# LayoutLLM-T2I/LayoutLLM-T2I

Hardware: AMD Instinct MI355X
Metric: 512x512 50-step images/sec (PLMS, CFG 7.5, layout-conditioned GLIGEN UNet) (higher is better)
Workload: dtype fp16 (fp32 accumulate); 1 GPU; configs[1]: 512x512, 50 PLMS steps, batch=4/GPU, 8 grounding boxes/image, fp16; survey_config=2, unet_forwards_per_image=102, parallelism=replicas x1, one weight broadcast, no per-step collectives

## Files before the change

include/gligen_hip.h:

```cpp
#ifndef GLIGEN_HIP_H
#define GLIGEN_HIP_H

#include <stdint.h>

#ifdef __cplusplus
extern "C" {
#endif

#define GL_ABI_VERSION 15

#define GL_ERR_BAD_ARG (-1)
#define GL_ERR_UNSUPPORTED (-2)

enum gl_epilogue {
    GL_EPI_BIAS = 0,
    GL_EPI_SILU = 1,
    GL_EPI_GEGLU = 2,
    GL_EPI_RES = 3,
    GL_EPI_GATE_RES = 4,
    GL_EPI_ROWBIAS = 5
};

enum gl_out_mode {
    GL_OUT_F16_ROWMAJOR = 0,
// ... 213 lines not shown
int gl_conv3x3(const gl_conv_args* a, void* stream);
int gl_conv3x3_pad01(const gl_conv_args* a, void* stream);
int gl_attention(const gl_attn_args* a, void* stream);

typedef struct gl_vae_config {
    int32_t ch;
    int32_t ch_mult[8];
    int32_t n_mult;
    int32_t num_res_blocks;
    int32_t z_channels;
    int32_t out_ch;
    int32_t embed_dim;
    float scale_factor;
} gl_vae_config;
typedef struct gl_vae gl_vae;
int gl_vae_create(const gl_vae_config* cfg, gl_vae** out);
int gl_vae_destroy(gl_vae* v);
int gl_vae_num_weights(const gl_vae* v);
int gl_vae_weight_at(const gl_vae* v, int32_t i, gl_weight_info* info);
int64_t gl_vae_weights_bytes(const gl_vae* v);
int gl_vae_load_weights(gl_vae* v, const void* packed, int64_t bytes, void* stream);
int gl_vae_decode(gl_vae* v, const float* z, int32_t B, int32_t side, float* out, int32_t use_graph, void* stream);
int gl_vae_decode_hw(gl_vae* v, const float* z, int32_t B, int32_t h, int32_t w, float* out, int32_t use_graph, void* stream);
int gl_vae_num_launches(const gl_vae* v);
int64_t gl_vae_pool_bytes(const gl_vae* v);
int gl_sizeof_vae_config(void);
int gl_vae_encoder_create(const gl_vae_config* cfg, gl_vae** out);
int gl_vae_encode(gl_vae* v, const float* x, int32_t B, int32_t side, const float* noise, float* z, int32_t use_graph, void* stream);
int gl_vae_encode_hw(gl_vae* v, const float* x, int32_t B, int32_t h, int32_t w, const float* noise, float* z, int32_t use_graph,
                     void* stream);

int gl_clip_patchify(const float* pixel_values, int32_t B, int32_t S, int32_t patch, int32_t Kpad, void* out, void* stream);
int gl_clip_assemble(const void* patch_emb, int32_t ldpe, const float* class_emb, const float* pos_emb, int32_t B, int32_t T,
                     int32_t C, const float* ln_gamma, const float* ln_beta, float ln_eps, float* x, void* stream);
int gl_clip_embed_tokens(const int32_t* ids, const float* tok_emb, const float* pos_emb, int32_t B, int32_t T, int32_t C,
                         int32_t vocab, float* x, void* stream);
int gl_clip_gather_rows(const float* x, int32_t ldx, const int32_t* rows, int32_t B, int32_t C, float* out, void* stream);
int gl_attention_small(const void* q, const void* k, const void* v, int32_t ld, int32_t B, int32_t T, int32_t H, int32_t d,
                       float scale, int32_t causal, void* out, int32_t ldo, void* stream);

int gl_image_to_u8(const float* img_nchw, int32_t B, int32_t H, int32_t W, uint8_t* out_hwc, void* stream);
int gl_resample_h_u8(const uint8_t* in, int32_t B, int32_t H, int32_t W, const int32_t* bounds, const int32_t* coeffs, int32_t ksize,
                     int32_t Wout, uint8_t* out, void* stream);
int gl_resample_v_norm(const uint8_t* in, int32_t B, int32_t H, int32_t W, const int32_t* bounds, const int32_t* coeffs, int32_t ksize,
                       int32_t Hout, int32_t top, int32_t left, int32_t crop_h, int32_t crop_w, const float* mean3, const float* std3,
                       float* out_nchw, uint8_t* out_u8_hwc, void* stream);

int gl_abi_version(void);
int gl_sizeof_gemm_args(void);
int gl_sizeof_conv_args(void);
int gl_sizeof_attn_args(void);
int gl_sizeof_gn_args(void);
int gl_set_option(int key, int value);
int gl_set_handle_option(gl_engine* e, int key, int value);
int gl_clear_handle_options(gl_engine* e);
int gl_vae_set_option(gl_vae* v, int key, int value);
int gl_debug_read(int what, void* dst, int64_t bytes);
int gl_init(void);

#ifdef __cplusplus
}
#endif
#endif
```

layoutllm_t2i_amd/_lib.py:

```python
from __future__ import annotations

import ctypes as C
import os

_HERE = os.path.dirname(os.path.abspath(__file__))
LIB_PATH = os.path.join(_HERE, os.path.basename(os.environ.get("GLIGEN_HIP_LIB", "") or "libgligen_hip.so"))
ABI_VERSION = 15

EPI_BIAS, EPI_SILU, EPI_GEGLU, EPI_RES, EPI_GATE_RES, EPI_ROWBIAS = range(6)
OUT_F16_ROWMAJOR, OUT_F32_NCHW, OUT_F32_ROWMAJOR, OUT_F16_HILO = 0, 1, 2, 3

GROUNDING_IDS = {"text": 0, "text_image": 1}

vp = C.c_void_p
i32 = C.c_int32
i64 = C.c_int64
f32 = C.c_float
fp = C.c_void_p


class GemmArgs(C.Structure):
    _fields_ = [
        ("a", vp), ("lda", i32),
        ("a2", vp), ("lda2", i32), ("ksplit", i32),
# ... 117 lines not shown
    "gl_layernorm": (i32, [vp, i32, i32, vp, i32, fp, fp, i32, i32, i32, i32, i32, f32, fp, vp, i32, i32, vp]),
    "gl_layernorm_stats": (i32, [fp, i32, i32, i32, f32, fp, vp]),
    "gl_split_f32": (i32, [fp, i32, i64, i32, vp, i32, vp]),
    "gl_timestep_embedding_f32": (i32, [fp, i32, i32, fp, vp]),
    "gl_posnet_input_f32": (i32, [fp, fp, fp, fp, fp, i32, i32, i32, fp, vp]),
    "gl_rela_pool_ln3": (i32, [fp, fp, fp, fp, i32, i32, i32, i32, vp, vp, vp, i32, i32, vp, fp, fp, vp, vp]),
    "gl_rela_pool": (i32, [vp, i32, i32, i32, i32, vp, vp, vp, i32, i32, vp, fp, fp, vp, vp]),
    "gl_rela_merge": (i32, [vp, i32, vp, fp, fp, fp, vp, i32, i32, i32, i32, vp, vp, vp, i32, i32, vp, fp, fp, vp, vp]),
    "gl_posnet_input": (i32, [fp, fp, fp, fp, fp, i32, i32, i32, vp, vp]),
    "gl_timestep_embedding": (i32, [fp, i32, i32, vp, vp]),
    "gl_silu_f16": (i32, [vp, vp, i64, vp]),
    "gl_cfg_combine": (i32, [fp, f32, i64, fp, vp]),
    "gl_plms_update": (i32, [fp, fp, fp, fp, fp, f32, f32, f32, f32, f32, f32, f32, f32, f32, i64, fp, vp]),
    "gl_pack_latent": (i32, [fp, i32, i32, i32, i32, i32, i32, vp, vp]),
    "gl_pack_latent_extra": (i32, [fp, fp, i32, i32, i32, i32, i32, i32, i32, i32, vp, vp]),
    "gl_latent_affine_pack": (i32, [fp, fp, fp, f32, i32, i32, i32, i32, vp, vp]),
    "gl_softmax_rows": (i32, [vp, i32, i32, i32, f32, vp]),
    "gl_abi_version": (i32, []),
    "gl_sizeof_gemm_args": (i32, []),
    "gl_sizeof_conv_args": (i32, []),
    "gl_sizeof_attn_args": (i32, []),
    "gl_init": (i32, []),
    "gl_create": (i32, [C.POINTER(UNetConfigC), C.POINTER(vp)]),
    "gl_destroy": (i32, [vp]),
    "gl_num_weights": (i32, [vp]),
    "gl_weight_at": (i32, [vp, i32, C.POINTER(WeightInfo)]),
    "gl_weights_bytes": (i64, [vp]),
    "gl_load_weights": (i32, [vp, vp, i64, i32, vp]),
    "gl_set_conditioning": (i32, [vp, fp, fp, fp, fp, fp, i32, i32, i32, i32, vp]),
    "gl_set_conditioning_hw": (i32, [vp, fp, fp, fp, fp, fp, i32, i32, i32, i32, i32, vp]),
    "gl_set_conditioning_ti": (i32, [vp, fp, fp, fp, fp, fp, fp, fp, fp, i32, i32, i32, i32, i32, vp]),
    "gl_posnet_input_ti": (i32, [fp, fp, fp, fp, fp, fp, fp, fp, fp, i32, i32, i32, vp, vp, vp]),
    "gl_posnet_input_ti_f32": (i32, [fp, fp, fp, fp, fp, fp, fp, fp, fp, i32, i32, i32, fp, fp, vp]),
    "gl_image_ground_feature": (i32, [fp, fp, i32, i32, f32, fp, vp]),
    "gl_set_inpaint_extra": (i32, [vp, fp, i32, vp]),
    "gl_last_error": (i32, [vp, C.c_char_p, i32]),
    "gl_unet_forward": (i32, [vp, fp, fp, f32, i32, f32, i32, fp, i32, vp]),
    "gl_plms_step": (i32, [vp, C.POINTER(PlmsStepArgs), vp]),
    "gl_pool_bytes": (i64, [vp]),
    "gl_num_launches": (i32, [vp]),
    "gl_sizeof_unet_config": (i32, []),
    "gl_sizeof_weight_info": (i32, []),
    "gl_sizeof_plms_step_args": (i32, []),
    "gl_reward_score": (i32, [C.POINTER(RewardArgs), vp]),
    "gl_sizeof_reward_args": (i32, []),
    "gl_ff_fused": (i32, [C.POINTER(FFArgs), vp]),
    "gl_ff_fused_supported": (i32, [i32]),
    "gl_ff_fused_applicable": (i32, [i32, i32]),
    "gl_sizeof_ff_args": (i32, []),
    "gl_image_to_u8": (i32, [vp, i32, i32, i32, vp, vp]),
    "gl_resample_h_u8": (i32, [vp, i32, i32, i32, vp, vp, i32, i32, vp, vp]),
    "gl_resample_v_norm": (i32, [vp, i32, i32, i32, vp, vp, i32, i32, i32, i32, i32, i32, vp, vp, vp, vp, vp]),
    "gl_set_option": (i32, [i32, i32]),
    "gl_set_handle_option": (i32, [vp, i32, i32]),
    "gl_clear_handle_options": (i32, [vp]),
    "gl_vae_set_option": (i32, [vp, i32, i32]),
    "gl_debug_read": (i32, [i32, vp, i64]),
    "gl_vae_create": (i32, [C.POINTER(VaeConfigC), C.POINTER(vp)]),
    "gl_vae_destroy": (i32, [vp]),
    "gl_vae_num_weights": (i32, [vp]),
    "gl_vae_weight_at": (i32, [vp, i32, C.POINTER(WeightInfo)]),
    "gl_vae_weights_bytes": (i64, [vp]),
    "gl_vae_load_weights": (i32, [vp, vp, i64, vp]),
    "gl_vae_decode": (i32, [vp, fp, i32, i32, fp, i32, vp]),
    "gl_vae_decode_hw": (i32, [vp, fp, i32, i32, i32, fp, i32, vp]),
    "gl_vae_num_launches": (i32, [vp]),
    "gl_vae_pool_bytes": (i64, [vp]),
    "gl_sizeof_vae_config": (i32, []),
    "gl_vae_encoder_create": (i32, [C.POINTER(VaeConfigC), C.POINTER(vp)]),
    "gl_vae_encode": (i32, [vp, fp, i32, i32, fp, fp, i32, vp]),
    "gl_vae_encode_hw": (i32, [vp, fp, i32, i32, i32, fp, fp, i32, vp]),
    "gl_conv3x3_pad01": (i32, [C.POINTER(ConvArgs), vp]),
    "gl_vae_posterior": (i32, [fp, fp, fp, fp, f32, i32, i32, i32, i32, fp, fp, vp]),
    "gl_latent_blend": (i32, [fp, fp, fp, fp, f32, f32, i32, i32, i32, i32, i32, vp]),
    "gl_clip_patchify": (i32, [fp, i32, i32, i32, i32, vp, vp]),
    "gl_clip_assemble": (i32, [vp, i32, fp, fp, i32, i32, i32, fp, fp, f32, fp, vp]),
    "gl_clip_embed_tokens": (i32, [vp, fp, fp, i32, i32, i32, i32, fp, vp]),
    "gl_clip_gather_rows": (i32, [fp, i32, vp, i32, i32, fp, vp]),
    "gl_attention_small": (i32, [vp, vp, vp, i32, i32, i32, i32, i32, f32, i32, vp, i32, vp]),
}

_lib = None
_inited = set()


class HipLibraryError(RuntimeError):
    pass


def lib() -> C.CDLL:
    global _lib
    if _lib is not None:
        return _lib
    if not os.path.exists(LIB_PATH):
        raise HipLibraryError(
            f"{LIB_PATH} not found: build it with `python -m layoutllm_t2i_amd.csrc.build` "
            "(or __graft_entry__.build()).  There is no CPU fallback for the denoising path.")
    try:
        l = C.CDLL(LIB_PATH)
    except OSError as e:
        raise HipLibraryError(f"cannot load {LIB_PATH}: {e}") from e
    for name, (res, args) in PROTOTYPES.items():
        try:
            fn = getattr(l, name)
        except AttributeError as e:
            raise HipLibraryError(f"{LIB_PATH} does not export {name}") from e
        fn.restype = res
        fn.argtypes = args
    if l.gl_abi_version() != ABI_VERSION:
        raise HipLibraryError(f"ABI version mismatch: lib {l.gl_abi_version()} vs host {ABI_VERSION}")
    for cls, fn in ((GemmArgs, l.gl_sizeof_gemm_args), (ConvArgs, l.gl_sizeof_conv_args), (AttnArgs, l.gl_sizeof_attn_args),
                    (UNetConfigC, l.gl_sizeof_unet_config), (WeightInfo, l.gl_sizeof_weight_info),
                    (PlmsStepArgs, l.gl_sizeof_plms_step_args), (RewardArgs, l.gl_sizeof_reward_args), (FFArgs, l.gl_sizeof_ff_args),
                    (VaeConfigC, l.gl_sizeof_vae_config), (GnArgs, l.gl_sizeof_gn_args)):
        if C.sizeof(cls) != fn():
            raise HipLibraryError(f"struct size mismatch for {cls.__name__}: host {C.sizeof(cls)} vs lib {fn()}")
    _lib = l
    return l


def init_device(index=None) -> None:
    import torch
    if index is None:
        index = torch.cuda.current_device()
    if index not in _inited:
        with torch.cuda.device(index):
            check(lib().gl_init(), "gl_init")
        _inited.add(index)


def unet_config_c(cfg) -> UNetConfigC:
    c = UNetConfigC()
    c.in_channels, c.model_channels, c.out_channels, c.num_res_blocks = cfg.in_channels, cfg.model_channels, cfg.out_channels, cfg.num_res_blocks
    if len(cfg.channel_mult) > 8 or len(cfg.attention_resolutions) > 8:
        raise ValueError("at most 8 levels / attention resolutions")
    c.n_levels = len(cfg.channel_mult)
    for i, m in enumerate(cfg.channel_mult):
        c.channel_mult[i] = int(m)
    c.n_attn_res = len(cfg.attention_resolutions)
    for i, m in enumerate(cfg.attention_resolutions):
        c.attention_resolutions[i] = int(m)
    c.num_heads, c.context_dim = cfg.num_heads, cfg.context_dim
    c.pos_in_dim, c.pos_out_dim, c.fourier_freqs, c.max_objs = cfg.pos_in_dim, cfg.pos_out_dim, cfg.fourier_freqs, cfg.max_objs
    c.split_weights = int(bool(getattr(cfg, "split_weights", False)))
    c.grounding = GROUNDING_IDS[getattr(cfg, "grounding", "text")]
    c.inpaint_mode = int(bool(getattr(cfg, "inpaint_mode", False)))
    c.no_relation = int(not getattr(cfg, "relation", True))
    return c


def create_engine(cfg) -> int:
    h = vp()
    cc = unet_config_c(cfg)
    check(lib().gl_create(C.byref(cc), C.byref(h)), "gl_create")
    return h.value


def create_vae(cfg, encoder: bool = False) -> int:
    cc = VaeConfigC()
    cc.ch, cc.n_mult, cc.num_res_blocks, cc.z_channels, cc.out_ch = cfg.ch, len(cfg.ch_mult), cfg.num_res_blocks, cfg.z_channels, cfg.out_ch
    for i, m in enumerate(cfg.ch_mult):
        cc.ch_mult[i] = int(m)
    cc.embed_dim, cc.scale_factor = cfg.embed_dim, float(cfg.scale_factor)
    h = vp()
    if encoder:
        check(lib().gl_vae_encoder_create(C.byref(cc), C.byref(h)), "gl_vae_encoder_create")
    else:
        check(lib().gl_vae_create(C.byref(cc), C.byref(h)), "gl_vae_create")
    return h.value


def vae_weight_table(handle: int):
    l = lib()
    out = []
    info = WeightInfo()
    for i in range(l.gl_vae_num_weights(handle)):
        check(l.gl_vae_weight_at(handle, i, C.byref(info)), "gl_vae_weight_at")
        out.append((info.name.decode(), int(info.offset), int(info.nbytes), int(info.dtype), tuple(int(info.shape[k]) for k in range(info.ndim))))
    return out, int(l.gl_vae_weights_bytes(handle))


def weight_table(handle: int):
    l = lib()
    out = []
    info = WeightInfo()
    for i in range(l.gl_num_weights(handle)):
        check(l.gl_weight_at(handle, i, C.byref(info)), "gl_weight_at")
        out.append((info.name.decode(), int(info.offset), int(info.nbytes), int(info.dtype), tuple(int(info.shape[k]) for k in range(info.ndim))))
    return out, int(l.gl_weights_bytes(handle))


def last_error(handle: int) -> str:
    buf = C.create_string_buffer(512)
    n = lib().gl_last_error(handle, buf, len(buf))
    return buf.value.decode() if n > 0 else ""


def check(code: int, what: str) -> None:
    if code != 0:
        raise HipLibraryError(f"{what} failed with code {code}" + (" (bad argument)" if code == -1 else ""))
```

layoutllm_t2i_amd/csrc/engine.hip:

```cpp
#include "common.h"
#include "gligen_hip.h"
#include "opts.h"

#include <cmath>
#include <cstring>
#include <map>
#include <string>
#include <tuple>
#include <unordered_map>
#include <vector>


namespace {

constexpr int CIN_PAD = 64;
constexpr int64_t ALIGN = 256;
#define g_fuse_merge_ln gl_opt(25)
#define g_fuse_vt gl_opt(21)
#define g_force_fuser gl_opt(20)
#define g_precise gl_opt(41)
#define g_h1_f32 gl_opt(42)
#define g_rela_compact gl_opt(43)
#define g_w3 gl_opt(45)
#define g_in_split gl_opt(38)
// ... 39 lines not shown
    for (size_t i = (size_t)blockIdx.x * blockDim.x + threadIdx.x; i < total; i += (size_t)gridDim.x * blockDim.x) {
        const int wd = (int)(i % words);
        const size_t row = i / words;
        const int k = (int)(row % n);
        const size_t cb = row / n;
        const int b = (int)(cb % B), c = (int)(cb / B);
        dst[(((size_t)b * 2 + c) * n + k) * words + wd] = src[i];
    }
}

#pragma clang fp contract(off)
__device__ __forceinline__ void py_slice(int start, int stop, int len, int* s, int* e) {
    if (start < 0) { start += len; if (start < 0) start = 0; } else if (start > len) start = len;
    if (stop < 0) { stop += len; if (stop < 0) stop = 0; } else if (stop > len) stop = len;
    *s = start;
    *e = stop > start ? stop : start;
}
__global__ void rela_rects_kernel(const float* __restrict__ boxes, const float* __restrict__ masks, int B, int n, int h, int w,
                                  int* __restrict__ rects, int* __restrict__ nvalid, int* __restrict__ poison) {
    const int k = blockIdx.x * blockDim.x + threadIdx.x;
    if (k >= B) return;
    float count = 0.0f;
    for (int i = 0; i < n; ++i) count += masks[(size_t)k * n + i];
    int nv = 0, bad = 0;
    bool open = true;
    for (int i = 0; i < n; ++i) {
        int* r = rects + ((size_t)k * n + i) * 4;
        r[0] = r[1] = r[2] = r[3] = 0;
        if (!open) continue;
        const float* bx = boxes + ((size_t)k * n + i) * 4;
        const int left = (int)(bx[0] * (float)w);
        const int top = (int)(bx[1] * (float)h);
        const int right = (int)fminf(bx[2] * (float)w, (float)w);
        const int bottom = (int)fminf(bx[3] * (float)h, (float)h);
        if ((float)i < count && left != right && top != bottom) {
            int t, b, l, rr;
            py_slice(top, bottom, h, &t, &b);
            py_slice(left, right, w, &l, &rr);
            r[0] = t; r[1] = b; r[2] = l; r[3] = rr;
            if ((b - t) * (rr - l) == 0) bad = 1;
            nv = i + 1;
        } else {
            open = false;
        }
    }
    nvalid[k] = nv;
    poison[k] = bad;
}
#pragma clang fp contract(fast)

}

struct gl_engine {
    bool strict_hoists_ok = false;
    int strict_hoists_w3 = -1;
    gl_unet_config cfg;
    std::vector<BlockD> input_blocks, output_blocks;
    BlockD middle;
    int out_channels_last = 0;
    std::vector<LayerD> st_layers;
    std::vector<std::string> names;
    std::unordered_map<std::string, WInfo> tab;
    int64_t total_bytes = 0;
    const char* wbase = nullptr;
    bool has_sd = false;
    std::unordered_map<std::string, int> emb_off;
    int emb_total = 0;
    std::vector<float> gate_tanh;
    struct Buf { void* p; size_t bytes; };
    std::unordered_map<std::string, Buf> pool;
    bool pool_changed = false, capturing = false;
    int device = -1;
    bool cond_set = false;
    int Bn = 0, R = 0, Lc = 0, lat_h = 0, lat_w = 0;
    bool extra_set = false;
    int extra_bs = 0;
    std::map<GraphKey, hipGraphExec_t> graphs;
    float fuser_scale_cur = -1e30f;
    std::vector<float> gate_host;
    float* gate_pin[2] = {nullptr, nullptr};
    hipEvent_t gate_pin_ev[2] = {nullptr, nullptr};
    bool gate_pin_used[2] = {false, false};
    size_t gate_pin_bytes = 0;
    int gate_pin_next = 0;
    int launches = 0;
    int rel_slots = 0;
    int opt_epoch = 0;
    int ovr_epoch = 0;
    gl_opt_overrides ovr;
    std::string err;
    hipStream_t cap_stream = nullptr;

    const WInfo* wi(const std::string& n) const {
        auto it = tab.find(n);
        return it == tab.end() ? nullptr : &it->second;
    }
    const void* W(const std::string& n) const {
        auto it = tab.find(n);
        if (it == tab.end() || wbase == nullptr) return nullptr;
        return wbase + it->second.off;
    }
    const float* Wf(const std::string& n) const { return reinterpret_cast<const float*>(W(n)); }

    void* buf(const std::string& tag, size_t bytes) {
        auto it = pool.find(tag);
        if (it != pool.end() && it->second.bytes >= bytes) return it->second.p;
// ... 72 lines not shown
            BlockD b;
            b.layers.push_back(LayerD{RES, "input_blocks." + std::to_string(idx) + ".0", ch, mult * mc, 0});
            ch = mult * mc;
            if (has_attn(ds)) b.layers.push_back(LayerD{ST, "input_blocks." + std::to_string(idx) + ".1", ch, ch, ch / heads});
            e->input_blocks.push_back(b);
            chans.push_back(ch);
        }
        if (level != c.n_levels - 1) {
            const int idx = (int)e->input_blocks.size();
            e->input_blocks.push_back(BlockD{{LayerD{DOWN, "input_blocks." + std::to_string(idx) + ".0.op", ch, ch, 0}}});
            chans.push_back(ch);
            ds *= 2;
        }
    }
    e->middle.layers = {LayerD{RES, "middle_block.0", ch, ch, 0}, LayerD{ST, "middle_block.1", ch, ch, ch / heads},
                        LayerD{RES, "middle_block.2", ch, ch, 0}};
    for (int level = c.n_levels - 1; level >= 0; --level) {
        const int mult = c.channel_mult[level];
        for (int i = 0; i <= c.num_res_blocks; ++i) {
            const int ich = chans.back();
            chans.pop_back();
            const int idx = (int)e->output_blocks.size();
            BlockD b;
            b.layers.push_back(LayerD{RES, "output_blocks." + std::to_string(idx) + ".0", ch + ich, mc * mult, 0});
            ch = mc * mult;
            if (has_attn(ds)) b.layers.push_back(LayerD{ST, "output_blocks." + std::to_string(idx) + ".1", ch, ch, ch / heads});
            if (level && i == c.num_res_blocks) {
                b.layers.push_back(LayerD{UP, "output_blocks." + std::to_string(idx) + "." + std::to_string(b.layers.size()) + ".conv", ch, ch, 0});
                ds /= 2;
            }
            e->output_blocks.push_back(b);
        }
    }
    e->out_channels_last = ch;
}

template <class F>
void for_all_layers(gl_engine* e, F f) {
    for (auto& b : e->input_blocks) for (auto& l : b.layers) f(l);
    for (auto& l : e->middle.layers) f(l);
    for (auto& b : e->output_blocks) for (auto& l : b.layers) f(l);
}

void build_table(gl_engine* e) {
    const gl_unet_config& c = e->cfg;
    const int mc = c.model_channels, te = 4 * mc, ctx = c.context_dim;
    add_lin(e, "time_embed.0", te, mc);
    add_lin(e, "time_embed.2", te, te);
    add_conv3(e, "input_blocks.0.0", CIN_PAD, mc, false);
    if (!c.inpaint_mode) add_conv3(e, "sd_first_conv", CIN_PAD, mc, false);
    int off = 0;
    for_all_layers(e, [&](LayerD& l) {
        const std::string& p = l.prefix;
        if (l.kind == DOWN || l.kind == UP) {
            add_conv3(e, p, l.cin, l.cout);
        } else if (l.kind == RES) {
            add_norm(e, p + ".in_layers.0", l.cin);
            add_conv3(e, p + ".in_layers.2", l.cin, l.cout);
            add_norm(e, p + ".out_layers.0", l.cout);
            add_conv3(e, p + ".out_layers.3", l.cout, l.cout);
            if (l.cin != l.cout) add_lin_split(e, p + ".skip_connection", l.cout, l.cin);
            e->emb_off[p] = off;
            off += l.cout;
        } else if (l.kind == ST) {
            const int C = l.cin;
            e->st_layers.push_back(l);
            add_norm(e, p + ".norm", C);
            add_lin_split(e, p + ".proj_in", C, C);
            add_lin_split(e, p + ".proj_out", C, C);
            const std::string t = p + ".transformer_blocks.0";
            add_mat(e, t + ".attn1.qkv.w", 3 * C, C);
            add_lin(e, t + ".attn1.o", C, C);
            add_mat(e, t + ".attn2.q.w", C, C);
            add_mat(e, t + ".attn2.kv.w", 2 * C, ctx);
            add_lin(e, t + ".attn2.o", C, C);
            add_ff(e, t + ".ff", C);
            for (const char* n : {".norm1", ".norm2", ".norm3"}) add_norm(e, t + n, C);
            const std::string f = t + ".fuser";
            add_lin(e, f + ".linear", C, ctx);
            add_mat(e, f + ".attn.qkv.w", 3 * C, C);
            add_lin(e, f + ".attn.o", C, C);
            add_ff(e, f + ".ff", C);
            add_norm(e, f + ".norm1", C);
            add_norm(e, f + ".norm2", C);
            add_w(e, f + ".tanh_attn", 1, {1});
            add_w(e, f + ".tanh_dense", 1, {1});
            if (c.no_relation) return;
            const std::string r = t + ".rela_fuse";
            add_mat(e, r + ".attn.q.w", C, C);
            add_mat(e, r + ".attn.kv.w", 2 * C, ctx);
            add_lin(e, r + ".attn.o", C, C);
            add_ff(e, r + ".ff", C);
            for (const char* n : {".norm1", ".norm2", ".norm3"}) add_norm(e, r + n, C);
            add_w(e, r + ".tanh_attn", 1, {1});
            add_w(e, r + ".tanh_dense", 1, {1});
        }
    });
    e->emb_total = off;
    add_lin(e, "emb_all", off, te);
    add_norm(e, "out.0", e->out_channels_last);
    add_conv3(e, "out.2", e->out_channels_last, c.out_channels);
    if (c.grounding == 1) {
        add_w(e, "position_net.null_text", 1, {c.pos_in_dim});
        add_w(e, "position_net.null_image", 1, {c.pos_in_dim});
        add_w(e, "position_net.null_xyxy", 1, {8 * c.fourier_freqs});
        for (const char* n : {"position_net.linears_text", "position_net.linears_image"}) {
            const std::string p = n;
// ... 57 lines not shown
        const WInfo* wi = e->wi(p + ".w");
        if (!wi) return GL_ERR_BAD_ARG;
        gl_gemm_args g{};
        g.a = a.p; g.lda = a.ld; g.a2 = o.a2.p; g.lda2 = o.a2.ld; g.ksplit = o.ksplit;
        g.w = e->W(p + ".w"); g.bias = o.bias ? e->Wf(p + ".b") : nullptr;
        if (o.bias && !g.bias) return GL_ERR_BAD_ARG;
        g.M = M; g.N = (int)wi->shape[0]; g.K = (int)wi->shape[1];
        const bool strict = g_strict != 0 && e->cfg.split_weights;
        if (o.wsplit || e->cfg.split_weights) {
            const int Kc = g.K / 2;
            g.ldw = g.K; g.K = Kc;
            if (a.hilo) {
                g.kwrap = Kc; g.K = 2 * Kc;
                const bool third = strict ? (g_strict_w3 != 0) : (o.wsplit && g_w3 > 0 && M > (g_w3 < 1024 ? 1024 : g_w3));
                if (third) {
                    if (o.a2.p != nullptr) return GL_ERR_BAD_ARG;
                    g.K = 3 * Kc; g.a2 = a.p; g.lda2 = a.ld; g.ksplit = 2 * Kc;
                }
            }
        } else if (a.hilo) {
            g.kwrap = g.K; g.ldw = g.K; g.K = 2 * g.K;
        }
        g.epi = o.epi; g.out_mode = o.out_mode; g.out = out; g.ldc = ldc;
        g.res = o.res.p; g.ldres = o.res.ld; g.res_f32 = o.res.f32; g.gate = o.gate;
        g.out2 = o.out2; g.ldc2 = o.ldc2;
        if (o.tail) {
            const VtTail& t = *o.tail;
            g.vt = t.vt; g.vt_lo = t.vt_lo; g.vt_col0 = t.col0; g.vt_rows = t.rows; g.vt_d = t.d; g.vt_ld = t.ld; g.vt_H = t.H;
        }
        g.workspace = ws; g.workspace_bytes = GL_WS_BYTES;
        ++launches;
        return gl_gemm(&g, st);
    }
    int gemm(Act a, const std::string& p, int M, void* out, int ldc) { return gemm(a, p, M, out, ldc, GemmOpt{}); }

    struct RowBias { const void* p = nullptr; int ld = 0, rows_per_sample = 0; };
    struct ConvOpt {
        int stride = 1, ups = 0, epi = GL_EPI_BIAS;
        Rows res{};
        RowBias rowbias{};
        void* out2 = nullptr;
        int nchw_hw = 0;
    };
    int conv(Act in, const std::string& p, int B, int Hin, int Win, void* out, int out_mode, const ConvOpt& o) {
        const WInfo* wi = e->wi(p + ".w");
        if (!wi) return GL_ERR_BAD_ARG;
        const int Cin = in.hilo ? in.ld / 2 : in.ld;
        gl_conv_args a{};
        a.w_split = wi->shape[1] == 18 * (int64_t)Cin;
        a.in_split = in.hilo ? ((a.w_split && g_strict_w3 != 0) ? 3 : 2) : 0;
        a.in = in.p; a.B = B; a.Hin = Hin; a.Win = Win; a.Cin = Cin;
        a.Hout = o.ups ? 2 * Hin : (Hin + 2 - 3) / o.stride + 1;
        a.Wout = o.ups ? 2 * Win : (Win + 2 - 3) / o.stride + 1;
        a.stride = o.stride; a.upsample2x = o.ups;
        a.g.w = e->W(p + ".w"); a.g.bias = e->Wf(p + ".b"); a.g.N = (int)wi->shape[0];
        a.g.epi = o.epi; a.g.out_mode = out_mode; a.g.out = out; a.g.ldc = a.g.N; a.g.hw = o.nchw_hw;
        a.g.res = o.res.p; a.g.ldres = o.res.ld; a.g.res_f32 = o.res.f32;
        a.g.rowbias = o.rowbias.p; a.g.ld_rowbias = o.rowbias.ld; a.g.rows_per_sample = o.rowbias.rows_per_sample;
        a.g.rowbias_f32 = o.rowbias.p != nullptr && (g_precise != 0 || g_strict != 0);
        a.g.out2 = o.out2; a.g.ldc2 = a.g.N;
        a.g.workspace = ws; a.g.workspace_bytes = GL_WS_BYTES;
        ++launches;
        return gl_conv3x3(&a, st);
    }

    enum LnFlags { LN_X_F32 = 1, LN_X2_F32 = 4, LN_Y_HILO = 8 };
    struct LnOpt {
        int rows_out = 0;
        float* stats = nullptr;
        Rows x2{}; int rows2 = 0;
        bool y_lo = false;
    };
    int ln(Rows x, half_t* y, int ldy, const std::string& p, int rows, int C, const LnOpt& o) {
        const int flags = (x.f32 ? LN_X_F32 : 0) | (o.x2.f32 ? LN_X2_F32 : 0) | (o.y_lo ? LN_Y_HILO : 0);
        ++launches;
        return gl_layernorm(x.p, x.ld, flags, y, ldy, e->Wf(p + ".g"), e->Wf(p + ".b"), e->Bn, rows, o.rows_out ? o.rows_out : rows, 0, C, 1e-5f, o.stats,
                            o.x2.p, C, o.rows2, st);
    }
    int ln(Rows x, half_t* y, int ldy, const std::string& p, int rows, int C) { return ln(x, y, ldy, p, rows, C, LnOpt{}); }
    int split(const float* x, int64_t rows, int C, half_t* y) {
        ++launches;
        return gl_split_f32(x, C, rows, C, y, 2 * C, st);
    }
    struct GnOpt {
        const void* x2 = nullptr; int C2 = 0;
        int ldo = 0;
        half_t* out_lo = nullptr;
        half_t* raw = nullptr; int ldraw = 0;
    };
    int gn(Rows x, int HW, const std::string& p, float eps, int silu, half_t* out, const GnOpt& o) {
        const int B = e->Bn, nchunk = gn_nchunk(HW);
        float* partial = e->f32("gn.partial", (size_t)B * nchunk * 64);
        CKP(partial);
        launches += gl_groupnorm_launches_ex(x.ld + o.C2, HW, x.f32);
        gl_gn_args a{};
        a.x1 = x.p; a.C1 = x.ld; a.x2 = o.x2; a.C2 = o.C2; a.x_f32 = x.f32; a.B = B; a.HW = HW;
        a.gamma = e->Wf(p + ".g"); a.beta = e->Wf(p + ".b"); a.eps = eps; a.silu = silu;
        a.out = out; a.ldo = o.ldo; a.out_lo = o.out_lo; a.raw = o.raw; a.ldraw = o.ldraw;
        a.partial = partial; a.nchunk = nchunk;
        return gl_groupnorm_ex(&a, st);
    }
    int gn(Rows x, int HW, const std::string& p, float eps, int silu, half_t* out) { return gn(x, HW, p, eps, silu, out, GnOpt{}); }
    int attn(Mat q, Mat k, VtMat vt, MatOut out, int d, int Nq, int Nk) {
        gl_attn_args a{};
        a.q_lo = q.lo; a.k_lo = k.lo; a.vt_lo = vt.lo; a.out_lo = out.lo;
        a.q = q.p; a.q_bstride = q.bs; a.ldq = q.ld; a.k = k.p; a.k_bstride = k.bs; a.ldk = k.ld; a.vt = vt.p; a.ldvt = vt.ld;
        a.out = out.p; a.o_bstride = out.bs; a.ldo = out.ld; a.B = e->Bn; a.H = e->cfg.num_heads; a.d = d; a.Nq = Nq; a.Nk = Nk;
        a.scale = 1.0f / sqrtf((float)d);
// ... 427 lines not shown
                }
                CK(r.conv(in, l.prefix, Bn, sh, sw, o.f, GL_OUT_F32_ROWMAJOR, {.stride = up ? 1 : 2, .ups = up, .out2 = o.h}));
                sh = oh; sw = ow;
            } else {
                return GL_ERR_BAD_ARG;
            }
            h = o;
            h_c = l.cout;
            if (half_pending && !(j + 1 < b.layers.size() && b.layers[j + 1].kind == ST)) {
                CK(r.dup_rows(h.f, (size_t)B0 * sh * sw * h_c * 4));
                if (h.h) CK(r.dup_rows(h.h, (size_t)B0 * sh * sw * h_c * 2));
                half_pending = false;
            }
        }
        return 0;
    };

    for (size_t i = 1; i < e->input_blocks.size(); ++i) {
        CK(run_block(e->input_blocks[i], "skip." + std::to_string(i), nullptr, i + 1 < e->input_blocks.size() ? &e->input_blocks[i + 1] : &e->middle,
                     share && i == 1));
        skips.push_back({h, sh, sw, h_c});
    }
    CK(run_block(e->middle, "mid", nullptr, e->output_blocks.empty() ? nullptr : &e->output_blocks[0]));
    for (size_t i = 0; i < e->output_blocks.size(); ++i) {
        const Skip sk = skips.back();
        skips.pop_back();
        if (sk.h != sh || sk.w != sw) return GL_ERR_BAD_ARG;
        CK(run_block(e->output_blocks[i], "out." + std::to_string(i), &sk, i + 1 < e->output_blocks.size() ? &e->output_blocks[i + 1] : nullptr));
    }
    const int ocl = e->out_channels_last;
    half_t* g = e->h16("fin.gn", (size_t)Bn * sh * sw * ocl * (strict ? 2 : 1));
    CKP(g);
    if (!precise) CKP(h.h);
    CK(r.gn({precise ? (const void*)h.f : (const void*)h.h, ocl, precise}, sh * sw, "out.0", 1e-5f, 1, g,
            {.ldo = strict ? 2 * ocl : 0, .out_lo = strict ? g + ocl : nullptr}));
    CK(r.conv({g, strict ? 2 * ocl : ocl, strict}, "out.2", Bn, sh, sw, eps, GL_OUT_F32_NCHW, {.nchw_hw = sh * sw}));
    if (n_launches) *n_launches = r.launches;
    return 0;
}

}

extern "C" int gl_create(const gl_unet_config* cfg, gl_engine** out) {
    if (!cfg || !out) return GL_ERR_BAD_ARG;
    if (cfg->n_levels <= 0 || cfg->n_levels > 8 || cfg->n_attn_res < 0 || cfg->n_attn_res > 8 || cfg->num_heads <= 0) return GL_ERR_BAD_ARG;
    if (cfg->model_channels % 64 || cfg->context_dim % 64 || cfg->pos_in_dim % 8 || cfg->pos_out_dim != cfg->context_dim) return GL_ERR_UNSUPPORTED;
    if ((cfg->pos_in_dim + 8 * cfg->fourier_freqs) % 64) return GL_ERR_UNSUPPORTED;
    if (cfg->grounding != 0 && cfg->grounding != 1) return GL_ERR_UNSUPPORTED;
    if (cfg->max_objs <= 0 || n_ground(*cfg) > 64) return GL_ERR_UNSUPPORTED;
    if (cfg->no_relation != 0 && cfg->no_relation != 1) return GL_ERR_UNSUPPORTED;
    if ((cfg->inpaint_mode != 0 && cfg->inpaint_mode != 1) || first_conv_in(*cfg) > CIN_PAD) return GL_ERR_UNSUPPORTED;
    gl_engine* e = new gl_engine();
    e->cfg = *cfg;
    build_plan(e);
    build_table(e);
    *out = e;
    return 0;
}

extern "C" int gl_destroy(gl_engine* e) {
    if (!e) return GL_ERR_BAD_ARG;
    e->drop_graphs();
    for (auto& kv : e->pool) (void)hipFree(kv.second.p);
    if (e->cap_stream) (void)hipStreamDestroy(e->cap_stream);
    for (int k = 0; k < 2; ++k) {
        if (e->gate_pin_ev[k]) { (void)hipEventSynchronize(e->gate_pin_ev[k]); (void)hipEventDestroy(e->gate_pin_ev[k]); }
        if (e->gate_pin[k]) (void)hipHostFree(e->gate_pin[k]);
    }
    delete e;
    return 0;
}

extern "C" int gl_num_weights(const gl_engine* e) { return e ? (int)e->names.size() : GL_ERR_BAD_ARG; }
extern "C" int64_t gl_weights_bytes(const gl_engine* e) { return e ? e->total_bytes : -1; }
extern "C" int gl_weight_at(const gl_engine* e, int32_t i, gl_weight_info* info) {
    if (!e || !info || i < 0 || i >= (int)e->names.size()) return GL_ERR_BAD_ARG;
    const std::string& n = e->names[i];
    if (n.size() >= sizeof(info->name)) return GL_ERR_BAD_ARG;
    const WInfo& w = e->tab.at(n);
    memset(info, 0, sizeof(*info));
    memcpy(info->name, n.c_str(), n.size());
    info->offset = w.off; info->nbytes = w.bytes; info->dtype = w.dtype; info->ndim = w.ndim;
    for (int k = 0; k < 4; ++k) info->shape[k] = w.shape[k];
    return 0;
}

extern "C" int gl_load_weights(gl_engine* e, const void* packed, int64_t bytes, int32_t has_sd_conv, void* stream) {
    if (!e || !packed || bytes < e->total_bytes) return GL_ERR_BAD_ARG;
    if (reinterpret_cast<uintptr_t>(packed) % 16) return GL_ERR_BAD_ARG;
    int dev = 0;
    if (hipGetDevice(&dev) != hipSuccess) return GL_ERR_BAD_ARG;
    e->device = dev;
    CK(gl_init());
    e->wbase = reinterpret_cast<const char*>(packed);
    if (has_sd_conv && e->cfg.inpaint_mode) {
        e->err = "gl_load_weights: an inpaint_mode handle has no sd_first_conv slots (its first conv is not restorable)";
        return GL_ERR_BAD_ARG;
    }
    e->has_sd = has_sd_conv != 0;
    e->drop_graphs();
    const size_t n = e->st_layers.size();
    e->gate_tanh.assign(n * 4, 0.0f);
    hipStream_t st = (hipStream_t)stream;
    if (hipStreamSynchronize(st) != hipSuccess) return GL_ERR_BAD_ARG;
    for (size_t i = 0; i < n; ++i) {
        const std::string t = e->st_layers[i].prefix + ".transformer_blocks.0";
// ... 424 lines not shown
```

layoutllm_t2i_amd/csrc/gemm8.hip:

```cpp
#include "common.h"
#include "gligen_hip.h"
#include "gemm_shared.h"
#include "opts.h"
#include <atomic>
#include <type_traits>

#ifndef G8_S3_PHASES
#define G8_S3_PHASES 3
#endif

namespace {

template <int BM_, int BN>
struct G8 {
    static constexpr int BM = BM_;
    static constexpr int NA = BM / 64;
    static constexpr int MI = BM / 64;
    static constexpr int MH = BM / 128;
    static constexpr int BK = 64;
    static constexpr int PW = BN / 2;
    static constexpr int TN = PW / 16;
    static constexpr int A_BYTES = BM * BK * 2;
    static constexpr int B_BYTES = BN * BK * 2;
    static constexpr int STAGE = A_BYTES + B_BYTES;
    static constexpr int NST = 3;
    static constexpr int LDS = NST * STAGE;
    static constexpr int B_UNITS = BN / 8;
    static constexpr int NB0 = (B_UNITS + 7) / 8;
    static constexpr int NB1 = B_UNITS / 4 - NB0;
    static constexpr int NI0 = NA + NB0;
    static constexpr int NI1 = NA + NB1;
    static_assert(PW % 16 == 0 && B_UNITS % 4 == 0 && NB1 >= 1 && (BM == 256 || BM == 128), "tile shape");
    static_assert(NA + 1 >= 3, "the first phase issues three instructions (X_FIRST): two A units + one B unit at least");
    static_assert(STAGE % 128 == 0, "stage alignment (the k-half XOR of the fragment offsets relies on it)");
};

template <int BN>
struct G8X {
    static constexpr int A_UNITS = 33;
    static constexpr int A_BYTES = A_UNITS * 1024;
    static constexpr int A_STRIDE = A_BYTES + 128;
    static constexpr int B_BYTES = BN * 64 * 2;
    static constexpr int B_BASE = 2 * A_STRIDE;
    static constexpr int LDS = B_BASE + 3 * B_BYTES;
    static_assert(A_STRIDE % 128 == 0 && B_BASE % 128 == 0, "the k-half XOR of the fragment offsets stays inside a 128-byte row");
    static_assert(LDS >= 8 * 32 * (BN / 2 + 4) * 4, "the epilogue restages through the ring memory");
};

template <int N>
__device__ __forceinline__ void wait_vm() {
    asm volatile("s_waitcnt vmcnt(%0)" ::"n"(N) : "memory");
}

__device__ __forceinline__ f32x4 mfma16(half8_t a, half8_t b, f32x4 c) {
    return __builtin_amdgcn_mfma_f32_16x16x32_f16(a, b, c, 0, 0, 0);
}

#define G8_SBAR()                              \
    do {                                       \
        __builtin_amdgcn_sched_barrier(0);     \
        __builtin_amdgcn_s_barrier();          \
        __builtin_amdgcn_sched_barrier(0);     \
    } while (0)

__device__ unsigned long long g8_stamps[4 * 4096];

template <int BM, int BN, bool CONV, int DBG = 0, bool S3 = false, bool KXR = false>
__global__ __launch_bounds__(512, 2) void gemm8_kernel(gl_gemm_args p, ConvGeom cg, int splitk, int kt_per_split, int order_flags) {
    using C = G8<BM, BN>;
    constexpr int KT = S3 ? 32 : 64;
    constexpr int NA = C::NA, MI = C::MI, MH = C::MH;
    unsigned long long ts0 = 0, ts1 = 0, ts2 = 0;
    if constexpr (DBG & 1) ts0 = __builtin_readcyclecounter();
    constexpr int TN = C::TN, PW = C::PW;
    extern __shared__ __attribute__((aligned(16))) unsigned char smem[];

    const int tid = threadIdx.x;
    const int lane = tid & 63;
    const int wave = __builtin_amdgcn_readfirstlane(tid >> 6);
    const int grp = wave >> 2;
    const int wm = wave & 3;
    const int M = p.M, N = p.N, K = S3 ? p.kwrap : p.K;

    const int nt = (N + BN - 1) / BN;
    int tile;
    {
        const int nwg = gridDim.x;
        const int bid = blockIdx.x;
        const int q = nwg >> 3, r = nwg & 7;
        const int xcd = bid & 7, local = bid >> 3;
        tile = (xcd < r ? xcd * (q + 1) : r * (q + 1) + (xcd - r) * q) + local;
    }
    const int mt_ = (M + C::BM - 1) / C::BM;
    const int order_m = order_flags & 1;
    const bool tap_major = CONV && (order_flags & 2);
    const int tmi = order_m ? tile % mt_ : tile / nt;
    const int m0 = tmi * C::BM;
    const int n0 = (order_m ? tile / mt_ : tile - tmi * nt) * BN;
    const int kt_begin = blockIdx.z * kt_per_split;
    const int kt_end = min(K / KT, kt_begin + kt_per_split);
    const int nkt = kt_end - kt_begin;

    const half_t* __restrict__ Ag = reinterpret_cast<const half_t*>(p.a);
    const half_t* __restrict__ A2g = reinterpret_cast<const half_t*>(p.a2);
    const half_t* __restrict__ Wg = reinterpret_cast<const half_t*>(p.w);
    const half_t* zsrc = cg.zero;

    const int srow = lane >> 3;
    const int sslot = lane & 7;
    int a_dst[NA];
    const half_t* aptr[NA];
    unsigned amask = 0u;
    unsigned cmask[NA];
    const int k_first = kt_begin * KT;
    const int a_lo = S3 ? (CONV ? (cg.Cin >> 1) : p.kwrap) : 0;
    auto chunk_off = [&](const int c, const int lo_off) __attribute__((always_inline)) -> int {
        if constexpr (S3) return ((c & 3) << 3) + ((c >> 2) ? lo_off : 0);
        else return c << 3;
    };
#pragma unroll
    for (int u = 0; u < NA; ++u) {
        const int trow0 = (16 * NA) * (wave >> 1) + 16 * (wave & 1) + 8 * (u & 1) + 32 * (u >> 1);
        a_dst[u] = trow0 * 128;
        const int r = trow0 + srow;
        const int gc = chunk_off(sslot ^ ((r >> 1) & 7), a_lo);
        const int m = m0 + r;
        const bool rowok = m < M;
        aptr[u] = zsrc; cmask[u] = 0u;
        if constexpr (CONV) {
            if (rowok) {
                int b, oy, ox;
                const int hw = cg.Hout * cg.Wout;
                if (((cg.Wout & (cg.Wout - 1)) | (hw & (hw - 1))) == 0) {
                    const int lw = __builtin_ctz(cg.Wout), lhw = __builtin_ctz(hw);
                    b = m >> lhw;
                    const int rr = m & (hw - 1);
                    oy = rr >> lw;
                    ox = rr & (cg.Wout - 1);
                } else {
                    b = m / hw;
                    const int rr = m - b * hw;
                    oy = rr / cg.Wout;
                    ox = rr - oy * cg.Wout;
                }
                const int sh = S3 ? 0 : cg.shift;
                const int iy = cg.ups ? oy : oy * cg.stride + sh, ix = cg.ups ? ox : ox * cg.stride + sh;
                const int hlim = cg.ups ? cg.Hout : cg.Hin, wlim = cg.ups ? cg.Wout : cg.Win;
                const unsigned rb = (iy >= 1 ? 1u : 0u) | 2u | (iy + 1 < hlim ? 4u : 0u);
                const unsigned cb = (ix >= 1 ? 1u : 0u) | 2u | (ix + 1 < wlim ? 4u : 0u);
                cmask[u] = ((rb & 1u) ? cb : 0u) | (cb << 3) | ((rb & 4u) ? (cb << 6) : 0u) | ((unsigned)(oy & 1) << 9) | ((unsigned)(ox & 1) << 10);
                const int sy = cg.ups ? (oy >> 1) : iy, sx = cg.ups ? (ox >> 1) : ix;
                aptr[u] = cg.in + ((size_t)(b * cg.Hin + sy) * cg.Win + sx) * cg.Cin + gc;
            }
        } else {
            if (rowok) {
                if (!S3 && A2g != nullptr && k_first >= p.ksplit) aptr[u] = A2g + (size_t)m * p.lda2 + (k_first - p.ksplit) + gc;
                else aptr[u] = Ag + (size_t)m * p.lda + k_first + gc;
                amask |= 1u << u;
            }
        }
    }
    const int nb = grp ? C::NB1 : C::NB0;
    const int bunit0 = grp ? 4 * C::NB0 + C::NB1 * (wave - 4) : C::NB0 * wave;
    const half_t* bptr[C::NB0];
    unsigned bmask = 0u;
#pragma unroll
    for (int j = 0; j < C::NB0; ++j) {
        const int r = 8 * (bunit0 + j) + srow;
        const int gc = chunk_off(sslot ^ ((r >> 1) & 7), p.kwrap);
        const int n = n0 + r;
        const bool ok = (j < nb) && (r < BN) && (n < N);
        bptr[j] = ok ? (Wg + (size_t)n * p.ldw + gc) : zsrc;
        if (ok) bmask |= 1u << j;
    }

    const int ncblk = CONV ? K / 576 : 1;
    const int in_lim = tap_major ? ncblk : 9;
    int is_out = 0, is_in = 0;
    int is_cblk = 0, is_tap = 0;
    if constexpr (CONV) {
        const int t64 = S3 ? (kt_begin >> 1) : kt_begin;
        is_out = t64 / in_lim;
        is_in = t64 - is_out * in_lim;
    }
    int is_kt = kt_begin;

    int is_off = 0;
    int is_ky = 0, is_kx = 0, is_acb = 0;
    int is_boff = 0;
    auto issue_begin = [&]() __attribute__((always_inline)) {
        if constexpr (CONV && S3) {
            is_tap = tap_major ? is_out : is_in;
            is_cblk = tap_major ? is_in : is_out;
            is_ky = (is_tap * 11) >> 5;
            is_kx = is_tap - is_ky * 3;
            is_acb = (is_cblk << 1) + (is_kt & 1);
            is_off = ((is_ky - 1) * cg.Win + (is_kx - 1)) * cg.Cin + (is_acb << 5);
            is_boff = ((is_cblk * 9 + is_tap) << 6) + ((is_kt & 1) << 5);
        } else if constexpr (S3) {
            is_boff = is_kt << 5;
        } else if constexpr (CONV) {
            is_tap = tap_major ? is_out : is_in;
            is_cblk = tap_major ? is_in : is_out;
            is_ky = (is_tap * 11) >> 5;
            is_kx = is_tap - is_ky * 3;
            is_acb = (cg.cwrap != 0 && is_cblk >= cg.cwrap) ? is_cblk - cg.cwrap : is_cblk;
            is_off = ((is_ky - 1) * cg.Win + (is_kx - 1)) * cg.Cin + (is_acb << 6);
            is_boff = (is_cblk * 9 + is_tap) << 6;
            if (p.kwrap != 0 && is_boff >= p.kwrap) is_boff -= p.kwrap;
        } else {
            is_boff = is_kt << 6;
            if (p.kwrap != 0 && is_boff >= p.kwrap) is_boff -= p.kwrap;
            if (A2g != nullptr && is_kt * 64 == p.ksplit && is_kt != kt_begin) {
#pragma unroll
                for (int u = 0; u < NA; ++u) {
                    const int r = (a_dst[u] >> 7) + srow;
                    const int m = m0 + r;
                    if (m < M) aptr[u] = A2g + (size_t)m * p.lda2 + ((sslot ^ ((r >> 1) & 7)) << 3);
                }
            }
        }
    };
    auto unit_src = [&](const int i) __attribute__((always_inline)) -> const half_t* {
        const half_t* src;
        if (i < NA) {
            const int u = i;
            if constexpr (CONV) {
                int off = is_off;
                if (cg.ups) {
                    const int ry = (is_ky - 1 + (int)((cmask[u] >> 9) & 1u)) >> 1, rx = (is_kx - 1 + (int)((cmask[u] >> 10) & 1u)) >> 1;
                    off = (ry * cg.Win + rx) * cg.Cin + (is_acb << (S3 ? 5 : 6));
                }
                const uint64_t a = reinterpret_cast<uint64_t>(aptr[u] + off), z = reinterpret_cast<uint64_t>(zsrc);
                const uint64_t keep = (uint64_t)0 - (uint64_t)((cmask[u] >> is_tap) & 1u);
                src = reinterpret_cast<const half_t*>((a & keep) | (z & ~keep));
            } else {
                src = aptr[u];
                aptr[u] += ((amask >> u) & 1u) ? KT : 0;
            }
            if constexpr (DBG & 2) src = zsrc;
        } else {
            const int j = i - NA;
            src = ((bmask >> (j < C::NB0 ? j : 0)) & 1u) ? bptr[j < C::NB0 ? j : 0] + is_boff : zsrc;
            if constexpr (DBG & 4) src = zsrc;
        }
        return src;
    };
    auto unit_fire = [&](const int st, const int i, const half_t* src) __attribute__((always_inline)) {
        unsigned char* sbase = smem + st * C::STAGE;
        if (i < NA) {
            glds16(src, reinterpret_cast<half_t*>(sbase + a_dst[i]));
        } else {
            const int j = i - NA;
            if (j < nb) glds16(src, reinterpret_cast<half_t*>(sbase + C::A_BYTES + (bunit0 + j) * 1024));
        }
    };
    auto issue_unit = [&](const int st, const int i) __attribute__((always_inline)) { unit_fire(st, i, unit_src(i)); };
    auto issue_advance = [&]() __attribute__((always_inline)) {
        ++is_kt;
        if constexpr (CONV) {
            if (!S3 || (is_kt & 1) == 0) {
                if (++is_in == in_lim) { is_in = 0; ++is_out; }
            }
        }
    };
    auto issue_all = [&](const int st) __attribute__((always_inline)) {
        issue_begin();
#pragma unroll
        for (int i = 0; i < NA + C::NB0; ++i) issue_unit(st, i);
        issue_advance();
    };

    const int lr = lane & 15, lq = lane >> 4;
    const int fsw = ((lq ^ ((lr >> 1) & 7)) << 4);
    const int a_off = ((BM / 4) * wm + lr) * 128 + fsw;
    const int b_off = C::A_BYTES + (PW * grp + lr) * 128 + fsw;

    f32x4 acc[MI][TN];
#pragma unroll
    for (int mi = 0; mi < MI; ++mi)
#pragma unroll
        for (int ni = 0; ni < TN; ++ni)
// ... 291 lines not shown
                acc[mi][ni] = mfma16(bf[ni], use_lo ? al[mi] : ah[mi], acc[mi][ni]);
                if constexpr (MORE) {
                    if constexpr (cnt > 0) { if (i == GP - 1) unit_fire(st_is, first + 0, nsrc[0]); }
                    if constexpr (cnt > 1) { if (i == 2 * GP - 1) unit_fire(st_is, first + 1, nsrc[1]); }
                    if constexpr (cnt > 2) { if (i == 3 * GP - 1) unit_fire(st_is, first + 2, nsrc[2]); }
                    if constexpr (cnt > 3) { if (i == 4 * GP - 1) unit_fire(st_is, first + 3, nsrc[3]); }
                    if constexpr (cnt > 4) { if (i == 5 * GP - 1) unit_fire(st_is, first + 4, nsrc[4]); }
                }
            }
            if constexpr (MORE) {
                if constexpr (cnt > 0) { __builtin_amdgcn_sched_group_barrier(0x008, GP, 0); __builtin_amdgcn_sched_group_barrier(0x020, 1, 0); }
                if constexpr (cnt > 1) { __builtin_amdgcn_sched_group_barrier(0x008, GP, 0); __builtin_amdgcn_sched_group_barrier(0x020, 1, 0); }
                if constexpr (cnt > 2) { __builtin_amdgcn_sched_group_barrier(0x008, GP, 0); __builtin_amdgcn_sched_group_barrier(0x020, 1, 0); }
                if constexpr (cnt > 3) { __builtin_amdgcn_sched_group_barrier(0x008, GP, 0); __builtin_amdgcn_sched_group_barrier(0x020, 1, 0); }
                if constexpr (cnt > 4) { __builtin_amdgcn_sched_group_barrier(0x008, GP, 0); __builtin_amdgcn_sched_group_barrier(0x020, 1, 0); }
                __builtin_amdgcn_sched_group_barrier(0x008, TOT - cnt * GP, 0);
            }
            __builtin_amdgcn_s_setprio(0);
            if constexpr (MORE && LAST) issue_advance();
            G8_SBAR();
        };
        phase(std::integral_constant<int, 0>{});
        phase(std::integral_constant<int, 1>{});
        if constexpr (NPH == 3) phase(std::integral_constant<int, 2>{});
        st_rd = (st_rd == 2) ? 0 : st_rd + 1;
        st_is = (st_is == 2) ? 0 : st_is + 1;
    };
    int t = 0;
    if constexpr (KXR) {
    } else if constexpr (S3) {
        for (; t + 2 < nkt; ++t) ktile3(std::true_type{});
        for (; t < nkt; ++t) ktile3(std::false_type{});
    } else {
        for (; t + 2 < nkt; ++t) ktile(std::true_type{});
        for (; t < nkt; ++t) ktile(std::false_type{});
    }
    if (grp == 0) G8_SBAR();
    if constexpr (DBG & 1) ts2 = __builtin_readcyclecounter();

    constexpr int EPS = PW + 4;
    constexpr int CG8 = PW / 8;
    constexpr int ITEMS = 32 * CG8;
    static_assert(ITEMS % 64 == 0, "whole sweeps");
    float* stage = reinterpret_cast<float*>(smem) + wave * (32 * EPS);
    const int epi = p.epi;
    const float* __restrict__ bias = p.bias;
    float gate = 1.0f;
    if (splitk == 1 && epi == GL_EPI_GATE_RES) gate = p.gate[0];
    const int nbase = n0 + PW * grp;
    half_t* outp = reinterpret_cast<half_t*>(p.out);
    constexpr int NQ = ITEMS / 64;
    const bool vt_wave = p.vt != nullptr && nbase >= p.vt_col0;
    const bool generic = splitk == 1 && !vt_wave && epi != GL_EPI_GEGLU;
    Fin8Aux aux[MH][NQ];
    if (generic) {
#pragma unroll
        for (int h = 0; h < MH; ++h)
#pragma unroll
            for (int q = 0; q < NQ; ++q) {
                const int idx = lane + 64 * q;
                const int r = idx / CG8, c = (idx - r * CG8) * 8;
                const int m = m0 + (BM / 4) * wm + 32 * h + r, n = nbase + c;
                if (m < M && n < N) fin8_load(p, m, n, aux[h][q]);
            }
    }
    float vt_bias[2] = {0.0f, 0.0f};
    if (splitk == 1 && vt_wave && bias) {
#pragma unroll
        for (int j = 0; j < 2; ++j) {
            const int col = 64 * j + lane;
            if (col < PW && nbase + col < N) vt_bias[j] = bias[nbase + col];
        }
    }
    float gg_bias[16];
#pragma unroll
    for (int j = 0; j < 16; ++j) gg_bias[j] = 0.0f;
    if constexpr (PW == 64) {
        if (splitk == 1 && epi == GL_EPI_GEGLU && bias) {
            const int nx = nbase + (lane & 3) * 8;
            if (nx < N) {
#pragma unroll
                for (int j = 0; j < 8; ++j) { gg_bias[j] = bias[nx + j]; gg_bias[8 + j] = bias[nx + 32 + j]; }
            }
        }
    }
#pragma unroll
    for (int h = 0; h < MH; ++h) {
        const int mbase = m0 + (BM / 4) * wm + 32 * h;
        __builtin_amdgcn_fence(__ATOMIC_RELEASE, "wavefront");
        __builtin_amdgcn_wave_barrier();
#pragma unroll
        for (int mi = 0; mi < 2; ++mi)
#pragma unroll
            for (int ni = 0; ni < TN; ++ni)
                *reinterpret_cast<float4*>(stage + (16 * mi + lr) * EPS + 16 * ni + 4 * lq) =
                    make_float4(acc[2 * h + mi][ni][0], acc[2 * h + mi][ni][1], acc[2 * h + mi][ni][2], acc[2 * h + mi][ni][3]);
        __builtin_amdgcn_fence(__ATOMIC_RELEASE, "wavefront");
        __builtin_amdgcn_wave_barrier();
        if (splitk > 1) {
            float* ws = reinterpret_cast<float*>(p.workspace) + (size_t)blockIdx.z * M * N;
#pragma unroll
            for (int q = 0; q < ITEMS / 64; ++q) {
                const int idx = lane + 64 * q;
                const int r = idx / CG8, c = (idx - r * CG8) * 8;
                const int m = mbase + r, n = nbase + c;
                if (m < M && n < N) {
                    float* o = ws + (size_t)m * N + n;
                    *reinterpret_cast<float4*>(o) = *reinterpret_cast<const float4*>(stage + r * EPS + c);
                    *reinterpret_cast<float4*>(o + 4) = *reinterpret_cast<const float4*>(stage + r * EPS + c + 4);
                }
            }
        } else if (vt_wave) {
            half_t* vtp = reinterpret_cast<half_t*>(p.vt);
#pragma unroll
            for (int c0 = 0; c0 < PW; c0 += 64) {
                const int col = c0 + lane;
                const int n = nbase + col;
                if (col < PW && n < N) {
                    const int nv = n - p.vt_col0;
                    const int hh = nv / p.vt_d;
                    const int cc = nv - hh * p.vt_d;
                    const float bv = vt_bias[c0 / 64];
                    half_t* vtl = reinterpret_cast<half_t*>(p.vt_lo);
#pragma unroll
                    for (int tg = 0; tg < 4; ++tg) {
                        const int m = mbase + tg * 8;
                        if (m >= M) continue;
                        half8_t o, l;
#pragma unroll
                        for (int k = 0; k < 8; ++k) {
                            float v = stage[(tg * 8 + k) * EPS + col] + bv;
                            if (vtl) v = pin_value(v);
                            o[k] = (half_t)v;
                            l[k] = vtl ? (half_t)(v - (float)o[k]) : (half_t)0.0f;
                        }
                        if ((p.vt_rows & 7) == 0) {
                            const int b = m / p.vt_rows;
                            const int key = m - b * p.vt_rows;
                            const size_t at = ((size_t)(b * p.vt_H + hh) * p.vt_d + cc) * p.vt_ld + key;
                            st16(vtp + at, *reinterpret_cast<uint4*>(&o));
                            if (vtl) st16(vtl + at, *reinterpret_cast<uint4*>(&l));
                        } else {
#pragma unroll
                            for (int k = 0; k < 8; ++k) {
                                const int mm = m + k;
                                if (mm < M) {
                                    const int b = mm / p.vt_rows;
                                    const int key = mm - b * p.vt_rows;
                                    const size_t at = ((size_t)(b * p.vt_H + hh) * p.vt_d + cc) * p.vt_ld + key;
                                    vtp[at] = o[k];
                                    if (vtl) vtl[at] = l[k];
                                }
                            }
                        }
                    }
                }
            }
        } else if (epi == GL_EPI_GEGLU) {
            if constexpr (PW == 64) {
#pragma unroll
                for (int ps = 0; ps < 2; ++ps) {
                    const int r = ps * 16 + (lane >> 2);
                    const int pc = (lane & 3) * 8;
                    const int m = mbase + r;
                    const int nx = nbase + pc;
                    if (m < M && nx < N) {
                        const float4 x0 = *reinterpret_cast<const float4*>(stage + r * EPS + pc);
                        const float4 x1 = *reinterpret_cast<const float4*>(stage + r * EPS + pc + 4);
                        const float4 g0 = *reinterpret_cast<const float4*>(stage + r * EPS + pc + 32);
                        const float4 g1 = *reinterpret_cast<const float4*>(stage + r * EPS + pc + 36);
                        float xv[8] = {x0.x, x0.y, x0.z, x0.w, x1.x, x1.y, x1.z, x1.w};
                        float gv[8] = {g0.x, g0.y, g0.z, g0.w, g1.x, g1.y, g1.z, g1.w};
                        half8_t o, lo8 = {};
#pragma unroll
                        for (int j = 0; j < 8; ++j) {
                            const float a = xv[j] + gg_bias[j], b = gv[j] + gg_bias[8 + j];
                            float y = a * gelu_erf_f(b);
                            if (p.out_mode == GL_OUT_F16_HILO) y = pin_value(y);
                            o[j] = (half_t)y;
                            if (p.out_mode == GL_OUT_F16_HILO) lo8[j] = (half_t)(y - (float)o[j]);
                        }
                        st16(outp + (size_t)m * p.ldc + (nbase >> 1) + pc, *reinterpret_cast<uint4*>(&o));
                        if (p.out_mode == GL_OUT_F16_HILO) st16(outp + (size_t)m * p.ldc + (N >> 1) + (nbase >> 1) + pc, *reinterpret_cast<uint4*>(&lo8));
                    }
                }
            }
        } else {
#pragma unroll
            for (int q = 0; q < NQ; ++q) {
                const int idx = lane + 64 * q;
                const int r = idx / CG8, c = (idx - r * CG8) * 8;
                const int m = mbase + r, n = nbase + c;
                if (m < M && n < N) {
                    const float4 a0 = *reinterpret_cast<const float4*>(stage + r * EPS + c);
                    const float4 a1 = *reinterpret_cast<const float4*>(stage + r * EPS + c + 4);
                    float v[8] = {a0.x, a0.y, a0.z, a0.w, a1.x, a1.y, a1.z, a1.w};
                    fin8_store(p, gate, m, n, v, aux[h][q]);
                }
            }
        }
    }
    if constexpr (DBG & 1) {
        asm volatile("s_waitcnt vmcnt(0)" ::: "memory");
        const unsigned long long ts3 = __builtin_readcyclecounter();
        const int bid = blockIdx.x + gridDim.x * blockIdx.z;
        if (tid == 0 && bid < 4096) {
            g8_stamps[4 * bid + 0] = ts0; g8_stamps[4 * bid + 1] = ts1; g8_stamps[4 * bid + 2] = ts2; g8_stamps[4 * bid + 3] = ts3;
        }
    }
}

#define g8_dbg gl_opt(32)
#define g8_kxr gl_opt(54)

std::atomic<uint64_t> g8_kxr_launches{0};

static bool kxr_default(const gl_gemm_args&, const ConvGeom&, int , int ) { return true; }

constexpr int G8_MAX_DEVICES = 64;
const half_t* g8_zero_page[G8_MAX_DEVICES] = {};

template <int BM, int BN, bool CONV, bool S3 = false>
int launch8(const gl_gemm_args& g, const ConvGeom& cg_in, int zs, int kper, int order_m, hipStream_t st) {
    int dev = -1;
    if (hipGetDevice(&dev) != hipSuccess || dev < 0 || dev >= G8_MAX_DEVICES) return GL_ERR_BAD_ARG;
    if (!g8_zero_page[dev]) return GL_ERR_BAD_ARG;
    ConvGeom cg = cg_in;
    cg.zero = g8_zero_page[dev];
    const int mt = gl_cdiv(g.M, BM), nt = gl_cdiv(g.N, BN);
    dim3 grid(mt * nt, 1, zs);
    bool done = false;
    if constexpr (CONV && !S3 && BM == 256) {
        const bool eligible = cg.stride == 1 && !cg.ups && cg.shift == 0 && g.kwrap == 0 && cg.cwrap == 0 && !(order_m & 2) && kper > 0 &&
                              (kper % 9) == 0 && cg.Hin == cg.Hout && cg.Win == cg.Wout && g.K == 9 * cg.Cin && g.a2 == nullptr;
        if (eligible && (g8_kxr == 1 || (g8_kxr == 2 && kxr_default(g, cg, BN, zs)))) {
            void (*k)(gl_gemm_args, ConvGeom, int, int, int) = gemm8_kernel<BM, BN, true, 0, false, true>;
            if constexpr (BN == 160) {
                if (g8_dbg == 1) k = gemm8_kernel<BM, BN, true, 1, false, true>;
                if (g8_dbg == 3) k = gemm8_kernel<BM, BN, true, 3, false, true>;
            }
            k<<<grid, dim3(512), G8X<BN>::LDS, st>>>(g, cg, zs, kper, order_m);
            GL_CHECK_LAUNCH();
            g8_kxr_launches.fetch_add(1, std::memory_order_relaxed);
            return 0;
        }
    }
    if constexpr (S3) {
        gemm8_kernel<BM, BN, CONV, 0, true><<<grid, dim3(512), G8<BM, BN>::LDS, st>>>(g, cg, zs, kper, order_m);
        done = true;
    } else if constexpr (BN == 160 && BM == 256) {
        void (*k)(gl_gemm_args, ConvGeom, int, int, int) = nullptr;
        if (g8_dbg == 1) k = gemm8_kernel<BM, BN, CONV, 1>;
        if (g8_dbg == 3) k = gemm8_kernel<BM, BN, CONV, 3>;
        if (k) {
            k<<<grid, dim3(512), G8<BM, BN>::LDS, st>>>(g, cg, zs, kper, order_m);
            done = true;
        }
    }
    if (!done) gemm8_kernel<BM, BN, CONV><<<grid, dim3(512), G8<BM, BN>::LDS, st>>>(g, cg, zs, kper, order_m);
    GL_CHECK_LAUNCH();
    return 0;
}

template <int BM, int BN, bool CONV>
int set_attr8() {
    hipError_t e = hipFuncSetAttribute((const void*)gemm8_kernel<BM, BN, CONV>, hipFuncAttributeMaxDynamicSharedMemorySize, G8<BM, BN>::LDS);
    if (e == hipSuccess) e = hipFuncSetAttribute((const void*)gemm8_kernel<BM, BN, CONV, 0, true>, hipFuncAttributeMaxDynamicSharedMemorySize, G8<BM, BN>::LDS);
    if constexpr (CONV && BM == 256) {
        if (e == hipSuccess) e = hipFuncSetAttribute((const void*)gemm8_kernel<BM, BN, true, 0, false, true>, hipFuncAttributeMaxDynamicSharedMemorySize, G8X<BN>::LDS);
        if constexpr (BN == 160) {
            if (e == hipSuccess) e = hipFuncSetAttribute((const void*)gemm8_kernel<BM, BN, true, 1, false, true>, hipFuncAttributeMaxDynamicSharedMemorySize, G8X<BN>::LDS);
            if (e == hipSuccess) e = hipFuncSetAttribute((const void*)gemm8_kernel<BM, BN, true, 3, false, true>, hipFuncAttributeMaxDynamicSharedMemorySize, G8X<BN>::LDS);
        }
    }
    if constexpr (BN == 160 && BM == 256) {
        if (e == hipSuccess) e = hipFuncSetAttribute((const void*)gemm8_kernel<BM, BN, CONV, 1>, hipFuncAttributeMaxDynamicSharedMemorySize, G8<BM, BN>::LDS);
        if (e == hipSuccess) e = hipFuncSetAttribute((const void*)gemm8_kernel<BM, BN, CONV, 3>, hipFuncAttributeMaxDynamicSharedMemorySize, G8<BM, BN>::LDS);
    }
    return e == hipSuccess ? 0 : (int)e;
}

}

int gl8_supported(const gl_gemm_args& g, bool conv, int* bn_out) {
    if (g.out_mode == GL_OUT_F32_NCHW) return 0;
    if ((g.K % 64) != 0 || (g.N % 8) != 0 || g.M < 256) return 0;
    int bn = 128;
    if (g.epi != GL_EPI_GEGLU && (g.N % 160) == 0) bn = 160;
    if (g.vt != nullptr && (g.vt_col0 % (bn / 2)) != 0) {
        if (bn == 160 && (g.vt_col0 % 64) == 0) bn = 128;
        else return 0;
    }
    if (g.a2 != nullptr && (g.ksplit % 64) != 0) return 0;
    *bn_out = bn;
    return 1;
}

template <bool S3>
static int gl8_launch_t(const gl_gemm_args& g, const ConvGeom& cg, bool conv, int bm, int bn, int zs, int kper, int order_m, hipStream_t st) {
    if (bm == 256 && bn == 160) return conv ? launch8<256, 160, true, S3>(g, cg, zs, kper, order_m, st) : launch8<256, 160, false, S3>(g, cg, zs, kper, order_m, st);
    if (bm == 256 && bn == 128) return conv ? launch8<256, 128, true, S3>(g, cg, zs, kper, order_m, st) : launch8<256, 128, false, S3>(g, cg, zs, kper, order_m, st);
    if (bm == 128 && bn == 160) return conv ? launch8<128, 160, true, S3>(g, cg, zs, kper, order_m, st) : launch8<128, 160, false, S3>(g, cg, zs, kper, order_m, st);
    if (bm == 128 && bn == 128) return conv ? launch8<128, 128, true, S3>(g, cg, zs, kper, order_m, st) : launch8<128, 128, false, S3>(g, cg, zs, kper, order_m, st);
    return GL_ERR_UNSUPPORTED;
}
int gl8_launch(const gl_gemm_args& g, const ConvGeom& cg, bool conv, int bm, int bn, int zs, int kper, int order_m, hipStream_t st, bool s3) {
    return s3 ? gl8_launch_t<true>(g, cg, conv, bm, bn, zs, kper, order_m, st) : gl8_launch_t<false>(g, cg, conv, bm, bn, zs, kper, order_m, st);
}

int gl8_init(void) {
    int e;
    void* zp = nullptr;
    int dev = -1;
    if (hipGetDevice(&dev) != hipSuccess || dev < 0 || dev >= G8_MAX_DEVICES) return GL_ERR_BAD_ARG;
    if (hipGetSymbolAddress(&zp, HIP_SYMBOL(g_zero16)) != hipSuccess) return GL_ERR_BAD_ARG;
    g8_zero_page[dev] = reinterpret_cast<const half_t*>(zp);
    if ((e = set_attr8<256, 160, false>())) return e;
    if ((e = set_attr8<256, 160, true>())) return e;
    if ((e = set_attr8<256, 128, false>())) return e;
    if ((e = set_attr8<256, 128, true>())) return e;
    if ((e = set_attr8<128, 160, false>())) return e;
    if ((e = set_attr8<128, 160, true>())) return e;
    if ((e = set_attr8<128, 128, false>())) return e;
    if ((e = set_attr8<128, 128, true>())) return e;
    return 0;
}

uint64_t gl8_kxr_launch_count(void) { return g8_kxr_launches.load(std::memory_order_relaxed); }

int gl8_read_stamps(void* dst, int64_t bytes) {
    if (bytes > (int64_t)sizeof(unsigned long long) * 4 * 4096) return GL_ERR_BAD_ARG;
    hipError_t e = hipMemcpyFromSymbol(dst, HIP_SYMBOL(g8_stamps), (size_t)bytes, 0, hipMemcpyDeviceToHost);
    void* p = nullptr;
    if (e == hipSuccess) e = hipGetSymbolAddress(&p, HIP_SYMBOL(g8_stamps));
    if (e == hipSuccess) e = hipMemset(p, 0, sizeof(unsigned long long) * 4 * 4096);
    return (int)e;
}
```

layoutllm_t2i_amd/csrc/gemm_conv.hip:

```cpp
#include <atomic>
#include <cstring>
#include "common.h"
#include "gligen_hip.h"
#include "gemm_shared.h"
#include "opts.h"

namespace {

#define g_opt_ksplit gl_opt(13)
#define g_opt_geglu32 gl_opt(8)
#define g_opt_big gl_opt(7)
#define g_opt_small gl_opt(4)
#define g_opt_splitk_tiles gl_opt(5)
#define g_opt_splitk_tiles_conv gl_opt(GL_OPT_SPLITK_TILES_CONV)
#define g_opt_splitk_nk gl_opt(6)
#define g_opt_skinny gl_opt(24)
#define g_opt_order gl_opt(23)
#define g_opt_tile gl_opt(2)
#define g_opt_g8 gl_opt(30)
#define g_opt_g8_tiles gl_opt(31)
#define g_opt_g8_tapmajor gl_opt(33)
#define g_opt_g8_minkt gl_opt(34)
std::atomic<uint64_t> g8_launches{0};
#define g_opt_g8_shortk gl_opt(37)
// ... 607 lines not shown
            const long t256 = (long)gl_cdiv(g.M, 256) * gl_cdiv(g.N, bn);
            if (t256 >= g_opt_big) {
                if (shape == 1) return launch<256, 160, 4, 1, CONV, 32>(g, cg, st);
                return launch<256, 128, 4, 1, CONV, 32>(g, cg, st);
            }
        }
        if constexpr (!CONV) {
            if (shape == 3 && (g_opt_ksplit == 2 || ((g_opt_ksplit == 1 || g_opt_ksplit == 4 || g_opt_ksplit == 5) && g.K >= 1024)))
                return launch<64, 128, 1, 2, false, 64, 2>(g, cg, st);
        }
        if (shape == 3) return launch<64, 128, 2, 2, CONV, 64>(g, cg, st);
        if (shape == 1) return launch<128, 160, 4, 1, CONV, 64>(g, cg, st);
        if (shape == 0) return launch<128, 128, 2, 2, CONV, 64>(g, cg, st);
        return launch<256, 64, 4, 1, CONV, 64>(g, cg, st);
    } else {
        static_assert(!CONV, "BK 32 dispatch is for plain GEMMs");
        if (shape == 3) return launch<64, 128, 2, 2, false, 32>(g, cg, st);
        return launch<128, 128, 2, 2, false, 32>(g, cg, st);
    }
}

template <bool CONV>
int dispatch(const gl_gemm_args& g, const ConvGeom& cg, hipStream_t st) {
    if (g.M <= 0 || g.N <= 0 || g.K <= 0 || (g.K % 64) != 0) return GL_ERR_BAD_ARG;
    if (g.out_mode < 0 || g.out_mode > GL_OUT_F16_HILO) return GL_ERR_BAD_ARG;
    if (g.out_mode == GL_OUT_F16_HILO && g.ldc < (g.epi == GL_EPI_GEGLU ? g.N : 2 * g.N)) return GL_ERR_BAD_ARG;
    if ((g.vt != nullptr && (g.out_mode == GL_OUT_F16_HILO) != (g.vt_lo != nullptr)) || (g.vt == nullptr && g.vt_lo != nullptr)) return GL_ERR_BAD_ARG;
    if (g.out_mode != GL_OUT_F32_NCHW && ((g.N % 8) != 0 || (g.ldc % 8) != 0)) return GL_ERR_BAD_ARG;
    if (g.out_mode == GL_OUT_F32_ROWMAJOR && g.out2 != nullptr && (g.ldc2 % 8) != 0) return GL_ERR_BAD_ARG;
    if (g.out_mode == GL_OUT_F32_ROWMAJOR && g.epi == GL_EPI_GEGLU) return GL_ERR_UNSUPPORTED;
    if (g.res != nullptr && (g.ldres % 8) != 0) return GL_ERR_BAD_ARG;
    if (g.rowbias != nullptr && (g.ld_rowbias % 8) != 0) return GL_ERR_BAD_ARG;
    if (g.epi == GL_EPI_GEGLU && (g.N % 64) != 0) return GL_ERR_BAD_ARG;
    if (g.a2 != nullptr && (g.ksplit % 64) != 0) return GL_ERR_BAD_ARG;
    if ((g.epi == GL_EPI_RES || g.epi == GL_EPI_GATE_RES) && g.res == nullptr) return GL_ERR_BAD_ARG;
    if (g.epi == GL_EPI_GATE_RES && g.gate == nullptr) return GL_ERR_BAD_ARG;
    if (g.epi == GL_EPI_ROWBIAS && (g.rowbias == nullptr || g.rows_per_sample <= 0)) return GL_ERR_BAD_ARG;
    if (g.vt != nullptr && (g.epi != GL_EPI_BIAS || (g.out_mode != GL_OUT_F16_ROWMAJOR && g.out_mode != GL_OUT_F16_HILO) || (g.vt_col0 % 64) != 0 || g.vt_col0 <= 0 ||
                            g.vt_col0 >= g.N || g.vt_rows <= 0 || g.vt_d <= 0 || ((g.N - g.vt_col0) % g.vt_d) != 0 || (g.vt_ld % 8) != 0 ||
                            g.vt_ld < g.vt_rows || g.vt_H * g.vt_d != g.N - g.vt_col0))
        return GL_ERR_BAD_ARG;
    if constexpr (!CONV) {
        if (g.vt_lo == nullptr && skinny_ok(g)) {
            gemm_skinny_kernel<<<dim3(g.N / 32, gl_cdiv(g.M, 32)), dim3(256), 0, st>>>(g);
            GL_CHECK_LAUNCH();
            return 0;
        }
    }
    const bool need8 = g.vt_lo != nullptr;
    if (need8) {
        int bn_ = 0;
        if (!g_opt_g8 || !gl8_supported(g, CONV, &bn_)) return GL_ERR_UNSUPPORTED;
    }
    if (g_opt_g8) {
        int bn = 0;
        if (gl8_supported(g, CONV, &bn)) {
            const int nk = g.K / 64;
            auto plan_split = [&](const int tiles_) {
                int sk = 1;
                if (tiles_ < g_opt_g8_tiles && g.workspace && g.epi != GL_EPI_GEGLU && g.vt == nullptr) {
                    sk = 256 / tiles_;
                    if (sk > nk / g_opt_g8_minkt) sk = nk / g_opt_g8_minkt;
                    while (sk > 1 && (int64_t)sk * g.M * g.N * 4 > g.workspace_bytes) --sk;
                    if (sk < 1) sk = 1;
                }
                return sk;
            };
            int bm = 256;
            int tiles = gl_cdiv(g.M, 256) * gl_cdiv(g.N, bn);
            int splitk = plan_split(tiles);
            if (tiles * 2 <= 256 && g.epi != GL_EPI_GEGLU && g.vt == nullptr) {
                const bool want = CONV ? ((g_opt_g8_bm128 & 4) || ((g_opt_g8_bm128 & 1) && nk / splitk <= 16)) : ((g_opt_g8_bm128 & 2) != 0);
                if (want) {
                    bm = 128;
                    tiles = gl_cdiv(g.M, 128) * gl_cdiv(g.N, bn);
                    splitk = plan_split(tiles);
                }
            }
            if (!CONV && (g_opt_g8_bm128 & 8) && bm == 256 && splitk == 1 && tiles > 256 && g.epi != GL_EPI_GEGLU) {
                const int t128 = gl_cdiv(g.M, 128) * gl_cdiv(g.N, bn);
                auto fills = [](const int b) { return b * 5 >= ((b + 255) / 256) * 256 * 4; };
                if (!fills(tiles) && fills(t128) && t128 <= 2048) {
                    bm = 128;
                    tiles = t128;
                }
            }
            if (!CONV && splitk > 1 && nk / splitk < 20) splitk = nk / 20 > 0 ? nk / 20 : 1;
            bool enough = tiles * splitk >= (CONV ? g_opt_g8_tiles : (g_opt_g8_minblk < g_opt_g8_tiles ? g_opt_g8_minblk : g_opt_g8_tiles)) && nk >= g_opt_g8_minnk;
            if (!CONV && enough) {
                const int blocks = tiles * splitk;
                const bool full_rounds = g_opt_g8_shortk && blocks * 5 >= ((blocks + 255) / 256) * 256 * 4;
                enough = nk >= 16 || blocks <= 256 || (g.epi == GL_EPI_GEGLU && (nk >= 10 || full_rounds)) || (full_rounds && blocks <= 2048);
            }
            if (g_opt_g8 == 2 || enough || need8) {
                const bool s3 = g_opt_g8_s3 != 0 && g.kwrap != 0 && g.K == 3 * g.kwrap &&
                                (CONV ? cg.cwrap != 0 : (g.a2 == g.a && g.lda2 == g.lda && g.ksplit == 2 * g.kwrap));
                const int nks = s3 ? g.kwrap / 32 : nk;
                const int kper = gl_cdiv(nks, splitk);
                const int zs = gl_cdiv(nks, kper);
                const int order_m = g_opt_order == 1 ? ((CONV ? 9L : 1L) * g.N > (long)g.M) : (g_opt_order == 2);
                const int e = gl8_launch(g, cg, CONV, bm, bn, zs, kper, order_m | (CONV && g_opt_g8_tapmajor ? 2 : 0), st, s3);
                if (e) return e;
                g8_launches.fetch_add(1, std::memory_order_relaxed);
                if (zs > 1) {
                    const size_t total = (size_t)g.M * (g.N / 8);
                    int nblk = (int)((total + 255) / 256);
                    if (nblk > 2048) nblk = 2048;
                    splitk_reduce_kernel<<<dim3(nblk), dim3(256), 0, st>>>(g, zs);
                    GL_CHECK_LAUNCH();
                }
                return 0;
            }
        }
    }
    if constexpr (!CONV) {
        if (g_opt_geglu32 && g.epi == GL_EPI_GEGLU && g.K <= 640 && g.a2 == nullptr) return dispatch_shape<false, 32>(g, cg, st);
    }
    return dispatch_shape<CONV, 64>(g, cg, st);
}

}

extern "C" int gl_gemm(const gl_gemm_args* a, void* stream) {
    if (!a || !a->a || !a->w || !a->out) return GL_ERR_BAD_ARG;
    ConvGeom cg{};
    gl_gemm_args g = *a;
    if (g.kwrap != 0 && ((g.kwrap % 64) != 0 || g.kwrap >= g.K || g.K > 3 * g.kwrap)) return GL_ERR_BAD_ARG;
    if (g.ldw == 0) g.ldw = g.kwrap != 0 ? g.kwrap : g.K;
    if (g.ldw < (g.kwrap != 0 ? (g.K > 2 * g.kwrap ? 2 * g.kwrap : g.kwrap) : g.K) || (g.ldw % 8) != 0) return GL_ERR_BAD_ARG;
    return dispatch<false>(g, cg, (hipStream_t)stream);
}

namespace {
int conv3x3_entry(const gl_conv_args* a, int shift, void* stream) {
    if (!a || !a->in || !a->g.w || !a->g.out) return GL_ERR_BAD_ARG;
    if ((a->Cin % 64) != 0) return GL_ERR_BAD_ARG;
    if (a->stride != 1 && a->stride != 2) return GL_ERR_BAD_ARG;
    if (a->upsample2x && (a->stride != 1 || a->Hout != 2 * a->Hin || a->Wout != 2 * a->Win)) return GL_ERR_BAD_ARG;
    if (a->B >= 2048 || a->Hout >= 1024 || a->Wout >= 1024) return GL_ERR_BAD_ARG;
    if (a->in_split != 0 && a->in_split != 2 && a->in_split != 3) return GL_ERR_BAD_ARG;
    if (a->in_split == 3 && !a->w_split) return GL_ERR_BAD_ARG;
    gl_gemm_args g = a->g;
    g.a = a->in;
    g.a2 = nullptr;
    g.M = a->B * a->Hout * a->Wout;
    g.K = 9 * a->Cin * (a->in_split ? a->in_split : 1);
    g.ldw = 9 * a->Cin * (a->w_split ? 2 : 1);
    g.kwrap = a->in_split ? 9 * a->Cin : 0;
    ConvGeom cg{reinterpret_cast<const half_t*>(a->in), a->B, a->Hin, a->Win, a->Cin * (a->in_split ? 2 : 1), a->Hout, a->Wout, a->stride,
                a->upsample2x, nullptr, a->in_split == 3 ? 2 * (a->Cin >> 6) : 0, shift};
    return dispatch<true>(g, cg, (hipStream_t)stream);
}
}

extern "C" int gl_conv3x3(const gl_conv_args* a, void* stream) { return conv3x3_entry(a, 0, stream); }

extern "C" int gl_conv3x3_pad01(const gl_conv_args* a, void* stream) {
    if (!a || a->stride != 2 || a->upsample2x != 0 || a->in_split != 0) return GL_ERR_BAD_ARG;
    if (a->Hout != a->Hin / 2 || a->Wout != a->Win / 2 || a->Hout <= 0 || a->Wout <= 0) return GL_ERR_BAD_ARG;
    return conv3x3_entry(a, 1, stream);
}

template <int BM, int BN, int WM, int WN, bool CONV, int BKT, int WK = 1>
int set_lds_attr() {
    hipError_t e = hipFuncSetAttribute((const void*)gemm_kernel<BM, BN, WM, WN, CONV, BKT, WK>,
                                       hipFuncAttributeMaxDynamicSharedMemorySize, lds_bytes<BM, BN, BKT, WM * WN * WK>());
    return e == hipSuccess ? 0 : (int)e;
}
template <int BM, int BN, int WM, int WN, int BKT, int WK = 1>
int set_lds_attr2() {
    int e = set_lds_attr<BM, BN, WM, WN, false, BKT, WK>();
    return e ? e : set_lds_attr<BM, BN, WM, WN, true, BKT, WK>();
}

extern "C" int gl_init_gemm(void) {
    int e;
    if ((e = set_lds_attr2<64, 128, 2, 2, 64>())) return e;
    if ((e = set_lds_attr2<128, 128, 2, 2, 64>())) return e;
    if ((e = set_lds_attr2<128, 160, 4, 1, 64>())) return e;
    if ((e = set_lds_attr2<256, 64, 4, 1, 64>())) return e;
    if ((e = set_lds_attr2<128, 160, 2, 1, 64, 2>())) return e;
    if ((e = set_lds_attr2<128, 128, 2, 1, 64, 2>())) return e;
    if ((e = set_lds_attr<64, 128, 1, 2, false, 64, 2>())) return e;
    if ((e = set_lds_attr2<256, 160, 4, 1, 32>())) return e;
    if ((e = set_lds_attr2<256, 128, 4, 1, 32>())) return e;
    if ((e = set_lds_attr<64, 128, 2, 2, false, 32>())) return e;
    if ((e = set_lds_attr<128, 128, 2, 2, false, 32>())) return e;
    if ((e = gl8_init())) return e;
    return 0;
}

int gl_attn_read_launch_counts(void* dst, int64_t bytes);

extern "C" int gl_debug_read(int what, void* dst, int64_t bytes) {
    if (what == 8) return gl8_read_stamps(dst, bytes);
    if (what == 10) return gl_attn_read_launch_counts(dst, bytes);
    if (what == 9 || what == 11) {
        if (!dst || bytes < (int64_t)sizeof(uint64_t)) return GL_ERR_BAD_ARG;
        const uint64_t n = what == 9 ? g8_launches.load(std::memory_order_relaxed) : gl8_kxr_launch_count();
        memcpy(dst, &n, sizeof n);
        return 0;
    }
    return GL_ERR_BAD_ARG;
}
```

layoutllm_t2i_amd/csrc/gemm_shared.h:

```cpp
#pragma once
#include "common.h"
#include "gligen_hip.h"

static __device__ uint4 g_zero16[4];

struct ConvGeom {
    const half_t* in;
    int B, Hin, Win, Cin, Hout, Wout, stride, ups;
    const half_t* zero;
    int cwrap;
    int shift;
};

namespace {

__device__ __forceinline__ void wait_vmcnt0() { asm volatile("s_waitcnt vmcnt(0)" ::: "memory"); }

__device__ __forceinline__ void glds16(const half_t* src, half_t* dst) {
    __builtin_amdgcn_global_load_lds(
        reinterpret_cast<const __attribute__((address_space(1))) void*>(reinterpret_cast<uintptr_t>(src)),
        reinterpret_cast<__attribute__((address_space(3))) void*>(reinterpret_cast<uintptr_t>(dst)), 16, 0, 0);
}

struct Fin8Aux {
// ... 38 lines not shown
    }
}

__device__ __forceinline__ void fin8_store(const gl_gemm_args& p, float gate, int m, int n, float (&v)[8], const Fin8Aux& a) {
    const int epi = p.epi;
    if (p.bias) {
#pragma unroll
        for (int j = 0; j < 8; ++j) v[j] += a.b[j];
    }
    if (epi == GL_EPI_SILU) {
#pragma unroll
        for (int j = 0; j < 8; ++j) v[j] = silu_f(v[j]);
    } else if (epi == GL_EPI_RES || epi == GL_EPI_ROWBIAS) {
#pragma unroll
        for (int j = 0; j < 8; ++j) v[j] += a.r[j];
    } else if (epi == GL_EPI_GATE_RES) {
#pragma unroll
        for (int j = 0; j < 8; ++j) v[j] = a.r[j] + gate * v[j];
    }
    half_t* o16 = reinterpret_cast<half_t*>(p.out);
    int ld16o = p.ldc;
    if (p.out_mode == GL_OUT_F32_ROWMAJOR) {
        float* o = reinterpret_cast<float*>(p.out) + (size_t)m * p.ldc + n;
        *reinterpret_cast<float4*>(o) = make_float4(v[0], v[1], v[2], v[3]);
        *reinterpret_cast<float4*>(o + 4) = make_float4(v[4], v[5], v[6], v[7]);
        o16 = reinterpret_cast<half_t*>(p.out2);
        ld16o = p.ldc2;
        if (o16 == nullptr) return;
    }
    if (p.out_mode == GL_OUT_F16_HILO) {
#pragma unroll
        for (int j = 0; j < 8; ++j) v[j] = pin_value(v[j]);
    }
    half8_t o;
#pragma unroll
    for (int j = 0; j < 8; ++j) o[j] = (half_t)v[j];
    st16(o16 + (size_t)m * ld16o + n, *reinterpret_cast<uint4*>(&o));
    if (p.out_mode == GL_OUT_F16_HILO) {
        half8_t l;
#pragma unroll
        for (int j = 0; j < 8; ++j) l[j] = (half_t)(v[j] - (float)o[j]);
        st16(o16 + (size_t)m * ld16o + p.N + n, *reinterpret_cast<uint4*>(&l));
    }
}

__device__ __forceinline__ void finish8(const gl_gemm_args& p, float gate, int m, int n, float (&v)[8]) {
    Fin8Aux a;
    fin8_load(p, m, n, a);
    fin8_store(p, gate, m, n, v, a);
}

}

int gl8_supported(const gl_gemm_args& g, bool conv, int* bn_out);
int gl8_launch(const gl_gemm_args& g, const ConvGeom& cg, bool conv, int bm, int bn, int zs, int kper, int order_m, hipStream_t st, bool s3 = false);
int gl8_init(void);
int gl8_read_stamps(void* dst, int64_t bytes);
uint64_t gl8_kxr_launch_count(void);
```

layoutllm_t2i_amd/csrc/misc.hip:

```cpp
#include "common.h"
#include "gligen_hip.h"
#include "opts.h"

namespace {

template <typename OT>
__global__ __launch_bounds__(256) void posnet_input_kernel(const float* __restrict__ boxes, const float* __restrict__ masks,
                                                           const float* __restrict__ emb, const float* __restrict__ null_pos,
                                                           const float* __restrict__ null_xyxy, int in_dim, int num_freqs,
                                                           OT* __restrict__ out) {
    const int row = blockIdx.x;
    const float m = masks[row];
    const int pos_dim = num_freqs * 8;
    OT* o = out + (size_t)row * (in_dim + pos_dim);
    for (int c = threadIdx.x; c < in_dim; c += 256) {
        const float v = emb[(size_t)row * in_dim + c] * m + (1.0f - m) * null_pos[c];
        o[c] = (OT)v;
    }
    for (int c = threadIdx.x; c < pos_dim; c += 256) {
        const int j = c / 8;
        const int r = c - j * 8;
        const int coord = r & 3;
        const float freq = powf(100.0f, (float)j / (float)num_freqs);
        const float arg = freq * boxes[(size_t)row * 4 + coord];
// ... 423 lines not shown
        latent_blend_kernel<4><<<dim3(ew_blocks(n / 4)), dim3(256), 0, (hipStream_t)stream>>>(x, x0, noise, mask, a, s, B, C, hw, x0_batch, mask_batch);
    else
        latent_blend_kernel<1><<<dim3(ew_blocks(n)), dim3(256), 0, (hipStream_t)stream>>>(x, x0, noise, mask, a, s, B, C, hw, x0_batch, mask_batch);
    GL_CHECK_LAUNCH();
    return 0;
}

extern "C" int gl_vae_posterior(const float* h, const float* w, const float* bias, const float* noise, float scale, int32_t B, int32_t Cin,
                                int32_t E, int32_t hw, float* z, float* mean, void* stream) {
    if (!h || !w || !bias || !noise || !z || B <= 0 || Cin <= 0 || E <= 0 || hw <= 0) return GL_ERR_BAD_ARG;
    vae_posterior_kernel<<<dim3(ew_blocks((size_t)B * hw)), dim3(256), 0, (hipStream_t)stream>>>(h, w, bias, noise, scale, B, Cin, E, hw, z, mean);
    GL_CHECK_LAUNCH();
    return 0;
}

extern "C" int gl_softmax_rows(void* x, int32_t rows, int32_t n, int32_t ld, float scale, void* stream) {
    if (!x || rows <= 0 || n <= 0 || (n % 8) || (ld % 8)) return GL_ERR_BAD_ARG;
    softmax_rows_kernel<<<dim3(rows), dim3(256), 0, (hipStream_t)stream>>>(reinterpret_cast<half_t*>(x), n, ld, scale);
    GL_CHECK_LAUNCH();
    return 0;
}

extern "C" int gl_latent_affine_pack(const float* z, const float* w, const float* bias, float pre, int32_t B, int32_t C,
                                     int32_t hw, int32_t Cpad, void* out, void* stream) {
    if (!z || !w || !bias || !out || B <= 0 || C <= 0 || hw <= 0 || Cpad < C) return GL_ERR_BAD_ARG;
    latent_affine_pack_kernel<<<dim3(ew_blocks((size_t)B * hw * Cpad)), dim3(256), 0, (hipStream_t)stream>>>(
        z, w, bias, pre, B, C, hw, Cpad, reinterpret_cast<half_t*>(out));
    GL_CHECK_LAUNCH();
    return 0;
}

extern "C" int gl_init_gemm(void);
extern "C" int gl_init_ff(void);
extern "C" int gl_init_attn(void);
static gl_opts make_default_opts() {
    gl_opts o{};
    o.v[2] = 0;    o.v[3] = 0;    o.v[4] = 400;  o.v[5] = 300;  o.v[GL_OPT_SPLITK_TILES_CONV] = 450;
    o.v[6] = 16;   o.v[7] = 300;  o.v[8] = 1;    o.v[10] = -1;  o.v[13] = 3;
    o.v[16] = 16;  o.v[17] = 1;   o.v[20] = 0;   o.v[21] = 1;   o.v[23] = 1;
    o.v[24] = 64;  o.v[25] = 1;   o.v[27] = 1;   o.v[29] = 1;   o.v[30] = 1;
    o.v[31] = 200; o.v[32] = 0;   o.v[33] = 0;   o.v[34] = 11;  o.v[35] = 5;
    o.v[37] = 1;
    o.v[41] = 1;
    o.v[42] = 1;
    o.v[43] = 1;
    o.v[38] = 1;
    o.v[44] = 1;
    o.v[45] = 1024;
    o.v[46] = 11;
    o.v[47] = 100;
    o.v[50] = 0;
    o.v[51] = 1;
    o.v[52] = 1;
    o.v[54] = 2;
    return o;
}
gl_opts g_gl_opts = make_default_opts();
thread_local const gl_opts* tl_gl_opts = nullptr;
int g_gl_option_epoch = 0;

bool gl_opts_put(gl_opts& t, int key, int value) {
    switch (key) {
        case 2: case 3: case 4: case 6: case 7: case 8: case 10: case 13: case 17: case 20: case 21: case 23: case 24: case 25:
        case 27: case 29: case 30: case 31: case 32: case 33: case 35: case 37: case 38: case 41: case 42: case 43: case 44: case 45: case 46: case 47: case 50: case 51: case 52: case 53: case 54:
            t.v[key] = value;
            return true;
        case 5:
            t.v[5] = value < 0 ? 300 : value;
            t.v[GL_OPT_SPLITK_TILES_CONV] = value < 0 ? 450 : value;
            return true;
        case 16: t.v[16] = value > 0 ? value : 16; return true;
        case 34: t.v[34] = value < 1 ? 1 : value; return true;
        default: return false;
    }
}

extern "C" int gl_set_option(int key, int value) {
    if (key < 0 || key >= GL_OPT_MAX || !gl_opts_put(g_gl_opts, key, value)) return GL_ERR_BAD_ARG;
    ++g_gl_option_epoch;
    return 0;
}

extern "C" int gl_abi_version(void) { return GL_ABI_VERSION; }
extern "C" int gl_sizeof_gemm_args(void) { return (int)sizeof(gl_gemm_args); }
extern "C" int gl_sizeof_conv_args(void) { return (int)sizeof(gl_conv_args); }
extern "C" int gl_sizeof_attn_args(void) { return (int)sizeof(gl_attn_args); }
extern "C" int gl_sizeof_gn_args(void) { return (int)sizeof(gl_gn_args); }
extern "C" int gl_init(void) {
    int e = gl_init_gemm();
    if (!e) e = gl_init_ff();
    return e ? e : gl_init_attn();
}
```

layoutllm_t2i_amd/csrc/vae_engine.hip:

```cpp
#include "common.h"
#include "gligen_hip.h"
#include "opts.h"

#include <cstring>
#include <map>
#include <string>
#include <tuple>
#include <unordered_map>
#include <vector>

namespace {
constexpr int VCIN_PAD = 64;
constexpr int64_t VALIGN = 256;
struct VW {
    int64_t off, bytes;
    int dtype, ndim;
    int64_t shape[4];
};
}

struct gl_vae {
    gl_vae_config cfg;
    std::vector<std::string> names;
    std::unordered_map<std::string, VW> tab;
    int64_t total = 0;
    const char* wbase = nullptr;
    struct Buf { void* p; size_t bytes; };
    std::unordered_map<std::string, Buf> pool;
    bool pool_changed = false;
    std::map<std::tuple<int, int, int>, hipGraphExec_t> graphs;
    hipStream_t cap_stream = nullptr;
    int launches = 0;
    int opt_epoch = 0;
    int ovr_epoch = 0;
    gl_opt_overrides ovr;
    bool encoder = false;

    void add(const std::string& n, int dtype, std::initializer_list<int64_t> shp) {
        VW w{};
        w.dtype = dtype;
        w.ndim = (int)shp.size();
        int64_t numel = 1;
        int i = 0;
        for (auto s : shp) { w.shape[i++] = s; numel *= s; }
        w.bytes = numel * (dtype == 0 ? 2 : 4);
        w.off = total;
        total += (w.bytes + VALIGN - 1) / VALIGN * VALIGN;
        names.push_back(n);
        tab[n] = w;
    }
    template <typename T>
    const T* W(const std::string& n) const {
        auto it = tab.find(n);
        return it == tab.end() ? nullptr : reinterpret_cast<const T*>(wbase + it->second.off);
    }
    void* get(const std::string& tag, size_t bytes) {
        auto it = pool.find(tag);
        if (it != pool.end() && it->second.bytes >= bytes) return it->second.p;
        void* p = nullptr;
        if (hipMalloc(&p, bytes) != hipSuccess) return nullptr;
        if (it != pool.end()) { (void)hipFree(it->second.p); it->second = Buf{p, bytes}; }
        else pool[tag] = Buf{p, bytes};
        pool_changed = true;
        return p;
    }
    half_t* f16(const std::string& tag, size_t n) { return reinterpret_cast<half_t*>(get(tag, n * 2)); }
    float* f32(const std::string& tag, size_t n) { return reinterpret_cast<float*>(get(tag, n * 4)); }
    void drop_graphs() {
        for (auto& kv : graphs) (void)hipGraphExecDestroy(kv.second);
        graphs.clear();
    }
};


namespace {

#define VCK(x)                    \
    do {                          \
        const int e__ = (x);      \
        if (e__ != 0) return e__; \
    } while (0)
#define VCKP(p) \
    if ((p) == nullptr) return GL_ERR_BAD_ARG

void plan_resnet(gl_vae* v, const std::string& p, int cin, int cout) {
    v->add(p + ".norm1.g", 1, {cin}); v->add(p + ".norm1.b", 1, {cin});
    v->add(p + ".conv1.w", 0, {cout, 9 * (int64_t)cin}); v->add(p + ".conv1.b", 1, {cout});
    v->add(p + ".norm2.g", 1, {cout}); v->add(p + ".norm2.b", 1, {cout});
    v->add(p + ".conv2.w", 0, {cout, 9 * (int64_t)cout}); v->add(p + ".conv2.b", 1, {cout});
    if (cin != cout) { v->add(p + ".nin_shortcut.w", 0, {cout, cin}); v->add(p + ".nin_shortcut.b", 1, {cout}); }
}

std::string lt(int h, int w) { return std::to_string(h) + "x" + std::to_string(w); }

struct VRun {
    gl_vae* v;
    hipStream_t st;
    int B;
    int* launches;
    void count(int n = 1) { if (launches) *launches += n; }
};

int v_gn(VRun& r, const half_t* x, int C, int HW, const std::string& p, bool silu, const std::string& tag, half_t** out) {
    gl_vae* v = r.v;
    const int nchunk = gn_nchunk(HW);
    float* partial = v->f32("gn.partial", (size_t)r.B * nchunk * 64);
    half_t* y = v->f16(tag, (size_t)r.B * HW * C);
    VCKP(partial); VCKP(y);
    VCK(gl_groupnorm(x, C, nullptr, 0, r.B, HW, v->W<float>(p + ".g"), v->W<float>(p + ".b"), 1e-6f, silu ? 1 : 0, y, partial, nchunk, r.st));
    r.count(gl_groupnorm_launches(C, HW));
    *out = y;
    return 0;
}

int v_conv(VRun& r, const half_t* x, int sh, int sw, int cin, const std::string& p, int cout, int up, int epi, const void* res, void* out,
           int out_mode = GL_OUT_F16_ROWMAJOR, int down = 0) {
    gl_vae* v = r.v;
    gl_conv_args a;
    memset(&a, 0, sizeof(a));
    a.in = x;
    a.B = r.B; a.Hin = sh; a.Win = sw; a.Cin = cin;
    a.Hout = up ? 2 * sh : (down ? sh / 2 : sh);
    a.Wout = up ? 2 * sw : (down ? sw / 2 : sw);
    a.stride = down ? 2 : 1; a.upsample2x = up;
    a.g.w = v->W<half_t>(p + ".w");
    a.g.bias = v->W<float>(p + ".b");
    a.g.N = cout;
    a.g.epi = epi;
    a.g.out_mode = out_mode;
    a.g.out = out;
    a.g.ldc = out_mode == GL_OUT_F32_NCHW ? 0 : cout;
    a.g.hw = out_mode == GL_OUT_F32_NCHW ? a.Hout * a.Wout : 0;
    a.g.res = res; a.g.ldres = cout;
    float* ws = v->f32("ws", (size_t)GL_WS_BYTES / 4);
    VCKP(ws);
    a.g.workspace = ws; a.g.workspace_bytes = GL_WS_BYTES;
    VCK(down ? gl_conv3x3_pad01(&a, r.st) : gl_conv3x3(&a, r.st));
    r.count();
    return 0;
}

int v_gemm(VRun& r, const half_t* a_, int lda, const half_t* w, const float* bias, int M, int N, int K, int epi, const void* res, half_t* out,
           int ldc) {
    gl_gemm_args g;
    memset(&g, 0, sizeof(g));
    g.a = a_; g.lda = lda; g.w = w; g.bias = bias; g.M = M; g.N = N; g.K = K; g.epi = epi;
    g.out_mode = GL_OUT_F16_ROWMAJOR; g.out = out; g.ldc = ldc; g.res = res; g.ldres = N;
    float* ws = r.v->f32("ws", (size_t)GL_WS_BYTES / 4);
    VCKP(ws);
    g.workspace = ws; g.workspace_bytes = GL_WS_BYTES;
    VCK(gl_gemm(&g, r.st));
    r.count();
    return 0;
}

int v_resnet(VRun& r, const std::string& p, const half_t* x, int sh, int sw, int cin, int cout, const std::string& tag, half_t** out) {
    gl_vae* v = r.v;
    const int HW = sh * sw;
    const std::string ss = lt(sh, sw);
    const size_t M = (size_t)r.B * HW;
    half_t *t1, *t2;
    VCK(v_gn(r, x, cin, HW, p + ".norm1", true, "rn.gn." + std::to_string(cin) + "." + ss, &t1));
    half_t* h = v->f16("rn.h." + std::to_string(cout) + "." + ss, M * cout);
    VCKP(h);
    VCK(v_conv(r, t1, sh, sw, cin, p + ".conv1", cout, 0, GL_EPI_BIAS, nullptr, h));
    VCK(v_gn(r, h, cout, HW, p + ".norm2", true, "rn.gn." + std::to_string(cout) + "." + ss, &t2));
    const half_t* sk = x;
    if (cin != cout) {
        half_t* s = v->f16("rn.sk." + std::to_string(cout) + "." + ss, M * cout);
        VCKP(s);
        VCK(v_gemm(r, x, cin, v->W<half_t>(p + ".nin_shortcut.w"), v->W<float>(p + ".nin_shortcut.b"), (int)M, cout, cin, GL_EPI_BIAS, nullptr, s, cout));
        sk = s;
    }
    half_t* o = v->f16(tag, M * cout);
    VCKP(o);
    VCK(v_conv(r, t2, sh, sw, cout, p + ".conv2", cout, 0, GL_EPI_RES, sk, o));
    *out = o;
// ... 118 lines not shown
    float* z = v->f32("out.z", (size_t)B * c.embed_dim * hw);
    VCKP(mom); VCKP(noise); VCKP(z);
    VCK(v_conv(r, g, sh, sw, ch, "encoder.conv_out", zc2, 0, GL_EPI_BIAS, nullptr, mom, GL_OUT_F32_NCHW));
    VCK(gl_vae_posterior(mom, v->W<float>("quant_conv.w"), v->W<float>("quant_conv.b"), noise, c.scale_factor, B, zc2, c.embed_dim, hw, z,
                         nullptr, st));
    r.count();
    return 0;
}

template <typename Launch>
int run_plan(gl_vae* v, int B, int sh, int sw, int use_graph, hipStream_t st, Launch launch) {
    if (v->opt_epoch != g_gl_option_epoch || v->ovr_epoch != v->ovr.epoch) {
        v->drop_graphs();
        v->opt_epoch = g_gl_option_epoch;
        v->ovr_epoch = v->ovr.epoch;
    }
    const auto key = std::make_tuple((int)B, (int)sh, (int)sw);
    auto it = v->graphs.find(key);
    if (use_graph && it == v->graphs.end()) {
        VCK(launch(st, &v->launches));
        if (hipStreamSynchronize(st) != hipSuccess) return GL_ERR_BAD_ARG;
        if (v->pool_changed) { v->drop_graphs(); v->pool_changed = false; }
        if (v->cap_stream == nullptr && hipStreamCreateWithFlags(&v->cap_stream, hipStreamNonBlocking) != hipSuccess) return GL_ERR_UNSUPPORTED;
        hipGraph_t graph = nullptr;
        if (hipStreamBeginCapture(v->cap_stream, hipStreamCaptureModeThreadLocal) != hipSuccess) return GL_ERR_UNSUPPORTED;
        const int rc = launch(v->cap_stream, nullptr);
        const hipError_t ec = hipStreamEndCapture(v->cap_stream, &graph);
        if (rc != 0 || ec != hipSuccess || graph == nullptr) {
            if (graph) (void)hipGraphDestroy(graph);
            return rc != 0 ? rc : GL_ERR_UNSUPPORTED;
        }
        hipGraphExec_t exec = nullptr;
        const hipError_t ei = hipGraphInstantiate(&exec, graph, nullptr, nullptr, 0);
        (void)hipGraphDestroy(graph);
        if (ei != hipSuccess) return GL_ERR_UNSUPPORTED;
        v->graphs[key] = exec;
    } else if (use_graph) {
        if (hipGraphLaunch(it->second, st) != hipSuccess) return GL_ERR_BAD_ARG;
    } else {
        VCK(launch(st, &v->launches));
        if (v->pool_changed) { v->drop_graphs(); v->pool_changed = false; }
    }
    return 0;
}

}

extern "C" int gl_vae_create(const gl_vae_config* cfg, gl_vae** out) {
    if (!cfg || !out || cfg->n_mult < 1 || cfg->n_mult > 8 || cfg->ch <= 0 || (cfg->ch % 64) || cfg->num_res_blocks < 0 || cfg->z_channels <= 0 ||
        cfg->z_channels > VCIN_PAD || cfg->out_ch <= 0 || cfg->scale_factor == 0.0f)
        return GL_ERR_BAD_ARG;
    gl_vae* v = new gl_vae();
    v->cfg = *cfg;
    const int nres = cfg->n_mult;
    int ch = cfg->ch * cfg->ch_mult[nres - 1];
    v->add("post_quant_conv.w", 1, {cfg->z_channels, cfg->embed_dim > 0 ? cfg->embed_dim : cfg->z_channels});
    v->add("post_quant_conv.b", 1, {cfg->z_channels});
    v->add("decoder.conv_in.w", 0, {ch, 9 * (int64_t)VCIN_PAD});
    v->add("decoder.conv_in.b", 1, {ch});
    plan_resnet(v, "decoder.mid.block_1", ch, ch);
    const std::string ap = "decoder.mid.attn_1";
    v->add(ap + ".norm.g", 1, {ch}); v->add(ap + ".norm.b", 1, {ch});
    for (const char* n : {"q", "k", "v", "proj_out"}) { v->add(ap + "." + n + ".w", 0, {ch, ch}); v->add(ap + "." + n + ".b", 1, {ch}); }
    plan_resnet(v, "decoder.mid.block_2", ch, ch);
    for (int lvl = nres - 1; lvl >= 0; --lvl) {
        const int cout = cfg->ch * cfg->ch_mult[lvl];
        for (int i = 0; i <= cfg->num_res_blocks; ++i) {
            plan_resnet(v, "decoder.up." + std::to_string(lvl) + ".block." + std::to_string(i), ch, cout);
            ch = cout;
        }
        if (lvl != 0) {
            v->add("decoder.up." + std::to_string(lvl) + ".upsample.conv.w", 0, {ch, 9 * (int64_t)ch});
            v->add("decoder.up." + std::to_string(lvl) + ".upsample.conv.b", 1, {ch});
        }
    }
    v->add("decoder.norm_out.g", 1, {ch}); v->add("decoder.norm_out.b", 1, {ch});
    v->add("decoder.conv_out.w", 0, {cfg->out_ch, 9 * (int64_t)ch});
    v->add("decoder.conv_out.b", 1, {cfg->out_ch});
    *out = v;
    return 0;
}

extern "C" int gl_vae_encoder_create(const gl_vae_config* cfg, gl_vae** out) {
    if (!cfg || !out || cfg->n_mult < 1 || cfg->n_mult > 8 || cfg->ch <= 0 || (cfg->ch % 64) || cfg->num_res_blocks < 0 || cfg->z_channels <= 0 ||
        cfg->out_ch <= 0 || cfg->out_ch > VCIN_PAD || cfg->embed_dim <= 0 || cfg->scale_factor == 0.0f)
        return GL_ERR_BAD_ARG;
    for (int l = 0; l < cfg->n_mult; ++l)
        if (cfg->ch_mult[l] <= 0) return GL_ERR_BAD_ARG;
    gl_vae* v = new gl_vae();
    v->cfg = *cfg;
    v->encoder = true;
    const int nres = cfg->n_mult;
    int ch = cfg->ch;
    v->add("encoder.conv_in.w", 0, {ch, 9 * (int64_t)VCIN_PAD});
    v->add("encoder.conv_in.b", 1, {ch});
    for (int lvl = 0; lvl < nres; ++lvl) {
        const int cout = cfg->ch * cfg->ch_mult[lvl];
        for (int i = 0; i < cfg->num_res_blocks; ++i) {
            plan_resnet(v, "encoder.down." + std::to_string(lvl) + ".block." + std::to_string(i), ch, cout);
            ch = cout;
        }
        if (lvl != nres - 1) {
            v->add("encoder.down." + std::to_string(lvl) + ".downsample.conv.w", 0, {ch, 9 * (int64_t)ch});
            v->add("encoder.down." + std::to_string(lvl) + ".downsample.conv.b", 1, {ch});
        }
    }
    plan_resnet(v, "encoder.mid.block_1", ch, ch);
    const std::string ap = "encoder.mid.attn_1";
    v->add(ap + ".norm.g", 1, {ch}); v->add(ap + ".norm.b", 1, {ch});
    for (const char* n : {"q", "k", "v", "proj_out"}) { v->add(ap + "." + n + ".w", 0, {ch, ch}); v->add(ap + "." + n + ".b", 1, {ch}); }
    plan_resnet(v, "encoder.mid.block_2", ch, ch);
    v->add("encoder.norm_out.g", 1, {ch}); v->add("encoder.norm_out.b", 1, {ch});
    v->add("encoder.conv_out.w", 0, {2 * cfg->z_channels, 9 * (int64_t)ch});
    v->add("encoder.conv_out.b", 1, {2 * cfg->z_channels});
    v->add("quant_conv.w", 1, {2 * cfg->embed_dim, 2 * cfg->z_channels});
    v->add("quant_conv.b", 1, {2 * cfg->embed_dim});
    *out = v;
    return 0;
}

extern "C" int gl_vae_encode(gl_vae* v, const float* x, int32_t B, int32_t side, const float* noise, float* z, int32_t use_graph, void* stream) {
    return gl_vae_encode_hw(v, x, B, side, side, noise, z, use_graph, stream);
}

extern "C" int gl_vae_encode_hw(gl_vae* v, const float* x, int32_t B, int32_t h, int32_t w, const float* noise, float* z, int32_t use_graph,
// ... 91 lines not shown
```

layoutllm_t2i_amd/dist.py:

```python
from __future__ import annotations

import contextlib

from typing import Dict, List, Optional, Tuple

import torch
import torch.distributed as dist

from .arch import UNetConfig, build_plan
from .weights import PackedWeights

_ALIGN = 256


def shard_indices(n_items: int, rank: int, world: int) -> List[int]:
    return list(range(rank, n_items, world))


def flatten_packed(P: PackedWeights) -> Tuple[torch.Tensor, dict]:
    if P.flat is None:
        P.to_flat()
    return P.flat, dict(total=int(P.flat.numel()), has_sd_conv=bool(P.has_sd_conv))


def unflatten_packed(flat: torch.Tensor, manifest: dict, cfg: UNetConfig, device) -> PackedWeights:
    assert manifest["total"] == flat.numel()
    return PackedWeights.from_flat(flat, cfg, device, manifest["has_sd_conv"])


def broadcast_packed(P: Optional[PackedWeights], cfg: UNetConfig, device, src: int = 0) -> PackedWeights:
    rank = dist.get_rank()
    if rank == src:
        flat, manifest = flatten_packed(P)
        box = [manifest]
    else:
        flat, box = None, [None]
    dist.broadcast_object_list(box, src=src)
    manifest = box[0]
    if rank != src:
        flat = torch.empty(manifest["total"], dtype=torch.uint8, device=device)
    dist.broadcast(flat.view(torch.int64) if flat.numel() % 8 == 0 else flat, src=src)
    return unflatten_packed(flat, manifest, cfg, device)


_DT = {"torch.float16": torch.float16, "torch.float32": torch.float32, "torch.int32": torch.int32, "torch.uint8": torch.uint8}


def flatten_tensors(tensors: Dict[str, torch.Tensor], device) -> Tuple[torch.Tensor, list]:
    man, off = [], 0
    for k in sorted(tensors):
        t = tensors[k]
        nb = t.numel() * t.element_size()
        man.append((k, str(t.dtype), tuple(t.shape), off, nb))
        off += (nb + _ALIGN - 1) // _ALIGN * _ALIGN
    flat = torch.zeros(max(off, _ALIGN), dtype=torch.uint8, device=device)
    for k, _, _, o, nb in man:
        if nb:
            flat[o:o + nb].copy_(tensors[k].contiguous().view(-1).view(torch.uint8))
    return flat, man


def unflatten_tensors(flat: torch.Tensor, manifest: list) -> Dict[str, torch.Tensor]:
    out = {}
    for k, dt, shape, o, nb in manifest:
        out[k] = flat[o:o + nb].view(_DT[dt]).view(tuple(shape))
    return out


def broadcast_bundle(P: Optional[PackedWeights], vae_w: Optional[Dict[str, torch.Tensor]], cfg: Optional[UNetConfig], device,
                     src: int = 0, extra: Optional[dict] = None, aux: Optional[Dict[str, Dict[str, torch.Tensor]]] = None,
                     want_aux: bool = False):
    rank = dist.get_rank()
    if rank == src:
        uflat, uman = flatten_packed(P)
        vflat, vman = (flatten_tensors(vae_w, uflat.device) if vae_w is not None else (None, None))
        usz = int(uflat.numel())
        parts = [uflat] + ([vflat] if vflat is not None else [])
        aman = {}
        for name in sorted(aux or {}):
            af, am = flatten_tensors(aux[name], uflat.device)
# ... 40 lines not shown
```

layoutllm_t2i_amd/engine.py:

```python
from __future__ import annotations

import ctypes as C
from typing import Dict, List, Optional, Tuple

import torch

from . import _lib
from ._lib import PlmsStepArgs, check, init_device
from .arch import UNetConfig
from .weights import PackedWeights

F16, F32 = torch.float16, torch.float32


def check_latent_hw(cfg: UNetConfig, h: int, w: int) -> None:
    f = 2 ** (len(cfg.channel_mult) - 1)
    if h <= 0 or w <= 0 or h % f or w % f:
        raise ValueError(f"latent shape {h} x {w}: rows and columns must each be a positive multiple of {f}")


class UNetEngine:
    def __init__(self, packed: PackedWeights):
        if not torch.cuda.is_available():
            raise RuntimeError("UNetEngine needs a GPU: the denoising path has no CPU fallback")
        if packed.flat is None or not packed.flat.is_cuda:
            raise _lib.HipLibraryError("packed weights must be a flat buffer on the GPU (PackedWeights.to_flat on a cuda device)")
        self.P = packed
        self.cfg: UNetConfig = packed.cfg
        self.plan = packed.plan
        self.dev = torch.device(packed.device)
        if self.dev.index is None:
            self.dev = torch.device("cuda", torch.cuda.current_device())
        self.W, self.S = packed.w, packed.s
        init_device(self.dev.index)
        self._lib = _lib.lib()
        self.handle = _lib.create_engine(self.cfg)
        with torch.cuda.device(self.dev):
            check(self._lib.gl_load_weights(self.handle, packed.flat.data_ptr(), packed.flat.numel(), int(packed.has_sd_conv), self._stream()),
                  "gl_load_weights")
        self._pool: Dict[Tuple, torch.Tensor] = {}
        self.cond: Optional[dict] = None
        self._cond_refs: Tuple = ()
        self._extra_ref: Optional[torch.Tensor] = None
        self.use_graphs = True

    def __del__(self):
        h, self.handle = getattr(self, "handle", None), None
        if h:
            try:
                self._lib.gl_destroy(h)
            except Exception:
                pass

    def _stream(self) -> int:
        return torch.cuda.current_stream(self.dev).cuda_stream

    def set_option(self, key: int, value: int) -> None:
        check(self._lib.gl_set_handle_option(self.handle, int(key), int(value)), "gl_set_handle_option")

    def clear_options(self) -> None:
        check(self._lib.gl_clear_handle_options(self.handle), "gl_clear_handle_options")

    def buf(self, tag: str, shape, dtype=F16, zero: bool = False) -> torch.Tensor:
        key = (tag, tuple(shape), dtype)
        t = self._pool.get(key)
        if t is None:
            t = (torch.zeros if zero else torch.empty)(tuple(shape), dtype=dtype, device=self.dev)
            self._pool[key] = t
        return t

    def pool_bytes(self) -> int:
        return int(self._lib.gl_pool_bytes(self.handle)) + sum(t.numel() * t.element_size() for t in self._pool.values())

    def num_launches(self) -> int:
        return int(self._lib.gl_num_launches(self.handle))

    @torch.no_grad()
    def set_conditioning(self, context, relations, boxes, masks, positive_embeddings, hw, text_masks=None, image_masks=None,
                         image_embeddings=None) -> None:
        rel_on = getattr(self.cfg, "relation", True)
        if not rel_on:
            relations = None
        elif relations is None:
            raise ValueError("this model carries the rela_fuse relation chain: it needs relations [Bn, R, ctx] (only a model loaded from a "
                             "checkpoint without rela_fuse, UNetConfig.relation = False, runs without)")
        ti = self.cfg.grounding == "text_image"
        extra = (text_masks, image_masks, image_embeddings)
        if ti and any(v is None for v in extra):
            raise ValueError("a text_image model needs text_masks, image_masks and image_embeddings")
# ... 126 lines not shown
```

layoutllm_t2i_amd/ops.py:

```python
from __future__ import annotations

import ctypes as C
from typing import Optional

import torch

from . import _lib
from ._lib import (EPI_BIAS, EPI_GATE_RES, EPI_GEGLU, EPI_RES, EPI_ROWBIAS, EPI_SILU, OUT_F16_HILO, OUT_F16_ROWMAJOR, OUT_F32_NCHW,
                   OUT_F32_ROWMAJOR, AttnArgs, ConvArgs, GemmArgs, GnArgs, check)

F16 = torch.float16
F32 = torch.float32


_DEV = None


def _stream() -> int:
    dev = _DEV if _DEV is not None else torch.cuda.current_device()
    if dev != torch.cuda.current_device():
        raise _lib.HipLibraryError(f"tensors live on cuda:{dev} but cuda:{torch.cuda.current_device()} is current: wrap the "
                                   "call in torch.cuda.device(...) (kernels launch on the current device)")
    _lib.init_device(dev)
    return torch.cuda.current_stream(dev).cuda_stream
# ... 93 lines not shown
        K //= 2
        g.ldw = 2 * K
    if wsplit == 2:
        if K1 != 2 * K:
            raise ValueError(f"hilo_a: a has {K1} columns, expected 2 x K = {2 * K}")
        g.kwrap = K
        g.a2, g.lda2, g.ksplit = a.data_ptr(), lda, 2 * K
        K = 3 * K
    elif a2 is not None:
        _req(a2, F16, "a2")
        M2, K2, lda2 = _rows(a2, "a2")
        if M2 != M or K1 + K2 != K:
            raise ValueError("a2 shape mismatch")
        g.a2, g.lda2, g.ksplit = a2.data_ptr(), lda2, K1
    elif hilo_a:
        if K1 != 2 * K:
            raise ValueError(f"hilo_a: a has {K1} columns, expected 2 x K = {2 * K}")
        g.kwrap = K
        if not wsplit:
            g.ldw = K
        K = 2 * K
    elif K1 != K:
        raise ValueError(f"a has K={K1}, w has K={K}")
    g.w = w.data_ptr()
    g.M, g.N, g.K = M, N, K
    _fill_epilogue(g, epi, out, N // 2 if epi == EPI_GEGLU else N, bias, res, gate, rowbias, rows_per_sample, nchw_hw, out16, hilo_out)
    if vt is not None:
        _req(vt, F16, "vt")
        if vt.dim() != 4 or not vt.is_contiguous():
            raise ValueError("vt must be a contiguous [B, H, d, ldvt] tensor")
        g.vt, g.vt_col0, g.vt_rows = vt.data_ptr(), vt_col0, vt_rows
        g.vt_H, g.vt_d, g.vt_ld = vt.shape[1], vt.shape[2], vt.shape[3]
        if vt_lo is not None:
            _req(vt_lo, F16, "vt_lo")
            if tuple(vt_lo.shape) != tuple(vt.shape) or not vt_lo.is_contiguous():
                raise ValueError("vt_lo must have vt's shape")
            g.vt_lo = vt_lo.data_ptr()
    check(_lib.lib().gl_gemm(C.byref(g), _stream()), "gl_gemm")
    return out


def conv3x3(x: torch.Tensor, w: torch.Tensor, out: torch.Tensor, B: int, Hin: int, Win: int, bias=None,
            stride: int = 1, upsample2x: bool = False, epi: int = EPI_BIAS, res=None, rowbias=None,
            rows_per_sample: int = 0, nchw_hw: int = 0, n_valid: Optional[int] = None, out16=None, in_split: int = 0,
            w_split: bool = False, pad01: bool = False) -> torch.Tensor:
    _req(x, F16, "x")
    _req(w, F16, "w")
    rows, Cin, ldx = _rows(x, "x")
    if ldx != Cin or rows != B * Hin * Win:
        raise ValueError("x must be a contiguous [B*Hin*Win, Cin] matrix")
    if in_split:
        Cin //= 2
    N, K, _ = _rows(w, "w")
    if K != (18 if w_split else 9) * Cin:
        raise ValueError("w must be [Cout, 9*Cin] ([Cout, 18*Cin] with w_split)")
    if upsample2x:
        Hout, Wout = 2 * Hin, 2 * Win
    elif pad01:
        Hout, Wout = Hin // 2, Win // 2
    else:
        Hout, Wout = (Hin + 2 - 3) // stride + 1, (Win + 2 - 3) // stride + 1
    a = ConvArgs()
    a.inp = x.data_ptr()
    a.B, a.Hin, a.Win, a.Cin, a.Hout, a.Wout = B, Hin, Win, Cin, Hout, Wout
    a.stride, a.upsample2x = stride, int(upsample2x)
    a.in_split, a.w_split = int(in_split), int(bool(w_split))
    a.g.w = w.data_ptr()
    a.g.N = N if n_valid is None else n_valid
    _fill_epilogue(a.g, epi, out, a.g.N, bias, res, None, rowbias, rows_per_sample, nchw_hw, out16)
    if pad01:
        check(_lib.lib().gl_conv3x3_pad01(C.byref(a), _stream()), "gl_conv3x3_pad01")
    else:
        check(_lib.lib().gl_conv3x3(C.byref(a), _stream()), "gl_conv3x3")
    return out


def conv3x3_pad01(x: torch.Tensor, w: torch.Tensor, out: torch.Tensor, B: int, Hin: int, Win: int, bias=None, **kw) -> torch.Tensor:
    return conv3x3(x, w, out, B, Hin, Win, bias, stride=2, pad01=True, **kw)


def vt_ld(Nk: int) -> int:
    n = (Nk + 63) // 64 * 64
    return n + 64 if n % 512 == 0 else n


def transpose_v(v: torch.Tensor, v_bstride: int, ldv: int, vt: torch.Tensor, B: int, H: int, d: int, Nk: int):
    _req(v, F16, "v", 2)
    _req(vt, F16, "vt")
    ldvt = vt.shape[-1]
    check(_lib.lib().gl_transpose_v(v.data_ptr(), v_bstride, ldv, vt.data_ptr(), ldvt, B, H, d, Nk, _stream()),
          "gl_transpose_v")
    return vt


def attention(q: torch.Tensor, q_bstride: int, ldq: int, k: torch.Tensor, k_bstride: int, ldk: int, vt: torch.Tensor,
              out: torch.Tensor, o_bstride: int, ldo: int, B: int, H: int, d: int, Nq: int, Nk: int, scale: float,
              q_prescaled: bool = False, q_lo=None, k_lo=None, vt_lo=None, out_lo=None):
    _req(q, F16, "q")
    _req(k, F16, "k")
    _req(vt, F16, "vt")
    _req(out, F16, "out", 8)
    a = AttnArgs()
    a.q, a.q_bstride, a.ldq = q.data_ptr(), q_bstride, ldq
    a.k, a.k_bstride, a.ldk = k.data_ptr(), k_bstride, ldk
    a.vt, a.ldvt = vt.data_ptr(), vt.shape[-1]
    a.out, a.o_bstride, a.ldo = out.data_ptr(), o_bstride, ldo
    a.B, a.H, a.d, a.Nq, a.Nk = B, H, d, Nq, Nk
    a.scale = scale
    a.q_prescaled = int(q_prescaled)
    for t_, n_ in ((q_lo, "q_lo"), (k_lo, "k_lo"), (vt_lo, "vt_lo"), (out_lo, "out_lo")):
        if t_ is not None:
            _req(t_, F16, n_, 8)
    a.q_lo, a.k_lo, a.vt_lo, a.out_lo = _ptr(q_lo), _ptr(k_lo), _ptr(vt_lo), _ptr(out_lo)
    check(_lib.lib().gl_attention(C.byref(a), _stream()), "gl_attention")
    return out


def gn_nchunk(HW: int) -> int:
# ... 294 lines not shown
        _req(mean, F32, "mean", 4)
    check(_lib.lib().gl_vae_posterior(h.data_ptr(), w.data_ptr(), bias.data_ptr(), noise.data_ptr(), float(scale), B, Cin, E, hh * ww,
                                      z.data_ptr(), _ptr(mean), _stream()), "gl_vae_posterior")
    return z


def latent_blend(x: torch.Tensor, x0: torch.Tensor, noise: torch.Tensor, mask: torch.Tensor, a: float, s: float) -> torch.Tensor:
    for t, n in ((x, "x"), (x0, "x0"), (noise, "noise"), (mask, "mask")):
        _req(t, F32, n, 4)
    B, Cc, hh, ww = x.shape
    if x0.shape[1:] != x.shape[1:] or noise.shape != x0.shape or x0.shape[0] not in (1, B) or \
            tuple(mask.shape[1:]) != (1, hh, ww) or mask.shape[0] not in (1, B):
        raise ValueError("latent_blend: x0 / noise [1|B, C, h, w], mask [1|B, 1, h, w]")
    check(_lib.lib().gl_latent_blend(x.data_ptr(), x0.data_ptr(), noise.data_ptr(), mask.data_ptr(), float(a), float(s), B, Cc, hh * ww,
                                     x0.shape[0], mask.shape[0], _stream()), "gl_latent_blend")
    return x


def softmax_rows(x: torch.Tensor, scale: float = 1.0) -> torch.Tensor:
    _req(x, F16, "x")
    rows, n, ld = _rows(x, "x")
    check(_lib.lib().gl_softmax_rows(x.data_ptr(), rows, n, ld, scale, _stream()), "gl_softmax_rows")
    return x


def latent_affine_pack(z: torch.Tensor, w: torch.Tensor, bias: torch.Tensor, pre: float, Cpad: int, out: torch.Tensor):
    for t, n in ((z, "z"), (w, "w"), (bias, "bias")):
        _req(t, F32, n, 4)
    _req(out, F16, "out")
    B, Cc, h, ww = z.shape
    check(_lib.lib().gl_latent_affine_pack(z.data_ptr(), w.data_ptr(), bias.data_ptr(), pre, B, Cc, h * ww, Cpad,
                                           out.data_ptr(), _stream()), "gl_latent_affine_pack")
    return out


def set_option(key: int, value: int) -> None:
    check(_lib.lib().gl_set_option(key, value), "gl_set_option")


def gemm8_launch_count() -> int:
    import ctypes
    n = ctypes.c_uint64(0)
    check(_lib.lib().gl_debug_read(9, ctypes.byref(n), 8), "gl_debug_read")
    return int(n.value)


def kxreuse_launch_count() -> int:
    import ctypes
    n = ctypes.c_uint64(0)
    check(_lib.lib().gl_debug_read(11, ctypes.byref(n), 8), "gl_debug_read")
    return int(n.value)


ATTN_FORMS = ("split_pipe", "split_8w", "split_4w_dbuf", "split_4w_single", "f16_8w_pre0", "f16_8w_pre1", "f16_8w_pre2", "f16_4w_pre0",
              "f16_4w_pre1", "f16_4w_pre2")


def attention_launch_counts() -> dict:
    import ctypes
    n = (ctypes.c_uint64 * len(ATTN_FORMS))()
    check(_lib.lib().gl_debug_read(10, ctypes.byref(n), ctypes.sizeof(n)), "gl_debug_read")
    return {k: int(v) for k, v in zip(ATTN_FORMS, n)}


def clip_patchify(pixel_values: torch.Tensor, patch: int, Kpad: int, out: torch.Tensor) -> torch.Tensor:
    _req(pixel_values, F32, "pixel_values")
    _req(out, F16, "out")
    B, c3, S, S2 = pixel_values.shape
    if c3 != 3 or S != S2 or not pixel_values.is_contiguous():
        raise ValueError("pixel_values must be a contiguous [B, 3, S, S] tensor")
    check(_lib.lib().gl_clip_patchify(pixel_values.data_ptr(), B, S, patch, Kpad, out.data_ptr(), _stream()), "gl_clip_patchify")
    return out


def clip_assemble(patch_emb: torch.Tensor, class_emb: torch.Tensor, pos_emb: torch.Tensor, B: int, T: int, x: torch.Tensor,
                  ln_gamma: Optional[torch.Tensor] = None, ln_beta: Optional[torch.Tensor] = None, eps: float = 1e-5) -> torch.Tensor:
    _req(patch_emb, F16, "patch_emb")
    for t, n in ((class_emb, "class_emb"), (pos_emb, "pos_emb"), (x, "x")):
        _req(t, F32, n)
    C_ = x.shape[-1]
    check(_lib.lib().gl_clip_assemble(patch_emb.data_ptr(), _rows(patch_emb, "patch_emb")[2], class_emb.data_ptr(), pos_emb.data_ptr(), B, T, C_,
                                      _ptr(ln_gamma), _ptr(ln_beta), eps, x.data_ptr(), _stream()), "gl_clip_assemble")
    return x


def clip_embed_tokens(ids: torch.Tensor, tok_emb: torch.Tensor, pos_emb: torch.Tensor, x: torch.Tensor) -> torch.Tensor:
    _req(ids, torch.int32, "ids", 4)
    for t, n in ((tok_emb, "tok_emb"), (pos_emb, "pos_emb"), (x, "x")):
        _req(t, F32, n)
    B, T = ids.shape
    check(_lib.lib().gl_clip_embed_tokens(ids.data_ptr(), tok_emb.data_ptr(), pos_emb.data_ptr(), B, T, x.shape[-1], tok_emb.shape[0],
                                          x.data_ptr(), _stream()), "gl_clip_embed_tokens")
    return x


def clip_gather_rows(x: torch.Tensor, rows: torch.Tensor, out: torch.Tensor) -> torch.Tensor:
    _req(x, F32, "x")
    _req(rows, torch.int32, "rows", 4)
    _req(out, F32, "out")
    check(_lib.lib().gl_clip_gather_rows(x.data_ptr(), _rows(x, "x")[2], rows.data_ptr(), rows.numel(), x.shape[-1], out.data_ptr(), _stream()),
          "gl_clip_gather_rows")
    return out


def attention_small(q: torch.Tensor, k: torch.Tensor, v: torch.Tensor, ld: int, B: int, T: int, H: int, d: int, scale: float,
                    causal: bool, out: torch.Tensor) -> torch.Tensor:
# ... 58 lines not shown
```

layoutllm_t2i_amd/vae.py:

```python
from __future__ import annotations

from typing import Dict, Mapping, Optional, Tuple

import torch

from . import ops
from ._lib import EPI_BIAS, EPI_RES, init_device
from .arch import VAEConfig, vae_decoder_param_shapes, vae_encoder_param_shapes
from .weights import CIN_PAD, _h, _t, pack_conv3x3

F16, F32 = torch.float16, torch.float32
_FP32_1X1 = ("post_quant_conv", "quant_conv")


def _pack_kind(p: str, shp: Tuple[int, ...]) -> str:
    if len(shp) == 1:
        return "norm"
    if shp[2] == 3:
        return "conv3x3"
    return "f32_1x1" if p in _FP32_1X1 else "gemm"


def packed_shapes(param_shapes: Mapping[str, Tuple[int, ...]]) -> Dict[str, Tuple[Tuple[int, ...], torch.dtype]]:
    out: Dict[str, Tuple[Tuple[int, ...], torch.dtype]] = {}
    for name, shp in param_shapes.items():
        if not name.endswith(".weight"):
            continue
        p, kind = name[:-7], _pack_kind(name[:-7], shp)
        if kind == "norm":
            out[p + ".g"], out[p + ".b"] = ((shp[0],), F32), ((shp[0],), F32)
            continue
        if kind == "conv3x3":
            out[p + ".w"] = ((shp[0], 9 * (CIN_PAD if shp[1] < 64 else shp[1])), F16)
        else:
            out[p + ".w"] = ((shp[0], shp[1]), F32 if kind == "f32_1x1" else F16)
        out[p + ".b"] = ((shp[0],), F32)
    return out


def _pack(state_dict: Mapping[str, object], need: Mapping[str, Tuple[int, ...]], device) -> Dict[str, torch.Tensor]:
    g = lambda k: _t(state_dict[k], device)
    W: Dict[str, torch.Tensor] = {}
    for name, shp in need.items():
        if not name.endswith(".weight"):
            continue
        p = name[:-7]
        w = g(name)
        b = g(p + ".bias")
        kind = _pack_kind(p, shp)
        if kind == "norm":
            W[p + ".g"], W[p + ".b"] = w.contiguous(), b.contiguous()
        elif kind == "conv3x3":
            W[p + ".w"] = pack_conv3x3(w, CIN_PAD if shp[1] < 64 else None)
            W[p + ".b"] = b.contiguous()
        elif kind == "f32_1x1":
            W[p + ".w"], W[p + ".b"] = w.reshape(shp[0], shp[1]).contiguous(), b.contiguous()
        else:
            w2, b2 = w.reshape(shp[0], shp[1]), b
            if p.endswith("attn_1.q"):
                s = float(shp[0]) ** -0.5
                w2, b2 = w2 * s, b2 * s
            W[p + ".w"], W[p + ".b"] = _h(w2), b2.contiguous()
    return W


def encoder_unsupported(state_dict: Mapping[str, object], cfg: VAEConfig):
    attn = sorted(k for k in state_dict if k.startswith("encoder.down.") and ".attn." in k)
    if attn:
        return f"the VAE encoder has down-level attention ({attn[0]}); only attn_resolutions = [] is implemented"
    w = state_dict.get("encoder.conv_in.weight")
    if w is not None and tuple(w.shape)[1] != cfg.out_ch:
        return f"the VAE encoder takes {tuple(w.shape)[1]} input channels, the decoder emits out_ch = {cfg.out_ch}"
    return None


class _VAEStage:
    _encoder_stage = False

    def _bind_engine(self):
        from . import _lib
        self.handle = _lib.create_vae(self.cfg, encoder=self._encoder_stage)
        table, total = _lib.vae_weight_table(self.handle)
        flat = torch.zeros(total, dtype=torch.uint8, device=self.device)
        views = {}
        for name, off, nbytes, dtype, shape in table:
            td = F16 if dtype == 0 else F32
            dst = flat[off:off + nbytes].view(td).view(shape)
            src = self.W[name]
            if tuple(src.shape) != tuple(shape) or src.dtype != td:
                raise ValueError(f"{name}: packed {tuple(src.shape)} {src.dtype} != engine table {shape} {td}")
            dst.copy_(src)
            views[name] = dst
        extra = set(self.W) - set(views)
        if extra:
            raise KeyError(f"packer produced tensors the VAE engine does not know: {sorted(extra)[:3]}")
        self.W, self.flat = views, flat
        with torch.cuda.device(self.device):
            _lib.check(_lib.lib().gl_vae_load_weights(self.handle, flat.data_ptr(), flat.numel(), torch.cuda.current_stream(self.device).cuda_stream),
                       "gl_vae_load_weights")
        self.use_graphs = True

    def set_option(self, key: int, value: int) -> None:
        from . import _lib
        _lib.check(_lib.lib().gl_vae_set_option(self.handle, int(key), int(value)), "gl_vae_set_option")

    def __del__(self):
        h, self.handle = getattr(self, "handle", None), None
        if h:
            try:
                from . import _lib
                _lib.lib().gl_vae_destroy(h)
            except Exception:
                pass

    def buf(self, tag, shape, dtype=F16):
        key = (tag, tuple(shape), dtype)
        t = self._pool.get(key)
        if t is None:
            t = torch.empty(tuple(shape), dtype=dtype, device=self.device)
            self._pool[key] = t
        return t

    def _gn(self, x, B, HW, p, silu, tag):
        C = x.shape[-1]
        nchunk = ops.gn_nchunk(HW)
        partial = self.buf("gn.partial", (B * nchunk * 64,), F32)
        return ops.groupnorm(x, None, B, HW, self.W[p + ".g"], self.W[p + ".b"], 1e-6, silu, self.buf(tag, (B * HW, C)), partial)

    def _resnet(self, p, x, B, sh, sw, cin, cout, tag):
        W, HW, side = self.W, sh * sw, f"{sh}x{sw}"
        t = self._gn(x, B, HW, p + ".norm1", True, f"rn.gn.{cin}.{side}")
        h = ops.conv3x3(t, W[p + ".conv1.w"], self.buf(f"rn.h.{cout}.{side}", (B * HW, cout)), B, sh, sw, W[p + ".conv1.b"])
        t2 = self._gn(h, B, HW, p + ".norm2", True, f"rn.gn.{cout}.{side}")
        if cin != cout:
            sk = ops.gemm(x, W[p + ".nin_shortcut.w"], self.buf(f"rn.sk.{cout}.{side}", (B * HW, cout)), W[p + ".nin_shortcut.b"])
        else:
            sk = x
        return ops.conv3x3(t2, W[p + ".conv2.w"], self.buf(tag, (B * HW, cout)), B, sh, sw, W[p + ".conv2.b"],
                           epi=EPI_RES, res=sk)

    def _attn(self, p, x, B, N, C, tag):
        W = self.W
        M = B * N
        hn = self._gn(x, B, N, p + ".norm", False, "at.gn")
        q = ops.gemm(hn, W[p + ".q.w"], self.buf("at.q", (M, C)), W[p + ".q.b"])
        k = ops.gemm(hn, W[p + ".k.w"], self.buf("at.k", (M, C)), W[p + ".k.b"])
        v = ops.gemm(hn, W[p + ".v.w"], self.buf("at.v", (M, C)), W[p + ".v.b"])
        Np = (N + 63) // 64 * 64
        Hs = 4
        vt = self.buf("at.vt", (B, Hs, C // Hs, Np))
        ops.transpose_v(v, N * C, C, vt, B, Hs, C // Hs, N)
        vt2 = vt.view(B, C, Np)
        s = self.buf("at.s", (B, N, Np))
        if Np != N:
            s.zero_()
        o = self.buf("at.o", (M, C))
        for b in range(B):
            sb = s[b][:, :N]
            ops.gemm(q[b * N:(b + 1) * N], k[b * N:(b + 1) * N], sb)
            ops.softmax_rows(sb, 1.0)
            ops.gemm(s[b], vt2[b], o[b * N:(b + 1) * N])
        return ops.gemm(o, W[p + ".proj_out.w"], self.buf(tag, (M, C)), W[p + ".proj_out.b"], EPI_RES, res=x)


class VAEDecoder(_VAEStage):
    def __init__(self, state_dict: Mapping[str, object], cfg: VAEConfig = VAEConfig(), device="cuda:0"):
        if not torch.cuda.is_available():
            raise RuntimeError("VAEDecoder needs a GPU: there is no CPU fallback")
        init_device()
        self.cfg, self.device = cfg, torch.device(device)
        self.scale_factor = cfg.scale_factor
        need = vae_decoder_param_shapes(cfg)
        missing = [k for k in need if k not in state_dict]
        if missing:
            raise KeyError(f"autoencoder state_dict is missing {len(missing)} decoder tensors, e.g. {missing[:3]}")
        self.W = _pack(state_dict, need, self.device)
        self._pool: Dict[tuple, torch.Tensor] = {}
        self._bind_engine()
        enc_missing = [k for k in vae_encoder_param_shapes(cfg) if k not in state_dict]
        self.encoder = VAEEncoder(state_dict, cfg, device) if not enc_missing else None
        self._no_encoder = (f"this autoencoder has no encode stage: its state_dict lacks {len(enc_missing)} encoder tensors, "
                            f"e.g. {enc_missing[:3]}") if enc_missing else None

    @classmethod
    def from_packed(cls, W: Mapping[str, torch.Tensor], cfg: VAEConfig, device="cuda:0") -> "VAEDecoder":
        if not torch.cuda.is_available():
            raise RuntimeError("VAEDecoder needs a GPU: there is no CPU fallback")
        init_device()
        self = cls.__new__(cls)
        self.cfg, self.device, self.scale_factor = cfg, torch.device(device), cfg.scale_factor
        self.W = {k: v.to(self.device) for k, v in W.items()}
        self._pool = {}
        self._bind_engine()
        self.encoder = None
        self._no_encoder = ("this decoder was built from packed decoder weights: the encoder tensors (encoder.*, quant_conv.*) are "
                            "not part of the packed bundle")
        return self

    def encode(self, x: torch.Tensor, noise=None) -> torch.Tensor:
        if self.encoder is None:
            raise RuntimeError(self._no_encoder)
        return self.encoder.encode(x, noise)

    @torch.no_grad()
    def decode(self, z: torch.Tensor) -> torch.Tensor:
        from . import _lib
        cfg = self.cfg
        z = z.to(self.device, F32).contiguous()
        B, zc, sh, sw = z.shape
        assert zc == cfg.z_channels
        f = 2 ** (len(cfg.ch_mult) - 1)
        out = torch.empty(B, cfg.out_ch, f * sh, f * sw, dtype=F32, device=self.device)
        st = torch.cuda.current_stream(self.device).cuda_stream
        with torch.cuda.device(self.device):
            if sh == sw:
                _lib.check(_lib.lib().gl_vae_decode(self.handle, z.data_ptr(), B, sh, out.data_ptr(), int(self.use_graphs), st), "gl_vae_decode")
            else:
                _lib.check(_lib.lib().gl_vae_decode_hw(self.handle, z.data_ptr(), B, sh, sw, out.data_ptr(), int(self.use_graphs), st),
                           "gl_vae_decode_hw")
        return out

    @torch.no_grad()
    def decode_oplevel(self, z: torch.Tensor) -> torch.Tensor:
        cfg, W = self.cfg, self.W
        z = z.to(self.device, F32).contiguous()
        B, zc, sh, sw = z.shape
        assert zc == cfg.z_channels
        nres = len(cfg.ch_mult)
        ch = cfg.ch * cfg.ch_mult[nres - 1]
        xin = ops.latent_affine_pack(z, W["post_quant_conv.w"], W["post_quant_conv.b"], 1.0 / cfg.scale_factor, CIN_PAD,
                                     self.buf("in", (B * sh * sw, CIN_PAD)))
        h = ops.conv3x3(xin, W["decoder.conv_in.w"], self.buf("conv_in", (B * sh * sw, ch)), B, sh, sw, W["decoder.conv_in.b"])
        h = self._resnet("decoder.mid.block_1", h, B, sh, sw, ch, ch, "mid.1")
        h = self._attn("decoder.mid.attn_1", h, B, sh * sw, ch, "mid.a")
        h = self._resnet("decoder.mid.block_2", h, B, sh, sw, ch, ch, "mid.2")
        for lvl in reversed(range(nres)):
            cout = cfg.ch * cfg.ch_mult[lvl]
            for i in range(cfg.num_res_blocks + 1):
                h = self._resnet(f"decoder.up.{lvl}.block.{i}", h, B, sh, sw, ch, cout, f"up.{lvl}.{i}")
                ch = cout
            if lvl != 0:
                p = f"decoder.up.{lvl}.upsample.conv"
                h = ops.conv3x3(h, W[p + ".w"], self.buf(f"up.{lvl}.u", (B * 4 * sh * sw, ch)), B, sh, sw, W[p + ".b"],
                                upsample2x=True)
# ... 96 lines not shown
```

layoutllm_t2i_amd/weights.py:

```python
from __future__ import annotations

import math
from typing import Dict, Mapping

import numpy as np
import torch

from .arch import Plan, UNetConfig, build_plan, param_shapes

CIN_PAD = 64
LOG2E = 1.4426950408889634


def q_fold(d_head: int) -> float:
    return float(d_head) ** -0.5 * LOG2E


def _t(v, device) -> torch.Tensor:
    if not torch.is_tensor(v):
        v = torch.from_numpy(np.ascontiguousarray(np.asarray(v, dtype=np.float32)))
    return v.to(device=device, dtype=torch.float32)


def _h(x: torch.Tensor) -> torch.Tensor:
    return x.to(torch.float16).contiguous()


def pack_conv3x3(w: torch.Tensor, cin_pad: int | None = None) -> torch.Tensor:
    cout, cin = w.shape[0], w.shape[1]
    if cin_pad is not None and cin_pad > cin:
        z = torch.zeros(cout, cin_pad - cin, 3, 3, dtype=w.dtype, device=w.device)
        w = torch.cat([w, z], dim=1)
        cin = cin_pad
    assert cin % 64 == 0, "conv input channels must be a multiple of 64 (pad the first conv)"
    wp = w.reshape(cout, cin // 64, 64, 3, 3).permute(0, 1, 3, 4, 2)
    return _h(wp.reshape(cout, -1))


def pack_first_conv(w: torch.Tensor, cin_pad: int) -> torch.Tensor:
    w = w.float()
    if 3 * w.shape[1] > cin_pad:
        return pack_conv3x3(w, cin_pad)
    hi = w.half().float()
    lo = (w - hi).half().float()
    return pack_conv3x3(torch.cat([hi, hi, lo], dim=1), cin_pad)


def geglu_interleave(t: torch.Tensor) -> torch.Tensor:
    half = t.shape[0] // 2
    assert half % 32 == 0, "GEGLU inner dim must be a multiple of 32"
    x = t[:half].reshape(half // 32, 1, 32, *t.shape[1:])
    g = t[half:].reshape(half // 32, 1, 32, *t.shape[1:])
    return torch.cat([x, g], dim=1).reshape(t.shape)


class PackedWeights:

    def __init__(self, cfg: UNetConfig, plan: Plan, device):
        self.cfg, self.plan, self.device = cfg, plan, device
        self.w: Dict[str, torch.Tensor] = {}
        self.s: Dict[str, float] = {}
        self.emb_offsets: Dict[str, int] = {}
        self.emb_total = 0
        self.flat: torch.Tensor | None = None
        self.has_sd_conv = False

    def nbytes(self) -> int:
        return int(self.flat.numel()) if self.flat is not None else sum(t.numel() * t.element_size() for t in self.w.values())

    def to_flat(self) -> "PackedWeights":
        from . import _lib
        handle = _lib.create_engine(self.cfg)
        try:
            table, total = _lib.weight_table(handle)
        finally:
            _lib.check(_lib.lib().gl_destroy(handle), "gl_destroy")
        flat = torch.zeros(total, dtype=torch.uint8, device=self.device)
        self.has_sd_conv = "sd_first_conv.w" in self.w
        views: Dict[str, torch.Tensor] = {}
        for name, off, nbytes, dtype, shape in table:
            td = torch.float16 if dtype == 0 else torch.float32
            dst = flat[off:off + nbytes].view(td).view(shape)
            if name in self.w:
                src = self.w[name]
                if tuple(src.shape) != tuple(shape) or src.dtype != td:
                    raise ValueError(f"{name}: packed {tuple(src.shape)} {src.dtype} != engine table {shape} {td}")
                dst.copy_(src)
            elif name in self.s:
                dst.fill_(float(self.s[name]))
                self.s[name] = float(dst.item())
            elif name.startswith("sd_first_conv."):
                pass
            else:
                raise KeyError(f"engine weight table wants {name}, which the packer did not produce")
            views[name] = dst
        extra = set(self.w) - set(views)
        if extra:
            raise KeyError(f"packer produced tensors the engine does not know: {sorted(extra)[:3]}")
        self.w, self.flat = views, flat
        return self

    @staticmethod
    def from_flat(flat: torch.Tensor, cfg: UNetConfig, device, has_sd_conv: bool) -> "PackedWeights":
        from . import _lib
        P = PackedWeights(cfg, build_plan(cfg), device)
        handle = _lib.create_engine(cfg)
        try:
            table, total = _lib.weight_table(handle)
        finally:
            _lib.check(_lib.lib().gl_destroy(handle), "gl_destroy")
        if flat.numel() != total:
            raise ValueError(f"flat buffer has {flat.numel()} bytes, the engine table needs {total}")
        for name, off, nbytes, dtype, shape in table:
            td = torch.float16 if dtype == 0 else torch.float32
            v = flat[off:off + nbytes].view(td).view(shape)
            if name.endswith((".tanh_attn", ".tanh_dense")):
                P.s[name] = float(v.item())
            P.w[name] = v
        off = 0
        for l in P.plan.all_layers():
            if l.kind == "res":
                P.emb_offsets[l.prefix] = off
                off += l.cout
        P.emb_total = off
        P.flat, P.has_sd_conv = flat, has_sd_conv
        return P


def pack_state_dict(sd: Mapping[str, object], cfg: UNetConfig, device, sd_first_conv: Mapping[str, object] | None = None
                    ) -> PackedWeights:
    plan = build_plan(cfg)
    need = param_shapes(cfg)
    missing = [k for k in need if k not in sd]
    if missing:
        raise KeyError(f"state_dict is missing {len(missing)} tensors, e.g. {missing[:3]}")
    for k, shp in need.items():
        if tuple(sd[k].shape) != tuple(shp):
            raise ValueError(f"{k}: shape {tuple(sd[k].shape)} != expected {shp}")
    if sd_first_conv is not None and getattr(cfg, "inpaint_mode", False):
        raise ValueError("an inpaint_mode model has no SD first conv (its first conv is not restorable, openaimodel.py:296)")
    P = PackedWeights(cfg, plan, device)
    W, S = P.w, P.s
    g = lambda k: _t(sd[k], device)
    split_all = bool(getattr(cfg, "split_weights", False))

    def mat(w32: torch.Tensor) -> torch.Tensor:
        w32 = w32.reshape(w32.shape[0], -1).float()
        hi = _h(w32)
        if not split_all:
            return hi
        return torch.cat([hi, _h(w32 - hi.float())], 1).contiguous()

    def lin(p, dst=None, bias=True):
        dst = dst or p
        W[dst + ".w"] = mat(g(p + ".weight"))
        if bias:
            W[dst + ".b"] = g(p + ".bias").contiguous()

    def lin_split(p):
        w32 = g(p + ".weight").reshape(g(p + ".weight").shape[0], -1).float()
        hi = _h(w32)
        lo = _h(w32 - hi.float())
        W[p + ".w"] = torch.cat([hi, lo], 1).contiguous()
        W[p + ".b"] = g(p + ".bias").contiguous()

    def norm(p):
        W[p + ".g"] = g(p + ".weight").contiguous()
        W[p + ".b"] = g(p + ".bias").contiguous()

    def conv3(p, cin_pad=None):
        w32 = g(p + ".weight").float()
        hi = pack_conv3x3(w32, cin_pad)
        if split_all:
            lo = pack_conv3x3(w32 - w32.half().float(), cin_pad)
            hi = torch.cat([hi, lo], 1).contiguous()
        W[p + ".w"] = hi
        W[p + ".b"] = g(p + ".bias").contiguous()

    def ff(p):
        W[p + ".ff1.w"] = mat(geglu_interleave(g(p + ".net.0.proj.weight")))
        W[p + ".ff1.b"] = geglu_interleave(g(p + ".net.0.proj.bias")).contiguous()
        lin(p + ".net.2", p + ".ff2")

    def self_attn(p, d):
        W[p + ".qkv.w"] = mat(torch.cat([g(p + ".to_q.weight") * q_fold(d), g(p + ".to_k.weight"), g(p + ".to_v.weight")], 0))
        lin(p + ".to_out.0", p + ".o")

    def cross_attn(p, d):
        W[p + ".q.w"] = mat(g(p + ".to_q.weight") * q_fold(d))
        W[p + ".kv.w"] = mat(torch.cat([g(p + ".to_k.weight"), g(p + ".to_v.weight")], 0))
        lin(p + ".to_out.0", p + ".o")

    lin("time_embed.0")
    lin("time_embed.2")
    W["input_blocks.0.0.w"] = pack_first_conv(g("input_blocks.0.0.weight"), CIN_PAD)
    W["input_blocks.0.0.b"] = g("input_blocks.0.0.bias").contiguous()
    if sd_first_conv is not None:
        W["sd_first_conv.w"] = pack_first_conv(_t(sd_first_conv["weight"], device), CIN_PAD)
        W["sd_first_conv.b"] = _t(sd_first_conv["bias"], device).contiguous()

    emb_w, emb_b, off = [], [], 0
    for l in plan.all_layers():
        p = l.prefix
        if l.kind in ("down", "up"):
            conv3(p)
        elif l.kind == "res":
            norm(p + ".in_layers.0")
            conv3(p + ".in_layers.2")
            norm(p + ".out_layers.0")
            conv3(p + ".out_layers.3")
            if l.cin != l.cout:
                lin_split(p + ".skip_connection")
            emb_w.append(g(p + ".emb_layers.1.weight"))
            emb_b.append(g(p + ".emb_layers.1.bias"))
            P.emb_offsets[p] = off
            off += l.cout
        elif l.kind == "st":
            norm(p + ".norm")
            lin_split(p + ".proj_in")
            lin_split(p + ".proj_out")
            t = p + ".transformer_blocks.0"
            self_attn(t + ".attn1", l.d_head)
            cross_attn(t + ".attn2", l.d_head)
            ff(t + ".ff")
            for n in ("norm1", "norm2", "norm3"):
                norm(f"{t}.{n}")
            f = t + ".fuser"
            lin(f + ".linear")
            self_attn(f + ".attn", l.d_head)
            ff(f + ".ff")
            norm(f + ".norm1")
            norm(f + ".norm2")
            S[f + ".tanh_attn"] = math.tanh(float(g(f + ".alpha_attn")))
            S[f + ".tanh_dense"] = math.tanh(float(g(f + ".alpha_dense")))
            if not getattr(cfg, "relation", True):
                continue
            r = t + ".rela_fuse"
            cross_attn(r + ".attn", l.d_head)
            ff(r + ".ff")
            for n in ("norm1", "norm2", "norm3"):
                norm(f"{r}.{n}")
            S[r + ".tanh_attn"] = math.tanh(float(g(r + ".alpha_attn")))
            S[r + ".tanh_dense"] = math.tanh(float(g(r + ".alpha_dense")))
    W["emb_all.w"] = mat(torch.cat(emb_w, 0))
    W["emb_all.b"] = torch.cat(emb_b, 0).contiguous()
    P.emb_total = off
    norm("out.0")
    conv3("out.2")
    if cfg.grounding == "text_image":
        W["position_net.null_text"] = g("position_net.null_text_feature").contiguous()
        W["position_net.null_image"] = g("position_net.null_image_feature").contiguous()
        W["position_net.null_xyxy"] = g("position_net.null_position_feature").contiguous()
        for chain in ("linears_text", "linears_image"):
            for i in (0, 2, 4):
                lin(f"position_net.{chain}.{i}")
        return P.to_flat()
    W["position_net.null_pos"] = g("position_net.null_positive_feature").contiguous()
# ... 52 lines not shown
```

Baseline: 5.027 images/s.

## Fold nearest-2x upsample into parity-decomposed 2x2 convolutions

Nearest-neighbour 2x upsampling followed by a 3x3 conv is replaced by four 2x2 convolutions, one per output pixel parity, applied to the low-resolution input. The weights are pre-summed at pack time. A new gemm8 kernel variant (UPF) maps each parity to a slice of M tiles and scatters results to interleaved output rows. This cuts the reduction length per output from 9·Cin to 4·Cin and avoids reading the upsampled image. In exchange it adds a new kernel path, a strided scatter epilogue and an option-gated weight layout that must match between packing and the engine, in both the UNet and the VAE decoder.

Result: faster. 5.136 images/s (median of 6 runs) (+2.2%).

```diff
diff --git a/include/gligen_hip.h b/include/gligen_hip.h
--- a/include/gligen_hip.h
+++ b/include/gligen_hip.h
@@ -289,6 +289,7 @@
 int gl_sizeof_attn_args(void);
 int gl_sizeof_gn_args(void);
 int gl_set_option(int key, int value);
+int gl_get_option(int key);
 int gl_set_handle_option(gl_engine* e, int key, int value);
 int gl_clear_handle_options(gl_engine* e);
 int gl_vae_set_option(gl_vae* v, int key, int value);
diff --git a/layoutllm_t2i_amd/_lib.py b/layoutllm_t2i_amd/_lib.py
--- a/layoutllm_t2i_amd/_lib.py
+++ b/layoutllm_t2i_amd/_lib.py
@@ -193,6 +193,7 @@
     "gl_resample_h_u8": (i32, [vp, i32, i32, i32, vp, vp, i32, i32, vp, vp]),
     "gl_resample_v_norm": (i32, [vp, i32, i32, i32, vp, vp, i32, i32, i32, i32, i32, i32, vp, vp, vp, vp, vp]),
     "gl_set_option": (i32, [i32, i32]),
+    "gl_get_option": (i32, [i32]),
     "gl_set_handle_option": (i32, [vp, i32, i32]),
     "gl_clear_handle_options": (i32, [vp]),
     "gl_vae_set_option": (i32, [vp, i32, i32]),
@@ -290,14 +291,49 @@
     return c
 
 
-def create_engine(cfg) -> int:
+OPT_FOLD_UP = 55
+
+
+def fold_up_option() -> int:
+    return int(lib().gl_get_option(OPT_FOLD_UP))
+
+
+def fold_up_default() -> bool:
+    return fold_up_option() == 1
+
+
+def resolve_fold_up(fold_up, rule: bool) -> bool:
+    if fold_up is not None:
+        return bool(fold_up)
+    v = fold_up_option()
+    return bool(rule) if v == 2 else v == 1
+
+
+class _fold_up_scope:
+
+    def __init__(self, fold_up):
+        self.want = None if fold_up is None else int(bool(fold_up))
+
+    def __enter__(self):
+        self.old = lib().gl_get_option(OPT_FOLD_UP)
+        self.changed = self.want is not None and self.want != self.old
+        if self.changed:
+            check(lib().gl_set_option(OPT_FOLD_UP, self.want), "gl_set_option")
+
+    def __exit__(self, *exc):
+        if self.changed:
+            check(lib().gl_set_option(OPT_FOLD_UP, self.old), "gl_set_option")
+
+
+def create_engine(cfg, fold_up=None) -> int:
     h = vp()
     cc = unet_config_c(cfg)
-    check(lib().gl_create(C.byref(cc), C.byref(h)), "gl_create")
+    with _fold_up_scope(fold_up):
+        check(lib().gl_create(C.byref(cc), C.byref(h)), "gl_create")
     return h.value
 
 
-def create_vae(cfg, encoder: bool = False) -> int:
+def create_vae(cfg, encoder: bool = False, fold_up=None) -> int:
     cc = VaeConfigC()
     cc.ch, cc.n_mult, cc.num_res_blocks, cc.z_channels, cc.out_ch = cfg.ch, len(cfg.ch_mult), cfg.num_res_blocks, cfg.z_channels, cfg.out_ch
     for i, m in enumerate(cfg.ch_mult):
@@ -307,7 +343,8 @@
     if encoder:
         check(lib().gl_vae_encoder_create(C.byref(cc), C.byref(h)), "gl_vae_encoder_create")
     else:
-        check(lib().gl_vae_create(C.byref(cc), C.byref(h)), "gl_vae_create")
+        with _fold_up_scope(fold_up):
+            check(lib().gl_vae_create(C.byref(cc), C.byref(h)), "gl_vae_create")
     return h.value
 
 
diff --git a/layoutllm_t2i_amd/csrc/engine.hip b/layoutllm_t2i_amd/csrc/engine.hip
--- a/layoutllm_t2i_amd/csrc/engine.hip
+++ b/layoutllm_t2i_amd/csrc/engine.hip
@@ -115,6 +115,7 @@
 }
 
 struct gl_engine {
+    bool fold_up = false;
     bool strict_hoists_ok = false;
     int strict_hoists_w3 = -1;
     gl_unet_config cfg;
@@ -293,7 +294,10 @@
     int off = 0;
     for_all_layers(e, [&](LayerD& l) {
         const std::string& p = l.prefix;
-        if (l.kind == DOWN || l.kind == UP) {
+        if (l.kind == UP && e->fold_up) {
+            add_w(e, p + ".w", 0, {4 * (int64_t)l.cout, 4 * (int64_t)l.cin});
+            add_w(e, p + ".b", 1, {l.cout});
+        } else if (l.kind == DOWN || l.kind == UP) {
             add_conv3(e, p, l.cin, l.cout);
         } else if (l.kind == RES) {
             add_norm(e, p + ".in_layers.0", l.cin);
@@ -457,8 +461,9 @@
         a.in = in.p; a.B = B; a.Hin = Hin; a.Win = Win; a.Cin = Cin;
         a.Hout = o.ups ? 2 * Hin : (Hin + 2 - 3) / o.stride + 1;
         a.Wout = o.ups ? 2 * Win : (Win + 2 - 3) / o.stride + 1;
-        a.stride = o.stride; a.upsample2x = o.ups;
-        a.g.w = e->W(p + ".w"); a.g.bias = e->Wf(p + ".b"); a.g.N = (int)wi->shape[0];
+        const bool folded = o.ups && wi->shape[1] == 4 * (int64_t)Cin;
+        a.stride = o.stride; a.upsample2x = folded ? 2 : o.ups;
+        a.g.w = e->W(p + ".w"); a.g.bias = e->Wf(p + ".b"); a.g.N = (int)(folded ? wi->shape[0] / 4 : wi->shape[0]);
         a.g.epi = o.epi; a.g.out_mode = out_mode; a.g.out = out; a.g.ldc = a.g.N; a.g.hw = o.nchw_hw;
         a.g.res = o.res.p; a.g.ldres = o.res.ld; a.g.res_f32 = o.res.f32;
         a.g.rowbias = o.rowbias.p; a.g.ld_rowbias = o.rowbias.ld; a.g.rows_per_sample = o.rowbias.rows_per_sample;
@@ -992,6 +997,7 @@
     if ((cfg->inpaint_mode != 0 && cfg->inpaint_mode != 1) || first_conv_in(*cfg) > CIN_PAD) return GL_ERR_UNSUPPORTED;
     gl_engine* e = new gl_engine();
     e->cfg = *cfg;
+    e->fold_up = gl_opt(55) == 1 && !cfg->split_weights;
     build_plan(e);
     build_table(e);
     *out = e;
diff --git a/layoutllm_t2i_amd/csrc/gemm8.hip b/layoutllm_t2i_amd/csrc/gemm8.hip
--- a/layoutllm_t2i_amd/csrc/gemm8.hip
+++ b/layoutllm_t2i_amd/csrc/gemm8.hip
@@ -65,7 +65,7 @@
 
 __device__ unsigned long long g8_stamps[4 * 4096];
 
-template <int BM, int BN, bool CONV, int DBG = 0, bool S3 = false, bool KXR = false>
+template <int BM, int BN, bool CONV, int DBG = 0, bool S3 = false, bool KXR = false, bool UPF = false>
 __global__ __launch_bounds__(512, 2) void gemm8_kernel(gl_gemm_args p, ConvGeom cg, int splitk, int kt_per_split, int order_flags) {
     using C = G8<BM, BN>;
     constexpr int KT = S3 ? 32 : 64;
@@ -91,11 +91,17 @@
         const int xcd = bid & 7, local = bid >> 3;
         tile = (xcd < r ? xcd * (q + 1) : r * (q + 1) + (xcd - r) * q) + local;
     }
-    const int mt_ = (M + C::BM - 1) / C::BM;
+    static_assert(!UPF || (CONV && !S3 && !KXR), "folded upsample conv: plain fp16 conv loop");
+    const int Ms = UPF ? cg.B * cg.Hin * cg.Win : 0;
+    const int mtp = UPF ? (Ms + C::BM - 1) / C::BM : 0;
+    const int mt_ = UPF ? 4 * mtp : (M + C::BM - 1) / C::BM;
+    const int Mrows = UPF ? Ms : M;
     const int order_m = order_flags & 1;
-    const bool tap_major = CONV && (order_flags & 2);
+    const bool tap_major = CONV && !UPF && (order_flags & 2);
     const int tmi = order_m ? tile % mt_ : tile / nt;
-    const int m0 = tmi * C::BM;
+    const int par = UPF ? tmi / mtp : 0;
+    const int py = par >> 1, px = par & 1;
+    const int m0 = (UPF ? tmi - par * mtp : tmi) * C::BM;
     const int n0 = (order_m ? tile / mt_ : tile - tmi * nt) * BN;
     const int kt_begin = blockIdx.z * kt_per_split;
     const int kt_end = min(K / KT, kt_begin + kt_per_split);
@@ -125,9 +131,28 @@
         const int r = trow0 + srow;
         const int gc = chunk_off(sslot ^ ((r >> 1) & 7), a_lo);
         const int m = m0 + r;
-        const bool rowok = m < M;
+        const bool rowok = m < Mrows;
         aptr[u] = zsrc; cmask[u] = 0u;
-        if constexpr (CONV) {
+        if constexpr (UPF) {
+            if (rowok) {
+                const int hw = cg.Hin * cg.Win;
+                int y, x;
+                if (((cg.Win & (cg.Win - 1)) | (hw & (hw - 1))) == 0) {
+                    const int rr = m & (hw - 1);
+                    y = rr >> __builtin_ctz(cg.Win);
+                    x = rr & (cg.Win - 1);
+                } else {
+                    const int rr = m % hw;
+                    y = rr / cg.Win;
+                    x = rr - y * cg.Win;
+                }
+                const int y0 = y + py - 1, x0 = x + px - 1;
+                const unsigned rb = (y0 >= 0 ? 1u : 0u) | (y0 + 1 < cg.Hin ? 2u : 0u);
+                const unsigned cb = (x0 >= 0 ? 1u : 0u) | (x0 + 1 < cg.Win ? 2u : 0u);
+                cmask[u] = ((rb & 1u) ? cb : 0u) | ((rb & 2u) ? (cb << 2) : 0u);
+                aptr[u] = cg.in + (size_t)m * cg.Cin + gc;
+            }
+        } else if constexpr (CONV) {
             if (rowok) {
                 int b, oy, ox;
                 const int hw = cg.Hout * cg.Wout;
@@ -170,12 +195,12 @@
         const int gc = chunk_off(sslot ^ ((r >> 1) & 7), p.kwrap);
         const int n = n0 + r;
         const bool ok = (j < nb) && (r < BN) && (n < N);
-        bptr[j] = ok ? (Wg + (size_t)n * p.ldw + gc) : zsrc;
+        bptr[j] = ok ? (Wg + (size_t)(UPF ? par * N + n : n) * p.ldw + gc) : zsrc;
         if (ok) bmask |= 1u << j;
     }
 
-    const int ncblk = CONV ? K / 576 : 1;
-    const int in_lim = tap_major ? ncblk : 9;
+    const int ncblk = UPF ? K / 256 : (CONV ? K / 576 : 1);
+    const int in_lim = UPF ? 4 : (tap_major ? ncblk : 9);
     int is_out = 0, is_in = 0;
     int is_cblk = 0, is_tap = 0;
     if constexpr (CONV) {
@@ -199,6 +224,11 @@
             is_boff = ((is_cblk * 9 + is_tap) << 6) + ((is_kt & 1) << 5);
         } else if constexpr (S3) {
             is_boff = is_kt << 5;
+        } else if constexpr (UPF) {
+            is_tap = is_in;
+            is_cblk = is_out;
+            is_off = ((py - 1 + (is_tap >> 1)) * cg.Win + (px - 1 + (is_tap & 1))) * cg.Cin + (is_cblk << 6);
+            is_boff = (is_cblk * 4 + is_tap) << 6;
         } else if constexpr (CONV) {
             is_tap = tap_major ? is_out : is_in;
             is_cblk = tap_major ? is_in : is_out;
@@ -227,7 +257,7 @@
             const int u = i;
             if constexpr (CONV) {
                 int off = is_off;
-                if (cg.ups) {
+                if (!UPF && cg.ups) {
                     const int ry = (is_ky - 1 + (int)((cmask[u] >> 9) & 1u)) >> 1, rx = (is_kx - 1 + (int)((cmask[u] >> 10) & 1u)) >> 1;
                     off = (ry * cg.Win + rx) * cg.Cin + (is_acb << (S3 ? 5 : 6));
                 }
@@ -625,6 +655,18 @@
     constexpr int NQ = ITEMS / 64;
     const bool vt_wave = p.vt != nullptr && nbase >= p.vt_col0;
     const bool generic = splitk == 1 && !vt_wave && epi != GL_EPI_GEGLU;
+    auto orow = [&](const int m) __attribute__((always_inline)) -> int {
+        if constexpr (UPF) {
+            const int hw = cg.Hin * cg.Win;
+            const int b = m / hw;
+            const int rr = m - b * hw;
+            const int y = rr / cg.Win;
+            const int x = rr - y * cg.Win;
+            return (b * cg.Hout + 2 * y + py) * cg.Wout + 2 * x + px;
+        } else {
+            return m;
+        }
+    };
     Fin8Aux aux[MH][NQ];
     if (generic) {
 #pragma unroll
@@ -634,7 +676,7 @@
                 const int idx = lane + 64 * q;
                 const int r = idx / CG8, c = (idx - r * CG8) * 8;
                 const int m = m0 + (BM / 4) * wm + 32 * h + r, n = nbase + c;
-                if (m < M && n < N) fin8_load(p, m, n, aux[h][q]);
+                if (m < Mrows && n < N) fin8_load(p, orow(m), n, aux[h][q]);
             }
     }
     float vt_bias[2] = {0.0f, 0.0f};
@@ -677,8 +719,8 @@
                 const int idx = lane + 64 * q;
                 const int r = idx / CG8, c = (idx - r * CG8) * 8;
                 const int m = mbase + r, n = nbase + c;
-                if (m < M && n < N) {
-                    float* o = ws + (size_t)m * N + n;
+                if (m < Mrows && n < N) {
+                    float* o = ws + (size_t)orow(m) * N + n;
                     *reinterpret_cast<float4*>(o) = *reinterpret_cast<const float4*>(stage + r * EPS + c);
                     *reinterpret_cast<float4*>(o + 4) = *reinterpret_cast<const float4*>(stage + r * EPS + c + 4);
                 }
@@ -764,11 +806,11 @@
                 const int idx = lane + 64 * q;
                 const int r = idx / CG8, c = (idx - r * CG8) * 8;
                 const int m = mbase + r, n = nbase + c;
-                if (m < M && n < N) {
+                if (m < Mrows && n < N) {
                     const float4 a0 = *reinterpret_cast<const float4*>(stage + r * EPS + c);
                     const float4 a1 = *reinterpret_cast<const float4*>(stage + r * EPS + c + 4);
                     float v[8] = {a0.x, a0.y, a0.z, a0.w, a1.x, a1.y, a1.z, a1.w};
-                    fin8_store(p, gate, m, n, v, aux[h][q]);
+                    fin8_store(p, gate, orow(m), n, v, aux[h][q]);
                 }
             }
         }
@@ -787,6 +829,7 @@
 #define g8_kxr gl_opt(54)
 
 std::atomic<uint64_t> g8_kxr_launches{0};
+std::atomic<uint64_t> g8_upf_launches{0};
 
 static bool kxr_default(const gl_gemm_args&, const ConvGeom&, int , int ) { return true; }
 
@@ -803,6 +846,17 @@
     const int mt = gl_cdiv(g.M, BM), nt = gl_cdiv(g.N, BN);
     dim3 grid(mt * nt, 1, zs);
     bool done = false;
+    if (cg.ups == 2) {
+        if constexpr (CONV && !S3) {
+            grid.x = 4 * gl_cdiv(cg.B * cg.Hin * cg.Win, BM) * nt;
+            gemm8_kernel<BM, BN, true, 0, false, false, true><<<grid, dim3(512), G8<BM, BN>::LDS, st>>>(g, cg, zs, kper, order_m);
+            GL_CHECK_LAUNCH();
+            g8_upf_launches.fetch_add(1, std::memory_order_relaxed);
+            return 0;
+        } else {
+            return GL_ERR_UNSUPPORTED;
+        }
+    }
     if constexpr (CONV && !S3 && BM == 256) {
         const bool eligible = cg.stride == 1 && !cg.ups && cg.shift == 0 && g.kwrap == 0 && cg.cwrap == 0 && !(order_m & 2) && kper > 0 &&
                               (kper % 9) == 0 && cg.Hin == cg.Hout && cg.Win == cg.Wout && g.K == 9 * cg.Cin && g.a2 == nullptr;
@@ -839,6 +893,9 @@
 int set_attr8() {
     hipError_t e = hipFuncSetAttribute((const void*)gemm8_kernel<BM, BN, CONV>, hipFuncAttributeMaxDynamicSharedMemorySize, G8<BM, BN>::LDS);
     if (e == hipSuccess) e = hipFuncSetAttribute((const void*)gemm8_kernel<BM, BN, CONV, 0, true>, hipFuncAttributeMaxDynamicSharedMemorySize, G8<BM, BN>::LDS);
+    if constexpr (CONV) {
+        if (e == hipSuccess) e = hipFuncSetAttribute((const void*)gemm8_kernel<BM, BN, true, 0, false, false, true>, hipFuncAttributeMaxDynamicSharedMemorySize, G8<BM, BN>::LDS);
+    }
     if constexpr (CONV && BM == 256) {
         if (e == hipSuccess) e = hipFuncSetAttribute((const void*)gemm8_kernel<BM, BN, true, 0, false, true>, hipFuncAttributeMaxDynamicSharedMemorySize, G8X<BN>::LDS);
         if constexpr (BN == 160) {
@@ -855,9 +912,9 @@
 
 }
 
-int gl8_supported(const gl_gemm_args& g, bool conv, int* bn_out) {
+int gl8_supported(const gl_gemm_args& g, bool conv, int* bn_out, bool upfold) {
     if (g.out_mode == GL_OUT_F32_NCHW) return 0;
-    if ((g.K % 64) != 0 || (g.N % 8) != 0 || g.M < 256) return 0;
+    if ((g.K % 64) != 0 || (g.N % 8) != 0 || (g.M < 256 && !upfold)) return 0;
     int bn = 128;
     if (g.epi != GL_EPI_GEGLU && (g.N % 160) == 0) bn = 160;
     if (g.vt != nullptr && (g.vt_col0 % (bn / 2)) != 0) {
@@ -900,6 +957,7 @@
 }
 
 uint64_t gl8_kxr_launch_count(void) { return g8_kxr_launches.load(std::memory_order_relaxed); }
+uint64_t gl8_upf_launch_count(void) { return g8_upf_launches.load(std::memory_order_relaxed); }
 
 int gl8_read_stamps(void* dst, int64_t bytes) {
     if (bytes > (int64_t)sizeof(unsigned long long) * 4 * 4096) return GL_ERR_BAD_ARG;
diff --git a/layoutllm_t2i_amd/csrc/gemm_conv.hip b/layoutllm_t2i_amd/csrc/gemm_conv.hip
--- a/layoutllm_t2i_amd/csrc/gemm_conv.hip
+++ b/layoutllm_t2i_amd/csrc/gemm_conv.hip
@@ -683,9 +683,11 @@
         int bn_ = 0;
         if (!g_opt_g8 || !gl8_supported(g, CONV, &bn_)) return GL_ERR_UNSUPPORTED;
     }
-    if (g_opt_g8) {
+    const bool upf = CONV && cg.ups == 2;
+    auto mtiles = [&](const int bm_) { return upf ? 4 * gl_cdiv(g.M / 4, bm_) : gl_cdiv(g.M, bm_); };
+    if (g_opt_g8 || upf) {
         int bn = 0;
-        if (gl8_supported(g, CONV, &bn)) {
+        if (gl8_supported(g, CONV, &bn, upf)) {
             const int nk = g.K / 64;
             auto plan_split = [&](const int tiles_) {
                 int sk = 1;
@@ -698,13 +700,13 @@
                 return sk;
             };
             int bm = 256;
-            int tiles = gl_cdiv(g.M, 256) * gl_cdiv(g.N, bn);
+            int tiles = mtiles(256) * gl_cdiv(g.N, bn);
             int splitk = plan_split(tiles);
             if (tiles * 2 <= 256 && g.epi != GL_EPI_GEGLU && g.vt == nullptr) {
                 const bool want = CONV ? ((g_opt_g8_bm128 & 4) || ((g_opt_g8_bm128 & 1) && nk / splitk <= 16)) : ((g_opt_g8_bm128 & 2) != 0);
                 if (want) {
                     bm = 128;
-                    tiles = gl_cdiv(g.M, 128) * gl_cdiv(g.N, bn);
+                    tiles = mtiles(128) * gl_cdiv(g.N, bn);
                     splitk = plan_split(tiles);
                 }
             }
@@ -723,7 +725,7 @@
                 const bool full_rounds = g_opt_g8_shortk && blocks * 5 >= ((blocks + 255) / 256) * 256 * 4;
                 enough = nk >= 16 || blocks <= 256 || (g.epi == GL_EPI_GEGLU && (nk >= 10 || full_rounds)) || (full_rounds && blocks <= 2048);
             }
-            if (g_opt_g8 == 2 || enough || need8) {
+            if (g_opt_g8 == 2 || enough || need8 || upf) {
                 const bool s3 = g_opt_g8_s3 != 0 && g.kwrap != 0 && g.K == 3 * g.kwrap &&
                                 (CONV ? cg.cwrap != 0 : (g.a2 == g.a && g.lda2 == g.lda && g.ksplit == 2 * g.kwrap));
                 const int nks = s3 ? g.kwrap / 32 : nk;
@@ -732,7 +734,7 @@
                 const int order_m = g_opt_order == 1 ? ((CONV ? 9L : 1L) * g.N > (long)g.M) : (g_opt_order == 2);
                 const int e = gl8_launch(g, cg, CONV, bm, bn, zs, kper, order_m | (CONV && g_opt_g8_tapmajor ? 2 : 0), st, s3);
                 if (e) return e;
-                g8_launches.fetch_add(1, std::memory_order_relaxed);
+                if (!upf) g8_launches.fetch_add(1, std::memory_order_relaxed);
                 if (zs > 1) {
                     const size_t total = (size_t)g.M * (g.N / 8);
                     int nblk = (int)((total + 255) / 256);
@@ -744,6 +746,7 @@
             }
         }
     }
+    if (upf) return GL_ERR_UNSUPPORTED;
     if constexpr (!CONV) {
         if (g_opt_geglu32 && g.epi == GL_EPI_GEGLU && g.K <= 640 && g.a2 == nullptr) return dispatch_shape<false, 32>(g, cg, st);
     }
@@ -767,7 +770,12 @@
     if (!a || !a->in || !a->g.w || !a->g.out) return GL_ERR_BAD_ARG;
     if ((a->Cin % 64) != 0) return GL_ERR_BAD_ARG;
     if (a->stride != 1 && a->stride != 2) return GL_ERR_BAD_ARG;
+    if (a->upsample2x < 0 || a->upsample2x > 2) return GL_ERR_BAD_ARG;
     if (a->upsample2x && (a->stride != 1 || a->Hout != 2 * a->Hin || a->Wout != 2 * a->Win)) return GL_ERR_BAD_ARG;
+    const bool upf = a->upsample2x == 2;
+    if (upf && (shift != 0 || a->in_split != 0 || a->w_split != 0 || a->g.out_mode == GL_OUT_F32_NCHW || a->g.out_mode == GL_OUT_F16_HILO ||
+                a->g.epi == GL_EPI_GEGLU || a->g.vt != nullptr || a->g.vt_lo != nullptr))
+        return GL_ERR_BAD_ARG;
     if (a->B >= 2048 || a->Hout >= 1024 || a->Wout >= 1024) return GL_ERR_BAD_ARG;
     if (a->in_split != 0 && a->in_split != 2 && a->in_split != 3) return GL_ERR_BAD_ARG;
     if (a->in_split == 3 && !a->w_split) return GL_ERR_BAD_ARG;
@@ -778,6 +786,7 @@
     g.K = 9 * a->Cin * (a->in_split ? a->in_split : 1);
     g.ldw = 9 * a->Cin * (a->w_split ? 2 : 1);
     g.kwrap = a->in_split ? 9 * a->Cin : 0;
+    if (upf) g.K = g.ldw = 4 * a->Cin;
     ConvGeom cg{reinterpret_cast<const half_t*>(a->in), a->B, a->Hin, a->Win, a->Cin * (a->in_split ? 2 : 1), a->Hout, a->Wout, a->stride,
                 a->upsample2x, nullptr, a->in_split == 3 ? 2 * (a->Cin >> 6) : 0, shift};
     return dispatch<true>(g, cg, (hipStream_t)stream);
@@ -826,9 +835,9 @@
 extern "C" int gl_debug_read(int what, void* dst, int64_t bytes) {
     if (what == 8) return gl8_read_stamps(dst, bytes);
     if (what == 10) return gl_attn_read_launch_counts(dst, bytes);
-    if (what == 9 || what == 11) {
+    if (what == 9 || what == 11 || what == 12) {
         if (!dst || bytes < (int64_t)sizeof(uint64_t)) return GL_ERR_BAD_ARG;
-        const uint64_t n = what == 9 ? g8_launches.load(std::memory_order_relaxed) : gl8_kxr_launch_count();
+        const uint64_t n = what == 9 ? g8_launches.load(std::memory_order_relaxed) : (what == 11 ? gl8_kxr_launch_count() : gl8_upf_launch_count());
         memcpy(dst, &n, sizeof n);
         return 0;
     }
diff --git a/layoutllm_t2i_amd/csrc/gemm_shared.h b/layoutllm_t2i_amd/csrc/gemm_shared.h
--- a/layoutllm_t2i_amd/csrc/gemm_shared.h
+++ b/layoutllm_t2i_amd/csrc/gemm_shared.h
@@ -114,8 +114,9 @@
 
 }
 
-int gl8_supported(const gl_gemm_args& g, bool conv, int* bn_out);
+int gl8_supported(const gl_gemm_args& g, bool conv, int* bn_out, bool upfold = false);
 int gl8_launch(const gl_gemm_args& g, const ConvGeom& cg, bool conv, int bm, int bn, int zs, int kper, int order_m, hipStream_t st, bool s3 = false);
 int gl8_init(void);
 int gl8_read_stamps(void* dst, int64_t bytes);
 uint64_t gl8_kxr_launch_count(void);
+uint64_t gl8_upf_launch_count(void);
diff --git a/layoutllm_t2i_amd/csrc/misc.hip b/layoutllm_t2i_amd/csrc/misc.hip
--- a/layoutllm_t2i_amd/csrc/misc.hip
+++ b/layoutllm_t2i_amd/csrc/misc.hip
@@ -499,6 +499,7 @@
     o.v[50] = 0;
     o.v[51] = 1;
     o.v[52] = 1;
+    o.v[55] = 2;
     o.v[54] = 2;
     return o;
 }
@@ -509,7 +510,7 @@
 bool gl_opts_put(gl_opts& t, int key, int value) {
     switch (key) {
         case 2: case 3: case 4: case 6: case 7: case 8: case 10: case 13: case 17: case 20: case 21: case 23: case 24: case 25:
-        case 27: case 29: case 30: case 31: case 32: case 33: case 35: case 37: case 38: case 41: case 42: case 43: case 44: case 45: case 46: case 47: case 50: case 51: case 52: case 53: case 54:
+        case 27: case 29: case 30: case 31: case 32: case 33: case 35: case 37: case 38: case 41: case 42: case 43: case 44: case 45: case 46: case 47: case 50: case 51: case 52: case 53: case 54: case 55:
             t.v[key] = value;
             return true;
         case 5:
@@ -522,6 +523,11 @@
     }
 }
 
+extern "C" int gl_get_option(int key) {
+    if (key < 0 || key >= GL_OPT_MAX) return GL_ERR_BAD_ARG;
+    return g_gl_opts.v[key];
+}
+
 extern "C" int gl_set_option(int key, int value) {
     if (key < 0 || key >= GL_OPT_MAX || !gl_opts_put(g_gl_opts, key, value)) return GL_ERR_BAD_ARG;
     ++g_gl_option_epoch;
diff --git a/layoutllm_t2i_amd/csrc/vae_engine.hip b/layoutllm_t2i_amd/csrc/vae_engine.hip
--- a/layoutllm_t2i_amd/csrc/vae_engine.hip
+++ b/layoutllm_t2i_amd/csrc/vae_engine.hip
@@ -34,6 +34,7 @@
     int opt_epoch = 0;
     int ovr_epoch = 0;
     gl_opt_overrides ovr;
+    bool fold_up = false;
     bool encoder = false;
 
     void add(const std::string& n, int dtype, std::initializer_list<int64_t> shp) {
@@ -122,7 +123,7 @@
     a.B = r.B; a.Hin = sh; a.Win = sw; a.Cin = cin;
     a.Hout = up ? 2 * sh : (down ? sh / 2 : sh);
     a.Wout = up ? 2 * sw : (down ? sw / 2 : sw);
-    a.stride = down ? 2 : 1; a.upsample2x = up;
+    a.stride = down ? 2 : 1; a.upsample2x = up ? (v->fold_up ? 2 : 1) : 0;
     a.g.w = v->W<half_t>(p + ".w");
     a.g.bias = v->W<float>(p + ".b");
     a.g.N = cout;
@@ -347,6 +348,7 @@
         return GL_ERR_BAD_ARG;
     gl_vae* v = new gl_vae();
     v->cfg = *cfg;
+    v->fold_up = gl_opt(55) == 1;
     const int nres = cfg->n_mult;
     int ch = cfg->ch * cfg->ch_mult[nres - 1];
     v->add("post_quant_conv.w", 1, {cfg->z_channels, cfg->embed_dim > 0 ? cfg->embed_dim : cfg->z_channels});
@@ -365,7 +367,8 @@
             ch = cout;
         }
         if (lvl != 0) {
-            v->add("decoder.up." + std::to_string(lvl) + ".upsample.conv.w", 0, {ch, 9 * (int64_t)ch});
+            if (v->fold_up) v->add("decoder.up." + std::to_string(lvl) + ".upsample.conv.w", 0, {4 * (int64_t)ch, 4 * (int64_t)ch});
+            else v->add("decoder.up." + std::to_string(lvl) + ".upsample.conv.w", 0, {ch, 9 * (int64_t)ch});
             v->add("decoder.up." + std::to_string(lvl) + ".upsample.conv.b", 1, {ch});
         }
     }
diff --git a/layoutllm_t2i_amd/dist.py b/layoutllm_t2i_amd/dist.py
--- a/layoutllm_t2i_amd/dist.py
+++ b/layoutllm_t2i_amd/dist.py
@@ -20,12 +20,12 @@
 def flatten_packed(P: PackedWeights) -> Tuple[torch.Tensor, dict]:
     if P.flat is None:
         P.to_flat()
-    return P.flat, dict(total=int(P.flat.numel()), has_sd_conv=bool(P.has_sd_conv))
+    return P.flat, dict(total=int(P.flat.numel()), has_sd_conv=bool(P.has_sd_conv), fold_up=P.fold_up)
 
 
 def unflatten_packed(flat: torch.Tensor, manifest: dict, cfg: UNetConfig, device) -> PackedWeights:
     assert manifest["total"] == flat.numel()
-    return PackedWeights.from_flat(flat, cfg, device, manifest["has_sd_conv"])
+    return PackedWeights.from_flat(flat, cfg, device, manifest["has_sd_conv"], manifest.get("fold_up"))
 
 
 def broadcast_packed(P: Optional[PackedWeights], cfg: UNetConfig, device, src: int = 0) -> PackedWeights:
diff --git a/layoutllm_t2i_amd/engine.py b/layoutllm_t2i_amd/engine.py
--- a/layoutllm_t2i_amd/engine.py
+++ b/layoutllm_t2i_amd/engine.py
@@ -34,7 +34,7 @@
         self.W, self.S = packed.w, packed.s
         init_device(self.dev.index)
         self._lib = _lib.lib()
-        self.handle = _lib.create_engine(self.cfg)
+        self.handle = _lib.create_engine(self.cfg, getattr(packed, "fold_up", None))
         with torch.cuda.device(self.dev):
             check(self._lib.gl_load_weights(self.handle, packed.flat.data_ptr(), packed.flat.numel(), int(packed.has_sd_conv), self._stream()),
                   "gl_load_weights")
diff --git a/layoutllm_t2i_amd/ops.py b/layoutllm_t2i_amd/ops.py
--- a/layoutllm_t2i_amd/ops.py
+++ b/layoutllm_t2i_amd/ops.py
@@ -169,8 +169,15 @@
     if in_split:
         Cin //= 2
     N, K, _ = _rows(w, "w")
-    if K != (18 if w_split else 9) * Cin:
-        raise ValueError("w must be [Cout, 9*Cin] ([Cout, 18*Cin] with w_split)")
+    folded = bool(upsample2x) and K == 4 * Cin and not w_split
+    if folded:
+        if n_valid is not None:
+            raise ValueError("n_valid does not go with folded upsample weights")
+        if N % 4:
+            raise ValueError("folded upsample weights must be [4*Cout, 4*Cin]")
+        N //= 4
+    elif K != (18 if w_split else 9) * Cin:
+        raise ValueError("w must be [Cout, 9*Cin] ([Cout, 18*Cin] with w_split; [4*Cout, 4*Cin] folded upsample weights)")
     if upsample2x:
         Hout, Wout = 2 * Hin, 2 * Win
     elif pad01:
@@ -180,7 +187,7 @@
     a = ConvArgs()
     a.inp = x.data_ptr()
     a.B, a.Hin, a.Win, a.Cin, a.Hout, a.Wout = B, Hin, Win, Cin, Hout, Wout
-    a.stride, a.upsample2x = stride, int(upsample2x)
+    a.stride, a.upsample2x = stride, (2 if folded else int(bool(upsample2x)))
     a.in_split, a.w_split = int(in_split), int(bool(w_split))
     a.g.w = w.data_ptr()
     a.g.N = N if n_valid is None else n_valid
@@ -581,6 +588,13 @@
     return int(n.value)
 
 
+def upfold_launch_count() -> int:
+    import ctypes
+    n = ctypes.c_uint64(0)
+    check(_lib.lib().gl_debug_read(12, ctypes.byref(n), 8), "gl_debug_read")
+    return int(n.value)
+
+
 ATTN_FORMS = ("split_pipe", "split_8w", "split_4w_dbuf", "split_4w_single", "f16_8w_pre0", "f16_8w_pre1", "f16_8w_pre2", "f16_4w_pre0",
               "f16_4w_pre1", "f16_4w_pre2")
 
diff --git a/layoutllm_t2i_amd/vae.py b/layoutllm_t2i_amd/vae.py
--- a/layoutllm_t2i_amd/vae.py
+++ b/layoutllm_t2i_amd/vae.py
@@ -7,7 +7,7 @@
 from . import ops
 from ._lib import EPI_BIAS, EPI_RES, init_device
 from .arch import VAEConfig, vae_decoder_param_shapes, vae_encoder_param_shapes
-from .weights import CIN_PAD, _h, _t, pack_conv3x3
+from .weights import CIN_PAD, _h, _t, pack_conv3x3, pack_conv_upfold
 
 F16, F32 = torch.float16, torch.float32
 _FP32_1X1 = ("post_quant_conv", "quant_conv")
@@ -21,7 +21,21 @@
     return "f32_1x1" if p in _FP32_1X1 else "gemm"
 
 
-def packed_shapes(param_shapes: Mapping[str, Tuple[int, ...]]) -> Dict[str, Tuple[Tuple[int, ...], torch.dtype]]:
+VAE_UPFOLD_MIN_CHANNELS = 256
+
+
+def _fold(fold_up, cfg) -> bool:
+    from . import _lib
+    ups = [shp[0] for n, shp in vae_decoder_param_shapes(cfg).items() if n.endswith(".upsample.conv.weight")]
+    return _lib.resolve_fold_up(fold_up, bool(ups) and min(ups) >= VAE_UPFOLD_MIN_CHANNELS)
+
+
+def _is_upsample(p: str) -> bool:
+    return p.startswith("decoder.up.") and p.endswith(".upsample.conv")
+
+
+def packed_shapes(param_shapes: Mapping[str, Tuple[int, ...]], fold_up: bool = False) -> Dict[str, Tuple[Tuple[int, ...], torch.dtype]]:
+    fold = bool(fold_up)
     out: Dict[str, Tuple[Tuple[int, ...], torch.dtype]] = {}
     for name, shp in param_shapes.items():
         if not name.endswith(".weight"):
@@ -30,7 +44,9 @@
         if kind == "norm":
             out[p + ".g"], out[p + ".b"] = ((shp[0],), F32), ((shp[0],), F32)
             continue
-        if kind == "conv3x3":
+        if kind == "conv3x3" and fold and _is_upsample(p):
+            out[p + ".w"] = ((4 * shp[0], 4 * shp[1]), F16)
+        elif kind == "conv3x3":
             out[p + ".w"] = ((shp[0], 9 * (CIN_PAD if shp[1] < 64 else shp[1])), F16)
         else:
             out[p + ".w"] = ((shp[0], shp[1]), F32 if kind == "f32_1x1" else F16)
@@ -38,7 +54,7 @@
     return out
 
 
-def _pack(state_dict: Mapping[str, object], need: Mapping[str, Tuple[int, ...]], device) -> Dict[str, torch.Tensor]:
+def _pack(state_dict: Mapping[str, object], need: Mapping[str, Tuple[int, ...]], device, fold_up=False) -> Dict[str, torch.Tensor]:
     g = lambda k: _t(state_dict[k], device)
     W: Dict[str, torch.Tensor] = {}
     for name, shp in need.items():
@@ -50,6 +66,9 @@
         kind = _pack_kind(p, shp)
         if kind == "norm":
             W[p + ".g"], W[p + ".b"] = w.contiguous(), b.contiguous()
+        elif kind == "conv3x3" and fold_up and _is_upsample(p):
+            W[p + ".w"] = pack_conv_upfold(w)
+            W[p + ".b"] = b.contiguous()
         elif kind == "conv3x3":
             W[p + ".w"] = pack_conv3x3(w, CIN_PAD if shp[1] < 64 else None)
             W[p + ".b"] = b.contiguous()
@@ -79,7 +98,7 @@
 
     def _bind_engine(self):
         from . import _lib
-        self.handle = _lib.create_vae(self.cfg, encoder=self._encoder_stage)
+        self.handle = _lib.create_vae(self.cfg, encoder=self._encoder_stage, fold_up=getattr(self, "fold_up", None))
         table, total = _lib.vae_weight_table(self.handle)
         flat = torch.zeros(total, dtype=torch.uint8, device=self.device)
         views = {}
@@ -164,17 +183,18 @@
 
 
 class VAEDecoder(_VAEStage):
-    def __init__(self, state_dict: Mapping[str, object], cfg: VAEConfig = VAEConfig(), device="cuda:0"):
+    def __init__(self, state_dict: Mapping[str, object], cfg: VAEConfig = VAEConfig(), device="cuda:0", fold_up=None):
         if not torch.cuda.is_available():
             raise RuntimeError("VAEDecoder needs a GPU: there is no CPU fallback")
         init_device()
         self.cfg, self.device = cfg, torch.device(device)
         self.scale_factor = cfg.scale_factor
+        self.fold_up = _fold(fold_up, cfg)
         need = vae_decoder_param_shapes(cfg)
         missing = [k for k in need if k not in state_dict]
         if missing:
             raise KeyError(f"autoencoder state_dict is missing {len(missing)} decoder tensors, e.g. {missing[:3]}")
-        self.W = _pack(state_dict, need, self.device)
+        self.W = _pack(state_dict, need, self.device, self.fold_up)
         self._pool: Dict[tuple, torch.Tensor] = {}
         self._bind_engine()
         enc_missing = [k for k in vae_encoder_param_shapes(cfg) if k not in state_dict]
@@ -190,6 +210,8 @@
         self = cls.__new__(cls)
         self.cfg, self.device, self.scale_factor = cfg, torch.device(device), cfg.scale_factor
         self.W = {k: v.to(self.device) for k, v in W.items()}
+        ups = [v for k, v in self.W.items() if k.endswith(".w") and _is_upsample(k[:-2])]
+        self.fold_up = bool(ups) and all(v.shape[0] == v.shape[1] for v in ups)
         self._pool = {}
         self._bind_engine()
         self.encoder = None
diff --git a/layoutllm_t2i_amd/weights.py b/layoutllm_t2i_amd/weights.py
--- a/layoutllm_t2i_amd/weights.py
+++ b/layoutllm_t2i_amd/weights.py
@@ -37,6 +37,34 @@
     return _h(wp.reshape(cout, -1))
 
 
+UPFOLD_TAPS = (((0,), (1, 2)), ((0, 1), (2,)))
+
+
+UPFOLD_MIN_CHANNELS = 512
+
+
+def fold_up_rule(cfg: UNetConfig) -> bool:
+    ups = [l.cin for l in build_plan(cfg).all_layers() if l.kind == "up"]
+    return bool(ups) and min(ups) >= UPFOLD_MIN_CHANNELS and not getattr(cfg, "split_weights", False)
+
+
+def pack_conv_upfold(w32: torch.Tensor) -> torch.Tensor:
+    w32 = w32.float()
+    cout, cin = w32.shape[0], w32.shape[1]
+    assert tuple(w32.shape[2:]) == (3, 3) and cin % 64 == 0, "upsample conv: 3x3 kernel, input channels a multiple of 64"
+    out = []
+    for py in range(2):
+        for px in range(2):
+            f = torch.zeros(cout, cin, 2, 2, dtype=torch.float32, device=w32.device)
+            for a in range(2):
+                for b in range(2):
+                    for ky in UPFOLD_TAPS[py][a]:
+                        for kx in UPFOLD_TAPS[px][b]:
+                            f[:, :, a, b] += w32[:, :, ky, kx]
+            out.append(f.reshape(cout, cin // 64, 64, 2, 2).permute(0, 1, 3, 4, 2).reshape(cout, -1))
+    return _h(torch.cat(out, 0))
+
+
 def pack_first_conv(w: torch.Tensor, cin_pad: int) -> torch.Tensor:
     w = w.float()
     if 3 * w.shape[1] > cin_pad:
@@ -64,13 +92,14 @@
         self.emb_total = 0
         self.flat: torch.Tensor | None = None
         self.has_sd_conv = False
+        self.fold_up: bool | None = None
 
     def nbytes(self) -> int:
         return int(self.flat.numel()) if self.flat is not None else sum(t.numel() * t.element_size() for t in self.w.values())
 
     def to_flat(self) -> "PackedWeights":
         from . import _lib
-        handle = _lib.create_engine(self.cfg)
+        handle = _lib.create_engine(self.cfg, self.fold_up)
         try:
             table, total = _lib.weight_table(handle)
         finally:
@@ -101,10 +130,11 @@
         return self
 
     @staticmethod
-    def from_flat(flat: torch.Tensor, cfg: UNetConfig, device, has_sd_conv: bool) -> "PackedWeights":
+    def from_flat(flat: torch.Tensor, cfg: UNetConfig, device, has_sd_conv: bool, fold_up: bool | None = None) -> "PackedWeights":
         from . import _lib
         P = PackedWeights(cfg, build_plan(cfg), device)
-        handle = _lib.create_engine(cfg)
+        P.fold_up = fold_up = _lib.resolve_fold_up(fold_up, fold_up_rule(cfg))
+        handle = _lib.create_engine(cfg, fold_up)
         try:
             table, total = _lib.weight_table(handle)
         finally:
@@ -127,8 +157,8 @@
         return P
 
 
-def pack_state_dict(sd: Mapping[str, object], cfg: UNetConfig, device, sd_first_conv: Mapping[str, object] | None = None
-                    ) -> PackedWeights:
+def pack_state_dict(sd: Mapping[str, object], cfg: UNetConfig, device, sd_first_conv: Mapping[str, object] | None = None,
+                    fold_up: bool | None = None) -> PackedWeights:
     plan = build_plan(cfg)
     need = param_shapes(cfg)
     missing = [k for k in need if k not in sd]
@@ -143,6 +173,9 @@
     W, S = P.w, P.s
     g = lambda k: _t(sd[k], device)
     split_all = bool(getattr(cfg, "split_weights", False))
+    from . import _lib
+    P.fold_up = _lib.resolve_fold_up(fold_up, fold_up_rule(cfg))
+    fold = P.fold_up and not split_all
 
     def mat(w32: torch.Tensor) -> torch.Tensor:
         w32 = w32.reshape(w32.shape[0], -1).float()
@@ -202,7 +235,10 @@
     emb_w, emb_b, off = [], [], 0
     for l in plan.all_layers():
         p = l.prefix
-        if l.kind in ("down", "up"):
+        if l.kind == "up" and fold:
+            W[p + ".w"] = pack_conv_upfold(g(p + ".weight"))
+            W[p + ".b"] = g(p + ".bias").contiguous()
+        elif l.kind in ("down", "up"):
             conv3(p)
         elif l.kind == "res":
             norm(p + ".in_layers.0")
```
